# sp-uhh/buddy

Measured on AMD Instinct MI355X. Metric: diffusion steps/sec (4 s@16 kHz utterance, blind Euler-Heun DPS, order 1, 10 operator updates/step), higher is better.
Workload: dtype f32 (GEMM operands -- Winograd-domain and 1x1 / NIN -- as two-term f16 splits, 2^-22, fp32 accumulation)

## Files before the change

### buddy_amd/_lib.py

```python
from __future__ import annotations

import ctypes as C
import os

_HERE = os.path.dirname(os.path.abspath(__file__))
LIB_PATH = os.path.join(_HERE, "libbuddy_hip.so")


class BuddyHipError(RuntimeError):
    pass


_lib = None

_f32p = C.c_void_p
_SIGS = {
    "buddy_last_error": (C.c_char_p, []),
    "buddy_version": (C.c_int, []),
    "buddy_ncsnpp_param_count": (C.c_int, [C.c_int, C.POINTER(C.c_int), C.c_int, C.c_int, C.POINTER(C.c_longlong)]),
    "buddy_ncsnpp_create": (C.c_int, [_f32p, C.c_longlong, C.c_int, C.POINTER(C.c_int), C.c_int, C.c_int, C.c_int, C.c_int,
                                      C.POINTER(C.c_void_p)]),
    "buddy_ncsnpp_param_count_attn": (C.c_int, [C.c_int, C.POINTER(C.c_int), C.c_int, C.c_int, C.c_int, C.POINTER(C.c_longlong)]),
    "buddy_ncsnpp_create_attn": (C.c_int, [_f32p, C.c_longlong, C.c_int, C.POINTER(C.c_int), C.c_int, C.c_int, C.c_int, C.c_int, C.c_int,
                                           C.POINTER(C.c_void_p)]),
    "buddy_ncsnpp_destroy": (C.c_int, [C.c_void_p]),
    "buddy_ncsnpp_replica": (C.c_int, [C.c_void_p, C.POINTER(C.c_void_p)]),
    "buddy_ncsnpp_weight_bytes": (C.c_int, [C.c_void_p, C.POINTER(C.c_longlong), C.POINTER(C.c_longlong), C.POINTER(C.c_longlong),
                                            C.POINTER(C.c_int)]),
    "buddy_conv3_weight_prep": (C.c_int, [_f32p, C.c_int, C.c_int, C.c_int, C.c_int, _f32p, C.c_void_p]),
    "buddy_ncsnpp_reserve": (C.c_int, [C.c_void_p, C.c_int, C.c_int, C.c_int, C.POINTER(C.c_longlong)]),
    "buddy_ncsnpp_forward": (C.c_int, [C.c_void_p, _f32p, _f32p, _f32p, _f32p, _f32p, _f32p, C.c_int, C.c_int, C.c_int, C.c_void_p]),
    "buddy_ncsnpp_vjp": (C.c_int, [C.c_void_p, _f32p, _f32p, C.c_void_p]),
    "buddy_ncsnpp_vjp_params": (C.c_int, [C.c_void_p, _f32p, _f32p, _f32p, C.c_int, C.c_void_p]),
    "buddy_ncsnpp_update_params": (C.c_int, [C.c_void_p, _f32p, C.c_void_p]),
    "buddy_optim_sqnorm_chunk": (C.c_longlong, []),
    "buddy_optim_sqnorm": (C.c_int, [_f32p, C.c_longlong, C.c_void_p, C.c_void_p, C.c_void_p]),
    "buddy_optim_step": (C.c_int, [_f32p, _f32p, _f32p, _f32p, _f32p, C.c_longlong, C.c_void_p, C.c_double, C.c_double, C.c_double, C.c_double,
                                   C.c_double, C.c_double, C.c_double, C.POINTER(C.c_longlong), C.c_int, C.c_void_p]),
    "buddy_optim_ema": (C.c_int, [_f32p, _f32p, C.c_longlong, C.c_double, C.c_void_p]),
    "buddy_ncsnpp_tap": (C.c_int, [C.c_void_p, C.c_int, C.POINTER(C.c_void_p), C.POINTER(C.c_int * 4)]),
    "buddy_prof_enable": (C.c_int, [C.c_int]),
    "buddy_wpe": (C.c_int, [_f32p, _f32p, _f32p, C.c_int, C.c_int, C.c_int, C.c_int, C.c_int, C.c_void_p]),
    "buddy_wpe_workspace_bytes": (C.c_longlong, [C.c_int, C.c_int]),
    "buddy_wpe_dereverb": (C.c_int, [_f32p, _f32p, C.c_void_p, C.c_int, C.c_int, C.c_int, C.c_int, C.c_int, C.c_void_p]),
    "buddy_prof_collect_wino4": (C.c_int, [C.POINTER(C.c_double), C.POINTER(C.c_double), C.POINTER(C.c_double), C.POINTER(C.c_double), C.POINTER(C.c_double),
                                           C.POINTER(C.c_longlong)]),
    "buddy_prof_collect_hbm": (C.c_int, [C.POINTER(C.c_double), C.POINTER(C.c_double), C.POINTER(C.c_longlong)]),
    "buddy_prof_collect": (C.c_int, [C.POINTER(C.c_double), C.POINTER(C.c_double), C.POINTER(C.c_longlong), C.POINTER(C.c_double), C.POINTER(C.c_double)]),
    "buddy_copy_d2d": (C.c_int, [C.c_void_p, C.c_void_p, C.c_longlong, C.c_void_p]),
    "buddy_hbm_ubench": (C.c_int, [C.c_void_p, C.c_void_p, C.c_longlong, C.c_int, C.c_int, C.c_int, C.c_void_p]),
    "buddy_mfma_ubench": (C.c_int, [_f32p, _f32p, C.c_int, C.c_int, C.c_void_p, C.c_void_p]),
    "buddy_mfma_ubench_bf16": (C.c_int, [_f32p, _f32p, C.c_int, C.c_int, C.c_void_p, C.c_void_p]),
    "buddy_gemm": (C.c_int, [_f32p, C.c_int, C.c_int, _f32p, C.c_int, C.c_int, _f32p, C.c_int, C.c_int, C.c_int, C.c_int, C.c_float,
                             _f32p, C.c_int, C.c_int, C.c_longlong, C.c_longlong, C.c_longlong, C.c_void_p]),
    "buddy_gemm_winograd_domain": (C.c_int, [_f32p, _f32p, _f32p, C.c_int, C.c_int, C.c_int, C.c_int, C.c_void_p]),
    "buddy_wgemm_packed_bytes": (C.c_longlong, [C.c_int, C.c_int, C.c_int]),
    "buddy_wgemm_pack_weights": (C.c_int, [_f32p, C.c_void_p, C.c_int, C.c_int, C.c_int, C.c_void_p]),
    "buddy_gemm_winograd_domain_bf16x3": (C.c_int, [_f32p, C.c_void_p, _f32p, C.c_int, C.c_int, C.c_int, C.c_int, C.c_void_p]),
    "buddy_wgemm_f16x2_packed_bytes": (C.c_longlong, [C.c_int, C.c_int, C.c_int]),
    "buddy_wgemm_f16x2_pack_weights": (C.c_int, [_f32p, C.c_void_p, C.c_int, C.c_int, C.c_int, C.c_void_p]),
    "buddy_gemm_winograd_domain_f16x2": (C.c_int, [_f32p, C.c_void_p, _f32p, C.c_int, C.c_int, C.c_int, C.c_int, C.c_void_p, C.c_int, C.c_void_p]),
    "buddy_wgemm_f16_packed_bytes": (C.c_longlong, [C.c_int, C.c_int, C.c_int]),
    "buddy_wgemm_f16_pack_weights": (C.c_int, [_f32p, C.c_void_p, C.c_int, C.c_int, C.c_int, C.c_void_p]),
    "buddy_gemm_winograd_domain_f16": (C.c_int, [C.c_void_p, C.c_void_p, C.c_void_p, _f32p, C.c_int, C.c_int, C.c_int, C.c_int, C.c_void_p]),
    "buddy_conv3x3_winograd6_f16": (C.c_int, [_f32p, C.c_void_p, _f32p, _f32p, _f32p, C.c_int, C.c_int, C.c_int, C.c_int, C.c_int, C.c_void_p]),
    "buddy_abs_max_bits": (C.c_int, [_f32p, C.c_int, C.c_int, C.c_longlong, C.c_void_p, C.c_void_p]),
    "buddy_gemm_bf16x3": (C.c_int, [_f32p, C.c_int, _f32p, C.c_int, C.c_int, C.c_void_p, _f32p, C.c_int, C.c_longlong, C.c_int, C.c_int, _f32p, C.c_float,
                                    C.c_int, C.c_void_p]),
    "buddy_conv3x3": (C.c_int, [_f32p, _f32p, _f32p, _f32p, C.c_int, C.c_int, C.c_int, C.c_int, C.c_int, C.c_void_p]),
    "buddy_winograd_transform_weights": (C.c_int, [C.c_void_p, C.c_int, C.c_int, C.c_void_p]),
    "buddy_winograd4_transform_weights": (C.c_int, [C.c_void_p, C.c_int, C.c_int, C.c_void_p]),
    "buddy_conv3x3_winograd4": (C.c_int, [_f32p, _f32p, _f32p, _f32p, _f32p, C.c_int, C.c_int, C.c_int, C.c_int, C.c_int, C.c_void_p]),
    "buddy_winograd6_transform_weights": (C.c_int, [C.c_void_p, C.c_int, C.c_int, C.c_void_p]),
    "buddy_conv3x3_winograd6": (C.c_int, [_f32p, _f32p, _f32p, _f32p, _f32p, C.c_int, C.c_int, C.c_int, C.c_int, C.c_int, C.c_void_p]),
    "buddy_gn_conv3x3_winograd6": (C.c_int, [_f32p, _f32p, C.c_int, _f32p, _f32p, C.c_int, C.c_int, _f32p, _f32p, _f32p, _f32p, _f32p, C.c_void_p,
                                             C.c_void_p, C.c_int, C.c_int, C.c_int, C.c_int, C.c_int, C.c_void_p]),
    "buddy_gn_conv3x3_winograd6_f16": (C.c_int, [_f32p, _f32p, C.c_int, _f32p, _f32p, C.c_int, C.c_int, _f32p, _f32p, _f32p, _f32p, _f32p, C.c_void_p,
                                                 C.c_void_p, C.c_int, C.c_int, C.c_int, C.c_int, C.c_int, C.c_void_p]),
    "buddy_conv3x3_winograd6_gn_bwd_sums": (C.c_int, [_f32p, _f32p, _f32p, _f32p, _f32p, _f32p, C.c_int, _f32p, _f32p, _f32p, C.c_int, C.c_int,
                                                      C.c_void_p, C.c_void_p, C.c_int, C.c_int, C.c_int, C.c_int, C.c_int, C.c_void_p]),
    "buddy_gemm_bf16x3_gn_bwd": (C.c_int, [_f32p, C.c_int, C.c_void_p, _f32p, _f32p, C.c_int, _f32p, _f32p, _f32p, _f32p, C.c_int, C.c_int, C.c_float,
                                           _f32p, _f32p, C.c_int, C.c_int, C.c_void_p, _f32p, C.c_int, C.c_int, C.c_int, C.c_int, C.c_void_p]),
    "buddy_gemm_f16x2": (C.c_int, [_f32p, C.c_int, _f32p, C.c_int, C.c_int, C.c_void_p, _f32p, C.c_int, C.c_longlong, C.c_int, C.c_int, _f32p, C.c_float,
                                    C.c_int, C.c_void_p]),
    "buddy_gemm_f16x2_gn_bwd": (C.c_int, [_f32p, C.c_int, C.c_void_p, _f32p, _f32p, C.c_int, _f32p, _f32p, _f32p, _f32p, C.c_int, C.c_int, C.c_float,
                                           _f32p, _f32p, C.c_int, C.c_int, C.c_void_p, _f32p, C.c_int, C.c_int, C.c_int, C.c_int, C.c_void_p]),
    "buddy_gn_upconv3x3_winograd6": (C.c_int, [_f32p, _f32p, _f32p, C.c_int, C.c_int, _f32p, _f32p, _f32p, _f32p, _f32p, C.c_void_p, C.c_void_p,
                                               C.c_int, C.c_int, C.c_int, C.c_int, C.c_int, C.c_void_p]),
    "buddy_gn_upconv3x3_winograd6_f16": (C.c_int, [_f32p, _f32p, _f32p, C.c_int, C.c_int, _f32p, _f32p, _f32p, _f32p, _f32p, C.c_void_p, C.c_void_p,
                                                   C.c_int, C.c_int, C.c_int, C.c_int, C.c_int, C.c_void_p]),
    "buddy_gnbwd_upconv3x3_winograd6": (C.c_int, [_f32p, _f32p, _f32p, _f32p, _f32p, C.c_int, C.c_int, _f32p, _f32p, _f32p, C.c_void_p, _f32p,
                                                  C.c_int, C.c_int, C.c_int, C.c_int, C.c_int, C.c_void_p]),
    "buddy_gnbwd_upconv3x3_winograd6_f16": (C.c_int, [_f32p, _f32p, _f32p, _f32p, _f32p, C.c_int, C.c_int, _f32p, _f32p, _f32p, C.c_void_p, _f32p,
                                                      C.c_int, C.c_int, C.c_int, C.c_int, C.c_int, C.c_void_p]),
    "buddy_gnbwd_conv3x3_winograd6": (C.c_int, [_f32p, _f32p, _f32p, _f32p, _f32p, C.c_int, C.c_int, _f32p, _f32p, _f32p, C.c_void_p, _f32p,
                                                C.c_int, C.c_int, C.c_int, C.c_int, C.c_int, C.c_void_p]),
    "buddy_gnbwd_conv3x3_winograd6_f16": (C.c_int, [_f32p, _f32p, _f32p, _f32p, _f32p, C.c_int, C.c_int, _f32p, _f32p, _f32p, C.c_void_p, _f32p,
                                                    C.c_int, C.c_int, C.c_int, C.c_int, C.c_int, C.c_void_p]),
    "buddy_gn_conv3x3_winograd4": (C.c_int, [_f32p, _f32p, C.c_int, _f32p, _f32p, C.c_int, C.c_int, _f32p, _f32p, _f32p, _f32p, _f32p, C.c_void_p,
                                             C.c_void_p, C.c_int, C.c_int, C.c_int, C.c_int, C.c_int, C.c_void_p]),
    "buddy_conv3x3_winograd": (C.c_int, [_f32p, _f32p, _f32p, _f32p, C.c_int, C.c_int, C.c_int, C.c_int, C.c_int, C.c_void_p]),
    "buddy_groupnorm_act": (C.c_int, [_f32p, _f32p, _f32p, _f32p, _f32p, C.c_void_p, C.c_int, C.c_int, C.c_int, C.c_int, C.c_int,
                                      C.c_int, C.c_int, C.c_void_p]),
    "buddy_groupnorm_act_bwd": (C.c_int, [_f32p, _f32p, _f32p, _f32p, _f32p, _f32p, C.c_void_p, _f32p, C.c_int, C.c_int, C.c_int,
                                          C.c_int, C.c_int, C.c_int, C.c_int, C.c_void_p]),
    "buddy_fir_resample2": (C.c_int, [_f32p, _f32p, C.c_int, C.c_int, C.c_int, C.c_int, C.c_int, C.c_float, C.c_int, C.c_void_p]),
    "buddy_ncsnpp_set_fir": (C.c_int, [C.c_void_p, C.c_int]),
    "buddy_ncsnpp_set_gemm": (C.c_int, [C.c_void_p, C.c_int]),
    "buddy_ncsnpp_set_attention": (C.c_int, [C.c_void_p, C.c_int]),
    "buddy_options_check": (C.c_int, []),
    "buddy_option_validate": (C.c_int, [C.c_char_p, C.c_int]),
    "buddy_ncsnpp_set_option": (C.c_int, [C.c_void_p, C.c_char_p, C.c_int]),
    "buddy_ncsnpp_get_option": (C.c_int, [C.c_void_p, C.c_char_p, C.POINTER(C.c_int)]),
    "buddy_flash_attention_fwd": (C.c_int, [_f32p, _f32p, _f32p, _f32p, _f32p, C.c_int, C.c_int, C.c_int, C.c_float, C.c_int, C.c_void_p]),
    "buddy_flash_attention_bwd": (C.c_int, [_f32p, _f32p, _f32p, _f32p, _f32p, _f32p, _f32p, _f32p, _f32p, _f32p, C.c_int, C.c_int, C.c_int, C.c_float,
                                            C.c_int, C.c_void_p]),
    "buddy_flash_attention16_workspace": (C.c_longlong, [C.c_int, C.c_int, C.c_int]),
    "buddy_flash_attention16_fwd": (C.c_int, [_f32p, _f32p, _f32p, _f32p, _f32p, C.c_int, C.c_int, C.c_int, C.c_float, C.c_int, _f32p, C.c_void_p]),
    "buddy_flash_attention16_bwd": (C.c_int, [_f32p, _f32p, _f32p, _f32p, _f32p, _f32p, _f32p, _f32p, _f32p, _f32p, C.c_int, C.c_int, C.c_int, C.c_float,
                                              C.c_int, _f32p, C.c_void_p]),
    "buddy_flash_attention_splits": (C.c_int, [C.c_int, C.c_int]),
    "buddy_flash_attention_workspace": (C.c_longlong, [C.c_int, C.c_int, C.c_int, C.c_int]),
    "buddy_flash_attention_fwd_split": (C.c_int, [_f32p, _f32p, _f32p, _f32p, _f32p, C.c_int, C.c_int, C.c_int, C.c_float, C.c_int, _f32p, C.c_void_p]),
    "buddy_flash_attention_bwd_split": (C.c_int, [_f32p, _f32p, _f32p, _f32p, _f32p, _f32p, _f32p, _f32p, _f32p, _f32p, C.c_int, C.c_int, C.c_int, C.c_float,
                                                  C.c_int, _f32p, C.c_void_p]),
    "buddy_axpby_rows": (C.c_int, [_f32p, _f32p, _f32p, _f32p, _f32p, C.c_int, C.c_int, C.c_void_p]),
    "buddy_perturb": (C.c_int, [_f32p, _f32p, C.c_float, _f32p, C.c_longlong, C.c_void_p]),
    "buddy_dps_update": (C.c_int, [_f32p, _f32p, _f32p, _f32p, _f32p, _f32p, _f32p, C.c_float, C.c_float, C.c_float, C.c_float, _f32p, _f32p, _f32p,
                                   C.c_int, C.c_int, C.c_void_p]),
    "buddy_row_scale": (C.c_int, [_f32p, _f32p, C.c_int, C.c_int, C.c_int, C.c_float, C.c_float, C.c_void_p]),
    "buddy_fill_rows4": (C.c_int, [_f32p, C.c_int, C.c_float, C.c_float, C.c_float, C.c_float, C.c_void_p]),
    "buddy_row_moments": (C.c_int, [_f32p, C.c_void_p, C.c_int, C.c_int, C.c_void_p]),
    "buddy_blindop_create": (C.c_int, [C.c_int, C.c_int, C.c_int, C.c_int, C.c_int, C.POINTER(C.c_float), C.c_int, C.c_float, C.c_float, C.c_float,
                                       C.c_float, C.c_float, C.c_int, C.c_int, C.POINTER(C.c_void_p)]),
    "buddy_blindop_destroy": (C.c_int, [C.c_void_p]),
    "buddy_blindop_set_params": (C.c_int, [C.c_void_p, _f32p, _f32p, _f32p, C.c_int, C.c_void_p]),
    "buddy_blindop_get_params": (C.c_int, [C.c_void_p, _f32p, _f32p, _f32p, C.c_void_p]),
    "buddy_blindop_update_H": (C.c_int, [C.c_void_p, _f32p, C.c_void_p]),
    "buddy_blindop_get_H": (C.c_int, [C.c_void_p, _f32p, C.c_void_p]),
    "buddy_blindop_set_y": (C.c_int, [C.c_void_p, _f32p, C.c_void_p]),
    "buddy_blindop_degrade": (C.c_int, [C.c_void_p, _f32p, _f32p, C.c_void_p]),
    "buddy_blindop_time_rir": (C.c_int, [C.c_void_p, _f32p, C.c_void_p]),
    "buddy_blindop_design_filter": (C.c_int, [C.c_void_p, _f32p, C.c_void_p]),
    "buddy_blindop_apply_stft": (C.c_int, [C.c_void_p, _f32p, _f32p, C.c_void_p]),
    "buddy_blindop_degrade_vjp": (C.c_int, [C.c_void_p, _f32p, _f32p, _f32p, _f32p, C.c_void_p]),
    "buddy_blindop_time_rir_vjp": (C.c_int, [C.c_void_p, _f32p, _f32p, C.c_void_p]),
    "buddy_blindop_update_H_vjp": (C.c_int, [C.c_void_p, _f32p, _f32p, _f32p, _f32p, C.c_void_p]),
    "buddy_blindop_stft": (C.c_int, [C.c_void_p, _f32p, C.c_int, _f32p, C.c_void_p]),
    "buddy_blindop_stft_adjoint": (C.c_int, [C.c_void_p, _f32p, C.c_int, _f32p, C.c_void_p]),
    "buddy_blindop_stft_loss": (C.c_int, [C.c_void_p, _f32p, _f32p, C.c_int, C.c_float, _f32p, _f32p, _f32p, C.c_void_p]),
    "buddy_blindop_set_compression": (C.c_int, [C.c_void_p, C.c_float]),
    "buddy_blindop_set_loss_norm": (C.c_int, [C.c_void_p, C.c_int]),
    "buddy_blindop_set_loss": (C.c_int, [C.c_void_p, C.c_int, C.c_int, C.c_int, C.c_float]),
    "buddy_blindop_set_freq_weights": (C.c_int, [C.c_void_p, C.c_int, _f32p]),
    "buddy_blindop_lengths": (C.c_int, [C.c_void_p, C.POINTER(C.c_int), C.POINTER(C.c_int), C.POINTER(C.c_int), C.POINTER(C.c_int)]),
    "buddy_blindop_minphase": (C.c_int, [C.c_void_p, _f32p, _f32p, C.c_void_p]),
    "buddy_blindop_project": (C.c_int, [C.c_void_p, C.c_void_p]),
    "buddy_blindop_get_adam": (C.c_int, [C.c_void_p, _f32p, _f32p, _f32p, _f32p, _f32p, _f32p, C.POINTER(C.c_int), C.c_void_p]),
    "buddy_blindop_rec_loss_grad": (C.c_int, [C.c_void_p, _f32p, C.c_float, _f32p, _f32p, C.c_void_p]),
    "buddy_blindop_fir_loss_grad": (C.c_int, [C.c_void_p, _f32p, _f32p, C.c_longlong, C.c_int, C.c_float, _f32p, _f32p, C.c_void_p]),
    "buddy_blindop_param_grads": (C.c_int, [C.c_void_p, _f32p, _f32p, C.c_float, C.c_float, C.c_float, _f32p, _f32p, _f32p, _f32p, C.c_void_p]),
    "buddy_blindop_optimize": (C.c_int, [C.c_void_p, _f32p, _f32p, C.c_float, C.c_int, C.c_float, C.c_float, C.c_float, C.c_float, C.c_float,
                                         C.c_float, C.c_void_p]),
    "buddy_fir": (C.c_int, [_f32p, _f32p, C.c_longlong, _f32p, C.c_int, C.c_int, C.c_int, C.c_int, C.c_void_p]),
}
EXPORTED = sorted(_SIGS)


def load():
    global _lib
    if _lib is None:
        if not os.path.exists(LIB_PATH):
            raise BuddyHipError(f"{LIB_PATH} not found: build it with `python -c 'import __graft_entry__ as g; g.build()'` "
                                "(buddy_amd/csrc/build.sh); there is no CPU fallback")
        import torch
        lib = C.CDLL(LIB_PATH)
        for name, (res, args) in _SIGS.items():
            fn = getattr(lib, name)
            fn.restype, fn.argtypes = res, args
        _lib = lib
        rc = lib.buddy_options_check()
        if rc != 0:
            msg = lib.buddy_last_error().decode()
            _lib = None
            raise BuddyHipError(f"libbuddy_hip: {msg}")
    return _lib


# ... 25 lines not shown
```

### buddy_amd/csrc/capi.hip

```cpp
#include "../../include/buddy_hip.h"
#include "common.h"
#include "net.h"

#include <cstring>

using namespace buddy;

namespace buddy {
void launch_axpby_rows(const float* x, const float* y, const float* a, const float* c, float* out, int B, int L, hipStream_t st);
void launch_row_moments(const float* x, double* out, int B, int L, hipStream_t st);
void launch_perturb(const float* x, const float* eps, float scale, float* out, long long n, hipStream_t st);
void launch_dps_update(const float* x_hat, const float* x_den, const float* lh, const float* lh_scale_b, const float* den_scale_b, const float* base, const float* d_prev,
                       float t, float dt, float w_prev, float w_cur, float* out, float* d_out, float* x_den_out, int B, int L, hipStream_t st);
void launch_row_scale(const float* x, float* out, int B, int L, int mode, float p0, float p1, hipStream_t st);
void launch_fill_rows4(float* out, int B, float v0, float v1, float v2, float v3, hipStream_t st);
void launch_mfma_ubench(const float* seed, float* out, int blocks, int iters, unsigned long long* clk, hipStream_t st);
void launch_mfma_ubench_bf16(const float* seed, float* out, int blocks, int iters, unsigned long long* clk, hipStream_t st);
int launch_hbm_ubench(const void* src, void* dst, long long bytes, int mode, int nt, int blocks, hipStream_t st);
void launch_fir(const float* x, const float* h, long long h_stride, float* y, int B, int L, int M, int adjoint, hipStream_t st);
}

static int finish() {
  hipError_t e = hipGetLastError();
  if (e != hipSuccess) { set_error(std::string("kernel launch: ") + hipGetErrorString(e)); return BUDDY_ERR_HIP; }
// ... 412 lines not shown
  W4Gn gn;
  gn.x.p0 = x; gn.x.p1 = nullptr; gn.x.C0 = C; gn.x.ld0 = C; gn.x.ld1 = 0;
  gn.stats = stats; gn.gamma = gamma; gn.beta = beta; gn.G = G; gn.silu = silu; gn.da = da; gn.ldda = C; gn.red = red;
  launch_gn_bwd_sums(gn.x, stats, gamma, beta, da, B, up ? 2 * H : H, up ? 2 * W : W, C, G, 0, silu, stat_scratch, red, st);
  long long vf = 0, mf = 0; wino6_scratch(p, &vf, &mf, up);
  launch_wino6(p, U6, scratch, scratch + vf, st, &gn, nullptr, nullptr, U1, up, U1 ? 3 : 1);
  return finish();
}
int buddy_gnbwd_conv3x3_winograd6(const float* x, const float* gamma, const float* beta, const float* stats, const float* da, int G, int silu,
                                  const float* U6, float* y, float* scratch, double* stat_scratch, float* red, int B, int H, int W, int C, int Cout,
                                  void* stream) {
  return gnbwd_conv3x3_winograd6(0, x, gamma, beta, stats, da, G, silu, U6, nullptr, y, scratch, stat_scratch, red, B, H, W, C, Cout, stream);
}
int buddy_gnbwd_conv3x3_winograd6_f16(const float* x, const float* gamma, const float* beta, const float* stats, const float* da, int G, int silu,
                                      const void* U1, float* y, float* scratch, double* stat_scratch, float* red, int B, int H, int W, int C, int Cout,
                                      void* stream) {
  if (!U1) { set_error("null argument"); return BUDDY_ERR_ARG; }
  return gnbwd_conv3x3_winograd6(0, x, gamma, beta, stats, da, G, silu, nullptr, U1, y, scratch, stat_scratch, red, B, H, W, C, Cout, stream);
}

static int gn_upconv3x3_winograd6(const float* x, const float* gamma, const float* beta, int G, int silu, const float* U6up, const void* U1, const float* bias,
                                  float* y, float* scratch, float* stats, double* stat_scratch, double* csum, int B, int H, int W, int Cin, int Cout, void* stream) {
  if (!x || !gamma || !beta || !(U6up || U1) || !y || !scratch || !stats || !stat_scratch || G < 1 || Cin % 4 || (Cin / G) % 4 || Cin > 1024 || Cout % 4 ||
      (U1 && !wgemm_f16_supported(4 * Cout, Cin))) {
    set_error("bad arguments"); return BUDDY_ERR_ARG;
  }
  hipStream_t st = (hipStream_t)stream;
  IgemmParams p; std::memset(&p, 0, sizeof(p));
  p.ldA0 = Cin; p.Cin = Cin; p.H = H; p.W = W; p.M = B * H * W; p.N = Cout; p.C = y; p.ldC = Cout;
  p.bias_n = bias; p.alpha = 1.f; p.out_scale = 1.f; p.rows_per_batch = H * W;
  if (!wino6_supported(p)) { set_error("shape not supported by the F(6x6,3x3) path (H, W >= 6; Cin, Cout multiples of 4)"); return BUDDY_ERR_ARG; }
  const int sc = csum ? wino6_stat_chunks(p, 1) : 0;
  if (csum && (sc == 0 || (long long)sc * Cout > 256LL * 1024)) { set_error("shape not supported by the statistics epilogue"); return BUDDY_ERR_ARG; }
  W4Gn gn;
  gn.x.p0 = x; gn.x.p1 = nullptr; gn.x.C0 = Cin; gn.x.ld0 = Cin; gn.x.ld1 = 0;
  gn.stats = stats; gn.gamma = gamma; gn.beta = beta; gn.G = G; gn.silu = silu;
  launch_gn_stats(gn.x, B, H * W, Cin, G, 1e-6f, stat_scratch, stats, st);
  long long vf = 0, mf = 0; wino6_scratch(p, &vf, &mf, 1);
  launch_wino6(p, U6up, scratch, scratch + vf, st, &gn, csum ? stat_scratch : nullptr, nullptr, U1, 1, U1 ? 3 : 1);
  if (csum) launch_csum_collapse(stat_scratch, sc, B, Cout, csum, st);
  return finish();
}

int buddy_gn_upconv3x3_winograd6(const float* x, const float* gamma, const float* beta, int G, int silu, const float* U6up, const float* bias, float* y,
                                 float* scratch, float* stats, double* stat_scratch, double* csum, int B, int H, int W, int Cin, int Cout, void* stream) {
  return gn_upconv3x3_winograd6(x, gamma, beta, G, silu, U6up, nullptr, bias, y, scratch, stats, stat_scratch, csum, B, H, W, Cin, Cout, stream);
}
int buddy_gn_upconv3x3_winograd6_f16(const float* x, const float* gamma, const float* beta, int G, int silu, const void* U1up, const float* bias, float* y,
                                     float* scratch, float* stats, double* stat_scratch, double* csum, int B, int H, int W, int Cin, int Cout, void* stream) {
  if (!U1up) { set_error("null argument"); return BUDDY_ERR_ARG; }
  return gn_upconv3x3_winograd6(x, gamma, beta, G, silu, nullptr, U1up, bias, y, scratch, stats, stat_scratch, csum, B, H, W, Cin, Cout, stream);
}

int buddy_gnbwd_upconv3x3_winograd6(const float* h, const float* gamma, const float* beta, const float* stats, const float* da, int G, int silu,
                                    const float* U6upT, float* y, float* scratch, double* stat_scratch, float* red, int B, int H, int W, int C,
                                    int Cout, void* stream) {
  return gnbwd_conv3x3_winograd6(2, h, gamma, beta, stats, da, G, silu, U6upT, nullptr, y, scratch, stat_scratch, red, B, H, W, C, Cout, stream);
}
int buddy_gnbwd_upconv3x3_winograd6_f16(const float* h, const float* gamma, const float* beta, const float* stats, const float* da, int G, int silu,
                                        const void* U1upT, float* y, float* scratch, double* stat_scratch, float* red, int B, int H, int W, int C,
                                        int Cout, void* stream) {
  if (!U1upT) { set_error("null argument"); return BUDDY_ERR_ARG; }
  return gnbwd_conv3x3_winograd6(2, h, gamma, beta, stats, da, G, silu, nullptr, U1upT, y, scratch, stat_scratch, red, B, H, W, C, Cout, stream);
}

int buddy_groupnorm_act(const float* x, const float* gamma, const float* beta, float* y, float* stats, void* scratch, int B, int H, int W, int C,
                        int G, int mode, int silu, void* stream) {
  if (!x || !y || !stats || !scratch || C % 4 || (C / G) % 4 || C > 1024) { set_error("bad groupnorm arguments"); return BUDDY_ERR_ARG; }
  Src2 s; s.p0 = x; s.p1 = nullptr; s.C0 = C; s.ld0 = C; s.ld1 = 0;
  launch_gn_stats(s, B, H * W, C, G, 1e-6f, (double*)scratch, stats, (hipStream_t)stream);
  launch_gn_apply(s, stats, gamma, beta, B, H, W, C, G, mode, silu, y, nullptr, (hipStream_t)stream);
  return finish();
}

int buddy_groupnorm_act_bwd(const float* x, const float* gamma, const float* beta, const float* stats, const float* dy, float* dx, void* scratch,
                            float* red, int B, int H, int W, int C, int G, int mode, int silu, void* stream) {
  if (!x || !dy || !dx || !stats || !scratch || !red || C % 4 || (C / G) % 4 || C > 1024) { set_error("bad groupnorm arguments"); return BUDDY_ERR_ARG; }
  Src2 s; s.p0 = x; s.p1 = nullptr; s.C0 = C; s.ld0 = C; s.ld1 = 0;
  Dst2 d; d.p0 = dx; d.p1 = nullptr; d.C0 = C; d.ld0 = C; d.ld1 = 0; d.acc0 = 0; d.acc1 = 0;
  launch_gn_bwd(s, stats, gamma, beta, dy, B, H, W, C, G, mode, silu, nullptr, 0, 0.f, (double*)scratch, red, d, (hipStream_t)stream);
  return finish();
}

int buddy_options_check(void) { return options_check(); }
int buddy_option_validate(const char* key, int value) { Options o = default_options(); return option_set(o, key, value); }
int buddy_ncsnpp_set_option(void* h, const char* key, int value) { if (!h) { set_error("null handle"); return BUDDY_ERR_ARG; } return net_set_option((Net*)h, key, value); }
int buddy_ncsnpp_get_option(void* h, const char* key, int* value) { if (!h) { set_error("null handle"); return BUDDY_ERR_ARG; } return net_get_option((Net*)h, key, value); }
int buddy_ncsnpp_set_gemm(void* h, int mode) { if (!h) { set_error("null handle"); return BUDDY_ERR_ARG; } return net_set_gemm((Net*)h, mode); }
int buddy_ncsnpp_set_attention(void* h, int mode) { if (!h) { set_error("null handle"); return BUDDY_ERR_ARG; } return net_set_attention((Net*)h, mode); }
int buddy_ncsnpp_set_fir(void* h, int fir) { if (!h) { set_error("null handle"); return BUDDY_ERR_ARG; } return net_set_fir((Net*)h, fir); }
int buddy_fir_resample2(const float* x, float* y, int B, int H, int W, int C, int up, float scale, int accumulate, void* stream) {
  if (!x || !y || B < 1 || H < 1 || W < 1 || C < 1 || (!up && ((H | W) & 1))) { set_error("bad resample arguments"); return BUDDY_ERR_ARG; }
  if (up) launch_fir_up2(x, y, B, H, W, C, scale, accumulate, (hipStream_t)stream);
  else launch_fir_down2(x, y, B, H, W, C, scale, accumulate, (hipStream_t)stream);
  return finish();
}

int buddy_flash_attention_fwd(const float* q, const float* k, const float* v, float* O, float* lse, int B, int T, int C, float scale, int prec,
                              void* stream) {
  if (!q || !k || !v || !O || !lse || B < 1 || T < 1 || !flash_attn_supported(C) || prec != 0) {
    set_error("bad attention arguments (C in {32, 64, 128, 256}; prec 0 -- the 16-bit-operand kernels are buddy_flash_attention16_*)"); return BUDDY_ERR_ARG;
  }
  launch_flash_attn_fwd(q, k, v, O, lse, B, T, C, scale, nullptr, 1, (hipStream_t)stream);
  return finish();
}
long long buddy_flash_attention16_workspace(int B, int T, int C) { return (B < 1 || T < 1 || !flash_attn16_supported(C)) ? 0 : flash_attn16_ws_floats(B, T, C); }
int buddy_flash_attention16_fwd(const float* q, const float* k, const float* v, float* O, float* lse, int B, int T, int C, float scale, int prec, float* ws,
                                void* stream) {
  if (!q || !k || !v || !O || !lse || !ws || B < 1 || T < 1 || !flash_attn16_supported(C) || prec < 1 || prec > 2) {
    set_error("bad attention arguments (C in {64, 128, 256}; prec 1 = bf16, 2 = f16; ws = buddy_flash_attention16_workspace floats)"); return BUDDY_ERR_ARG;
  }
  launch_flash_attn16_fwd(q, k, v, O, lse, B, T, C, scale, prec, ws, (hipStream_t)stream);
  return finish();
}
int buddy_flash_attention16_bwd(const float* q, const float* k, const float* v, const float* O, const float* dO, const float* lse, float* delta, float* dq,
                                float* dk, float* dv, int B, int T, int C, float scale, int prec, float* ws, void* stream) {
  if (!q || !k || !v || !O || !dO || !lse || !delta || !dq || !dk || !dv || !ws || B < 1 || T < 1 || !flash_attn16_supported(C) || prec < 1 || prec > 2) {
    set_error("bad attention arguments (C in {64, 128, 256}; prec 1 = bf16, 2 = f16; ws = buddy_flash_attention16_workspace floats)"); return BUDDY_ERR_ARG;
  }
  launch_flash_attn16_bwd(q, k, v, O, dO, lse, delta, dq, dk, dv, B, T, C, scale, prec, ws, (hipStream_t)stream);
  return finish();
}
long long buddy_flash_attention_workspace(int B, int T, int C, int splits) {
  if (B < 1 || T < 1 || !flash_attn_supported(C)) return 0;
  return flash_attn_ws_floats(B, T, C, splits > 0 ? splits : flash_attn_splits(B, T));
}
int buddy_flash_attention_splits(int B, int T) { return (B < 1 || T < 1) ? 1 : flash_attn_splits(B, T); }
static bool split_args_ok(int T, int splits, const float* ws) {
  const int nb = (T + 31) / 32;
  if (splits < 1 || splits > nb || (splits > 1 && !ws)) return false;
  return splits == 1 || (long long)((nb + splits - 1) / splits) * (splits - 1) < nb;
}
int buddy_flash_attention_fwd_split(const float* q, const float* k, const float* v, float* O, float* lse, int B, int T, int C, float scale, int splits,
                                    float* ws, void* stream) {
  if (!q || !k || !v || !O || !lse || B < 1 || T < 1 || !flash_attn_supported(C) || !split_args_ok(T, splits, ws)) {
    set_error("bad split-attention arguments (C in {32, 64, 128, 256}; every split needs at least one 32-row block)"); return BUDDY_ERR_ARG;
  }
  launch_flash_attn_fwd(q, k, v, O, lse, B, T, C, scale, ws, splits, (hipStream_t)stream);
  return finish();
}
int buddy_flash_attention_bwd_split(const float* q, const float* k, const float* v, const float* O, const float* dO, const float* lse, float* delta,
                                    float* dq, float* dk, float* dv, int B, int T, int C, float scale, int splits, float* ws, void* stream) {
  if (!q || !k || !v || !O || !dO || !lse || !delta || !dq || !dk || !dv || B < 1 || T < 1 || !flash_attn_supported(C) || !split_args_ok(T, splits, ws)) {
    set_error("bad split-attention arguments (C in {32, 64, 128, 256}; every split needs at least one 32-row block)"); return BUDDY_ERR_ARG;
  }
  launch_flash_attn_bwd(q, k, v, O, dO, lse, delta, dq, dk, dv, B, T, C, scale, ws, splits, (hipStream_t)stream);
  return finish();
}
int buddy_flash_attention_bwd(const float* q, const float* k, const float* v, const float* O, const float* dO, const float* lse, float* delta, float* dq,
                              float* dk, float* dv, int B, int T, int C, float scale, int prec, void* stream) {
  if (prec != 0 || !q || !k || !v || !O || !dO || !lse || !delta || !dq || !dk || !dv || B < 1 || T < 1 || !flash_attn_supported(C)) {
    set_error("bad attention arguments (C in {32, 64, 128, 256}; prec 0 -- the 16-bit-operand kernels are buddy_flash_attention16_*)"); return BUDDY_ERR_ARG;
  }
  launch_flash_attn_bwd(q, k, v, O, dO, lse, delta, dq, dk, dv, B, T, C, scale, nullptr, 1, (hipStream_t)stream);
  return finish();
}

int buddy_axpby_rows(const float* x, const float* y, const float* a, const float* c, float* out, int B, int L, void* stream) {
  if (!x || !a || !out || (y && !c)) { set_error("null argument"); return BUDDY_ERR_ARG; }
  launch_axpby_rows(x, y, a, c, out, B, L, (hipStream_t)stream);
  return finish();
}

int buddy_perturb(const float* x, const float* eps, float scale, float* out, long long n, void* stream) {
  if (!x || !eps || !out) { set_error("null argument"); return BUDDY_ERR_ARG; }
  launch_perturb(x, eps, scale, out, n, (hipStream_t)stream);
// ... 124 lines not shown
```

### buddy_amd/csrc/common.h

```cpp
#pragma once
#include <hip/hip_runtime.h>
#include <cstdint>
#include <cstdio>

#define BUDDY_OK 0
#define BUDDY_ERR_HIP 1
#define BUDDY_ERR_ARG 2
#define BUDDY_ERR_STATE 3

namespace buddy {

struct Options {
  int conv;
  int gemm;
  int attn;
  int gn_fuse, upconv, c2_fuse;
  int attn_split, attn_nw;
  int wgemm_rt, gen_f16x2, gen_rows, gen_cp, gnb_nt;
  int c2out_tiled;
  int op_graph;
};
const Options& default_options();
int options_check();
const Options& cur_opt();
struct OptScope { const Options* prev; explicit OptScope(const Options* o); ~OptScope(); OptScope(const OptScope&) = delete; };
int option_set(Options& o, const char* key, int value);
int option_get(const Options& o, const char* key, int* value);
const char* prof_dump_path();

struct IgemmParams {
  const float* A0; const float* A1; int C0; int ldA0; int ldA1;
  int Cin;
  int H, W;
  int M, N;
  const float* Bt; int ldB;
  float* C; int ldC;
  long long sA, sB, sC;
  const float* bias_n; const float* bias_m; const float* bias_bn; int ld_bias_bn; int rows_per_batch;
  const float* res; int ldRes; int res_mode;
  float alpha, out_scale; int accumulate;
  int wide_epi;
  int tag;
};
void launch_igemm(const IgemmParams& p, int taps, bool transA, bool transB, int batch, hipStream_t st);
bool wgemm_supported(int Cout, int Cin);
size_t wgemm_packed_bytes(int P, int Cout, int Cin);
void wgemm_pack_weights(const float* U_dev, void* U3_dev, int P, int Cout, int Cin, hipStream_t st);
void launch_wgemm_bf16x3(const float* V, const void* U3, float* M, long long Mt, int Cout, int Cin, int P, hipStream_t st);
bool wgemm_f16x2_supported(int Cout, int Cin);
size_t wgemm_f16x2_packed_bytes(int P, int Cout, int Cin);
void wgemm_f16x2_pack_weights(const float* U_dev, void* U2_dev, int P, int Cout, int Cin, hipStream_t st);
constexpr int VMAX_SUB = 64, VMAX_STRIDE = 32;
void launch_abs_max_bits(const float* x, int groups, int segments, long long seg_len, unsigned* out, hipStream_t st);
void launch_wgemm_f16x2(const float* V, const void* U2, float* M, long long Mt, int Cout, int Cin, int P, const unsigned* vmax, int tiles_per_utt, hipStream_t st);
bool wgemm_f16_supported(int Cout, int Cin);
size_t wgemm_f16_packed_bytes(int P, int Cout, int Cin);
void wgemm_f16_pack_weights(const float* U_dev, void* U1_dev, int P, int Cout, int Cin, hipStream_t st);
void launch_wgemm_f16(const void* V16, const signed char* vexp, const void* U1, float* M, long long Mt, int Cout, int Cin, int P, hipStream_t st);
bool wgemm_general_supported(int N, int K, int C0, int ldA0, int ldA1, int ldC, const void* A0, const void* A1, const void* C, const void* bias);
void launch_wgemm_bf16x3_general(const float* A0, int ldA0, const float* A1, int ldA1, int C0, const void* W3, float* C, int ldC, long long M, int N, int K,
                                 const float* bias_n, float alpha, int accumulate, hipStream_t st);
bool wgemm_f16x2_general_supported(int N, int K, int C0, int ldA0, int ldA1, int ldC, const void* A0, const void* A1, const void* C, const void* bias);
void launch_wgemm_f16x2_general(const float* A0, int ldA0, const float* A1, int ldA1, int C0, const void* W2, float* C, int ldC, long long M, int N, int K,
                                const float* bias_n, float alpha, int accumulate, hipStream_t st);
bool wino_supported(const IgemmParams& p);
void launch_wino(const IgemmParams& p, const float* Uw, hipStream_t st);
void wino_transform_weights(const float* wt_host, int Cout, int Cin, float* U_host);
struct Src2 { const float* p0; const float* p1; int C0; int ld0; int ld1; };
struct Dst2 { float* p0; float* p1; int C0; int ld0; int ld1; int acc0; int acc1; };
bool wgemm_gnbwd_supported(int N, int K, int ldA, const Src2& x, const Dst2& d, const void* A, const void* da);
void launch_wgemm_bf16x3_gnbwd(const float* A, int ldA, const void* W3, long long M, int N, int K, float alpha, Src2 x, const float* da, const float* stats,
                               const float* red, const float* gamma, const float* beta, int G, int silu, int HW, Dst2 d, hipStream_t st);
void launch_wgemm_f16x2_gnbwd(const float* A, int ldA, const void* W2, long long M, int N, int K, float alpha, Src2 x, const float* da, const float* stats,
                              const float* red, const float* gamma, const float* beta, int G, int silu, int HW, Dst2 d, hipStream_t st);
struct W4Gn { Src2 x; const float* stats; const float* gamma; const float* beta; int G; int silu;
              const float* da = nullptr; int ldda = 0; const float* red = nullptr; };
bool wino4_supported(const IgemmParams& p);
void wino4_scratch(const IgemmParams& p, long long* v_floats, long long* m_floats);
int wino4_stat_chunks(const IgemmParams& p);
void launch_wino4(const IgemmParams& p, const float* U4, float* V, float* Mb, hipStream_t st, const W4Gn* gn = nullptr, double* stat = nullptr,
                  const void* U4x = nullptr);
void wino4_transform_weights(const float* wt_host, int Cout, int Cin, float* U4_host);
bool wino6_supported(const IgemmParams& p);
bool wino6_pays(const IgemmParams& p);
void wino6_scratch(const IgemmParams& p, long long* v_floats, long long* m_floats, int up = 0);
int wino6_stat_chunks(const IgemmParams& p, int up = 0);
double wino6_exec_ratio(const IgemmParams& p, int up = 0);
void launch_wino6(const IgemmParams& p, const float* U6, float* V, float* Mb, hipStream_t st, const W4Gn* gn = nullptr, double* stat = nullptr,
                  const W4Gn* bwd_gn = nullptr, const void* U6x = nullptr, int up = 0, int xform = 1, unsigned* vmax = nullptr);
void wino6_transform_weights(const float* wt_host, int Cout, int Cin, float* U6_host);
long long conv3_weight_floats(int O, int I, int kind);
int launch_conv3_weight_prep(const float* w_oihw, int O, int I, bool dgrad, int kind, float* out, hipStream_t st);
void igemm_prof_record(const IgemmParams& p, int taps, int batch, hipStream_t st, bool begin, double exec_ratio = 4.0 / 9.0);
void igemm_prof_enable(int level);
bool igemm_prof_enabled();
int igemm_prof_level();
void prof_w4_push(hipEvent_t e0, hipEvent_t e1, hipEvent_t e2, hipEvent_t e3, double gemm_flops, double bytes_in, double bytes_out, double bytes_gemm);
int prof_w4_collect(double ms[3], double* gemm_flops, double* bytes_in, double* bytes_out, double* bytes_gemm, long long* launches);
void prof_hbm_begin(double algorithmic_bytes, hipStream_t st);
void prof_hbm_end(hipStream_t st);
int prof_hbm_collect(double* ms, double* bytes, long long* launches);
int igemm_prof_collect(double ms[2], double flops[2], long long launches[2], double bytes[2], double exec_flops[2]);

void launch_conv_c2in(const float* x, const float* w , const float* bias, const float* add, int add_ld,
                      float* y, int ldY, int B, int H, int W, int Cout, int taps, int accumulate, hipStream_t st);
void launch_conv_c2out(const float* x, int ldX, const float* w , const float* bias, const float* up_add,
                       float* y, int B, int H, int W, int Cin, int taps, int accumulate, hipStream_t st);

int  gn_num_chunks(int HW);
void launch_gn_stats(Src2 x, int B, int HW, int C, int G, float eps, double* partial, float* stats , hipStream_t st);
void launch_chan_sums(const float* x, int B, int HW, int C, double* partial, double* csum, hipStream_t st);
void launch_csum_collapse(const double* partial, int chunks, int B, int C, double* csum, hipStream_t st);
void launch_gn_stats_partial(const double* partial, int chunks, int B, int HW, int C, int G, float eps, float* stats, hipStream_t st);
void launch_gn_stats_csum(const double* csum0, const double* csum1, int C0, int B, int HW, int C, int G, float eps, float* stats, hipStream_t st);
void launch_gn_apply(Src2 x, const float* stats, const float* gamma, const float* beta, int B, int H, int W, int C, int G,
                     int mode, int silu, float* out, float* pooled_raw, hipStream_t st);
void launch_gn_bwd_sums(Src2 x, const float* stats, const float* gamma, const float* beta, const float* da, int B, int H, int W, int C, int G,
                        int mode, int silu, double* partial, float* red , hipStream_t st, int ready_chunks = 0);
void launch_gn_bwd_apply(Src2 x, const float* stats, const float* gamma, const float* beta, const float* da, int B, int H, int W, int C, int G,
                         int mode, int silu, const float* extra, int extra_mode, float extra_scale, const float* red, Dst2 dx, hipStream_t st);
void launch_gn_bwd(Src2 x, const float* stats, const float* gamma, const float* beta, const float* da, int B, int H, int W, int C,
                   int G, int mode, int silu, const float* extra, int extra_mode, float extra_scale, double* partial,
                   float* red , Dst2 dx, hipStream_t st, int ready_chunks = 0);

void launch_wpe(const double* Y, double* X, double* inv_scratch, int rows, int T, int taps, int delay, int iters, hipStream_t st);
size_t wpe_workspace_bytes(int B, int L);
int wpe_frames(int L);
void launch_wpe_dereverb(const float* y, float* out, void* work, int B, int L, int taps, int delay, int iters, hipStream_t st);
void launch_axpy(float* dst, const float* src, float alpha, long long n, int accumulate, hipStream_t st);
void launch_fir_up2(const float* x, float* y, int B, int H, int W, int C, float scale, int accumulate, hipStream_t st);
void launch_fir_down2(const float* x, float* y, int B, int H, int W, int C, float scale, int accumulate, hipStream_t st);
void launch_pool2(const float* src, float* dst, int B, int H, int W, int C, float scale, int accumulate, hipStream_t st);
void launch_up2_acc(const float* src, float* dst, int B, int Hs, int Ws, int C, float scale, int accumulate, hipStream_t st);
bool flash_attn_supported(int C);
bool flash_attn16_supported(int C);
int flash_attn_splits(int B, int T);
long long flash_attn_ws_floats(int B, int T, int C, int splits);
void launch_flash_attn_fwd(const float* q, const float* k, const float* v, float* O, float* Lse, int B, int T, int C, float scale, float* ws, int splits,
                           hipStream_t st);
void launch_flash_attn_bwd(const float* q, const float* k, const float* v, const float* O, const float* dO, const float* Lse, float* D, float* dq,
                           float* dk, float* dv, int B, int T, int C, float scale, float* ws, int splits, hipStream_t st);
long long flash_attn16_ws_floats(int B, int T, int C);
void launch_flash_attn16_fwd(const float* q, const float* k, const float* v, float* O, float* Lse, int B, int T, int C, float scale, int prec, float* ws,
                             hipStream_t st);
void launch_flash_attn16_bwd(const float* q, const float* k, const float* v, const float* O, const float* dO, const float* Lse, float* D, float* dq,
                             float* dk, float* dv, int B, int T, int C, float scale, int prec, float* ws, hipStream_t st);
void launch_softmax_rows(float* S, int rows, int cols, hipStream_t st);
void launch_softmax_bwd_rows(const float* P, float* dP , int rows, int cols, hipStream_t st);
void launch_linear(const float* x, const float* W, const float* b, float* y, int B, int K, int N, int silu_in, hipStream_t st);
void launch_fourier(const float* cnoise, const float* Wf, float* out, int B, int nf, hipStream_t st);
void launch_mix2(const float* x, const float* w , const float* b, float* y, long long npix, int transpose, int accumulate, hipStream_t st);

void launch_reflect_pad(const float* x, float* xp, int B, int L, int pad, int Lp, float scale, const float* scale_b, hipStream_t st);
void launch_ola(const float* frames, int ldF, int Tp, int n_fft, int hop, const float* inv_env, float* y, int B, int L,
                int pad, const float* xin, const float* cskip_b, const float* cout_b, hipStream_t st);
void launch_ola_adj(const float* g, int B, int L, int pad, int Tp, int n_fft, int hop, const float* inv_env, const float* cout_b,
                    float* frames, int ldF, hipStream_t st);
void launch_unpad_adj(const float* dframes, int ldF, int T, int n_fft, int hop, int B, int L, int pad, float scale,
                      const float* scale_b, const float* g_out, const float* cskip_b, float* dx, hipStream_t st);

inline int cdiv(long long a, long long b) { return (int)((a + b - 1) / b); }

struct WgY { const float* p; long long T, sb, sm, sn; };
struct WgA { Src2 x; int H, W, Cin, taps, rs; const float* stats; const float* gamma; const float* beta; int G, silu; };
int wgrad_chunks(long long M, int N, int K);
long long wgrad_ws_floats(long long M, int N, int K);
void launch_wgrad(const WgY& y, const WgA& a, long long M, int N, int layout, float alpha, float* ws, float* out, hipStream_t st);
long long colsum_ws_floats(int B, long long T, int N);
void launch_colsum(const WgY& y, int B, int N, float alpha, float* ws, float* bc, int ld_bc, float* out, float* out2, hipStream_t st);
long long basis_bias_ws_floats(int B, long long T, int K);
void launch_basis_bias(const float* x, int K, int B, long long T, const double* bsum, float* ws, float* out, hipStream_t st);
long long gn_pgrad_ws_floats(int B, int H, int W, int C);
void launch_gn_pgrad(const Src2& x, const float* stats, const float* gamma, const float* beta, int G, int silu, const float* da, int da_mode, int B,
                     int H, int W, int C, float* ws, float* dgamma, float* dbeta, hipStream_t st);
void launch_linear_bwd_w(const float* dy, int ld_dy, const float* x, int silu_in, int B, int N, int K, float* gw, float* gb, float* gb2, hipStream_t st);
void launch_linear_bwd_x(const float* dy, const float* W, const float* x, int silu_in, int B, int N, int K, float* dx, hipStream_t st);

}
```

### buddy_amd/csrc/net.hip

```cpp
#include "common.h"
#include "net.h"

#include <algorithm>
#include <cmath>
#include <cstdlib>
#include <cstring>
#include <deque>
#include <functional>
#include <memory>
#include <mutex>
#include <string>
#include <vector>
#include <unordered_map>

namespace buddy {

#define HIPCHK(x) do { hipError_t e_ = (x); if (e_ != hipSuccess) { set_error(std::string(#x) + ": " + hipGetErrorString(e_)); return BUDDY_ERR_HIP; } } while (0)

static thread_local std::string g_err;
void set_error(const std::string& s) { g_err = s; }
const char* last_error() { return g_err.c_str(); }

static const float INV_SQRT2 = 0.70710678118654752440f;

// ... 62 lines not shown
  return v.back().off + v.back().numel;
}

struct Tens {
  float* p = nullptr; float* g = nullptr; int ginit = 0;
  int B = 0, H = 0, W = 0, C = 0;
  double* csum = nullptr; bool has_csum = false;
  long long numel() const { return (long long)B * H * W * C; }
};
struct View { Tens* a = nullptr; Tens* b = nullptr; int C() const { return a->C + (b ? b->C : 0); } };

struct Arena {
  char* base = nullptr; size_t cap = 0, off = 0, peak = 0; bool dry = false; bool overflow = false;
  void* alloc(size_t bytes) {
    off = (off + 255) & ~(size_t)255;
    void* r = dry ? (void*)(uintptr_t)(0x10000 + off) : (void*)(base + off);
    off += bytes;
    if (off > peak) peak = off;
    if (!dry && off > cap) overflow = true;
    return r;
  }
  float* f(long long n) { return (float*)alloc((size_t)n * 4); }
};

struct WVar { float* u = nullptr; void* x[4] = {nullptr, nullptr, nullptr, nullptr}; };
struct ConvW { int cin = 0, cout = 0, taps = 0; const float* raw = nullptr; float* wf = nullptr; float* wb = nullptr; float* bias = nullptr;
               mutable WVar var[2][5];
               long long go = -1; };
struct GNW { float* gamma = nullptr; float* beta = nullptr; int C = 0; long long go = -1; };
struct ResW { GNW gn0, gn1; ConvW c0, c1, c2; bool has_c2 = false; int cin = 0, cout = 0, dense_off = 0; long long dense_go = -1; };
struct AttnW { GNW gn; float* Wt[4]; float* Wn[4]; float* b[4]; int C = 0; int level = -1;
               long long go[4] = {-1, -1, -1, -1}; };

struct W3Img { const void* img; int N, K; const void* img2 = nullptr; };
struct Weights {
  NetCfg cfg;
  std::vector<PSpec> specs;
  float* dparams = nullptr;
  float* dpacked = nullptr;
  std::vector<long long> doff;
  std::vector<float> host_pack;
  std::vector<std::pair<long long, std::function<std::vector<float>(const float*)>>> repack;
  struct Img { const float* src; void* img; void* img2; int n, k; };
  std::vector<Img> imgs;
  int gen = 0;
  long long lin1_go = -1, lin2_go = -1, out_go = -1;
  float* Wf = nullptr; float* lin1_w = nullptr; float* lin1_b = nullptr; float* lin2_w = nullptr; float* lin2_b = nullptr;
  float* dense_w = nullptr; float* dense_b = nullptr; int dense_total = 0;
  ConvW conv_in;
  std::vector<ResW> res;
  std::vector<ConvW> combine;
  AttnW attn;
  std::vector<AttnW> sites;
  std::vector<GNW> pyr_gn; std::vector<ConvW> pyr_conv;
  float* out_w = nullptr; float* out_b = nullptr;
  float* basisF = nullptr; float* basisI = nullptr;
  double* basisI_sum = nullptr;
  unsigned char* dpacked3 = nullptr;
  std::unordered_map<const float*, W3Img> w3;
  std::mutex mu;
  std::vector<void*> lazy_allocs; size_t lazy_bytes = 0; int lazy_count = 0;
  float* prep_tmp = nullptr; size_t prep_cap = 0;
  ~Weights() {
    if (dparams) (void)hipFree(dparams);
    if (dpacked) (void)hipFree(dpacked);
    if (dpacked3) (void)hipFree(dpacked3);
    if (basisI_sum) (void)hipFree(basisI_sum);
    if (prep_tmp) (void)hipFree(prep_tmp);
    for (void* q : lazy_allocs) (void)hipFree(q);
  }
};

struct Net {
  NetCfg cfg;
  int Fb = 0, Kp = 0, pad = 0;
  std::shared_ptr<Weights> W;
  int B = 0, L = 0, T = 0, Tp = 0, Lp = 0;
  float* inv_env = nullptr; int env_len = 0; int env_Tp = -1;
  Arena arena;
  std::deque<Tens> pool;
  std::vector<std::function<void()>> tape;
  std::vector<std::pair<int, Tens*>> taps;
  double* partial = nullptr; float* red = nullptr;
  bool have_tape = false;
  hipStream_t st = nullptr;
  bool pgrad = false, pg_run = false; float* pg = nullptr; float* dtemb = nullptr; int tape_gen = 0;
  const float* k_four = nullptr; const float* k_t1 = nullptr; const float* k_temb = nullptr;
  Tens* spec = nullptr; Tens* pyr0 = nullptr;
  const float* k_cin = nullptr; const float* k_cskip = nullptr; const float* k_cout = nullptr;

  int rsv_B = 0, rsv_L = 0, rsv_vjp = -1;
  Options opt;
  bool prep_failed = false;
  bool fir = false;
  float* w4_scratch = nullptr; size_t w4_cap = 0, w4_need = 0;
  unsigned* vmax = nullptr; size_t vmax_cap = 0; int vslot = 0, vslots = 0, vdry = 0;
  int vslot_need[2] = {0, 0};
  bool dry() const { return arena.dry; }
  Tens* mk(int B_, int H, int W, int C, bool grad) {
    pool.emplace_back();
    Tens* t = &pool.back();
    t->B = B_; t->H = H; t->W = W; t->C = C;
    t->p = arena.f(t->numel());
    if (grad) t->g = arena.f(t->numel());
    t->csum = (double*)arena.alloc((size_t)B_ * C * 2 * sizeof(double));
    return t;
  }
  float* tmp(long long n) { return arena.f(n); }
};

namespace {
struct Packer {
  std::vector<float> buf;
  long long put(const std::vector<float>& v) {
    long long off = (long long)buf.size();
    buf.insert(buf.end(), v.begin(), v.end());
    while (buf.size() % 64) buf.push_back(0.f);
    return off;
  }
};

inline float w3(const float* w, int O, int I, int o, int i, int dy, int dx) { return w[(((long long)o * I + i) * 3 + dx) * 3 + dy]; }

std::vector<float> transpose2(const float* w, int R, int Cc) {
  std::vector<float> r((size_t)R * Cc);
  for (int i = 0; i < R; ++i) for (int j = 0; j < Cc; ++j) r[(size_t)j * R + i] = w[(size_t)i * Cc + j];
  return r;
}
}

static const PSpec* find_spec(const std::vector<PSpec>& v, const std::string& n) {
  for (auto& s : v) if (s.name == n) return &s;
  return nullptr;
}


static int weights_create(const float* hp, long long n, const NetCfg& cfg, std::shared_ptr<Weights>* out) {
  auto Wp = std::make_shared<Weights>();
  Weights* N = Wp.get();
  N->cfg = cfg;
  N->specs = build_specs(cfg);
  if (n != param_count(cfg)) { set_error("parameter blob size mismatch"); return BUDDY_ERR_ARG; }
  if (cfg.n_fft % 2) { set_error("n_fft must be even"); return BUDDY_ERR_ARG; }
  if (cfg.attn_mask < 0 || (cfg.attn_mask >> cfg.nlev) != 0) { set_error("attention mask selects a level the network does not have"); return BUDDY_ERR_ARG; }
  {
    int cmax = 0;
    for (int l = 0; l < cfg.nlev; ++l) cmax = std::max(cmax, cfg.nf * cfg.ch_mult[l]);
    if (2 * cmax > 1024) { set_error("nf * max(ch_mult) must be <= 512 (concatenated skip tensors of up to 1024 channels)"); return BUDDY_ERR_ARG; }
  }
  for (const PSpec& ps : N->specs) {
    if (ps.name.find("GroupNorm_") == std::string::npos) continue;
    const int C = ps.shape[0];
    if (C % 4 || (C > 128 && C % 128)) {
      set_error("unsupported width: a GroupNorm over " + std::to_string(C) + " channels (" + ps.name + ") has " + std::to_string(C / (C / 4 < 32 ? C / 4 : 32)) +
                " channels per group; the kernels need a multiple of 4 (C <= 128 or C % 128 == 0)");
      return BUDDY_ERR_ARG;
    }
  }
  const int Fb = cfg.n_fft / 2 + 1, Kp = (cfg.n_fft + 3) / 4 * 4;
  if (Fb % (1 << (cfg.nlev - 1))) { set_error("frequency bins not divisible by 2^(levels-1)"); return BUDDY_ERR_ARG; }
  std::vector<long long>& doff = N->doff;
  doff.resize(N->specs.size());
  {
    long long o = 0;
    for (size_t i = 0; i < N->specs.size(); ++i) { doff[i] = o; o += (N->specs[i].numel + 63) / 64 * 64; }
    HIPCHK(hipMalloc(&N->dparams, (size_t)o * 4));
// ... 321 lines not shown
  const int ki = kind == 0 ? 0 : kind == 2 ? 1 : kind == 4 ? 2 : kind == 6 ? 3 : 4;
  WVar& v = c.var[dgrad ? 1 : 0][ki];
  std::lock_guard<std::mutex> lk(Wt->mu);
  if (want_x ? v.x[want_x] != nullptr : v.u != nullptr) return &v;
  const int ph = kind == 61 ? 4 : 1;
  const int Co = dgrad ? c.cin : ph * c.cout, Ci = dgrad ? ph * c.cout : c.cin;
  const size_t nfl = (size_t)conv3_weight_floats(c.cout, c.cin, kind);
  hipStream_t st = N->st;
  float* u = v.u;
  if (u == nullptr) {
    if (want_x) {
      if (Wt->prep_cap < nfl) {
        if (Wt->prep_tmp) (void)hipFree(Wt->prep_tmp);
        Wt->prep_tmp = nullptr; Wt->prep_cap = 0;
        if (hipMalloc(&Wt->prep_tmp, nfl * 4) != hipSuccess) { N->prep_failed = true; set_error("out of memory preparing convolution weights"); return nullptr; }
        Wt->prep_cap = nfl;
      }
      u = Wt->prep_tmp;
    } else {
      if (hipMalloc(&u, nfl * 4) != hipSuccess) { N->prep_failed = true; set_error("out of memory preparing convolution weights"); return nullptr; }
      Wt->lazy_allocs.push_back(u); Wt->lazy_bytes += nfl * 4;
    }
    if (launch_conv3_weight_prep(c.raw, c.cout, c.cin, dgrad, kind, u, st) != BUDDY_OK) { N->prep_failed = true; set_error("bad weight form"); return nullptr; }
  }
  void* x = nullptr;
  if (want_x) {
    const int P = kind == 4 ? 36 : 64;
    const size_t bytes = kArith[want_x].packed_bytes(P, Co, Ci);
    if (hipMalloc(&x, bytes) != hipSuccess) { N->prep_failed = true; set_error("out of memory preparing convolution weights"); return nullptr; }
    Wt->lazy_allocs.push_back(x); Wt->lazy_bytes += bytes;
    kArith[want_x].pack_weights(u, x, P, Co, Ci, st);
  }
  (void)hipStreamSynchronize(st);
  if (want_x) v.x[want_x] = x; else v.u = u;
  ++Wt->lazy_count;
  return &v;
}

static Src2 src_of(const View& v) {
  Src2 s; s.p0 = v.a->p; s.p1 = v.b ? v.b->p : nullptr; s.C0 = v.a->C; s.ld0 = v.a->C; s.ld1 = v.b ? v.b->C : 0;
  return s;
}
static Dst2 gdst_of(const View& v) {
  Dst2 d; d.p0 = v.a->g; d.p1 = v.b ? v.b->g : nullptr; d.C0 = v.a->C; d.ld0 = v.a->C; d.ld1 = v.b ? v.b->C : 0;
  d.acc0 = v.a->ginit; d.acc1 = v.b ? v.b->ginit : 0;
  v.a->ginit = 1; if (v.b) v.b->ginit = 1;
  return d;
}
static IgemmParams ig_base() {
  IgemmParams p; std::memset(&p, 0, sizeof(p));
  p.alpha = 1.f; p.out_scale = 1.f; p.rows_per_batch = 1; p.H = 1; p.W = 1;
  return p;
}
static inline int gn_groups(int C) { int g = C / 4; return g < 32 ? g : 32; }

struct Conv3 {
  const float* a = nullptr;
  int B = 0, H = 0, W = 0, Cin = 0, Cout = 0;
  const ConvW* w = nullptr; bool dgrad = false;
  const float* bias = nullptr; const float* bias_bn = nullptr; int ld_bn = 0;
  const float* res = nullptr; int ldRes = 0; int res_mode = 0;
  float alpha = 1.f, out_scale = 1.f;
  float* out = nullptr;
  const W4Gn* gn = nullptr; float* gn_tmp = nullptr;
  Tens* stat_out = nullptr; bool direct = false;
  const W4Gn* bwd_gn = nullptr;
  int up = 0;
};
static unsigned* vmax_slot(Net* N, int B) {
  if (N->vmax == nullptr || N->vslot >= N->vslots || (size_t)(N->vslot + 1) * B * VMAX_SUB * VMAX_STRIDE > N->vmax_cap) { N->prep_failed = true; set_error("abs-max slots of the f16x2 GEMM exhausted"); return nullptr; }
  return N->vmax + (size_t)(N->vslot++) * B * VMAX_SUB * VMAX_STRIDE;
}
static bool conv3_up_ok(Net* N, int B, int H, int W, int Cin, int Cout) {
  if (H < 7 || W < 7) return false;
  const Options& o = N->opt;
  const bool on = o.conv == 0 && o.gn_fuse && o.upconv;
  if (!on || Cin % 8 || Cout % 8 || H < 6 || W < 6) return false;
  IgemmParams p = ig_base();
  p.ldA0 = Cin; p.Cin = Cin; p.H = H; p.W = W; p.M = B * H * W; p.N = Cout; p.ldC = Cout; p.ld_bias_bn = 4;
  if (!wino6_supported(p) || !wino6_pays(p)) return false;
  const int sc = wino6_stat_chunks(p, 1);
  return sc > 0 && (long long)sc * Cout <= 256LL * 1024 && (long long)wino6_stat_chunks(p, 0) * Cin <= 256LL * 1024;
}
static int conv3(Net* N, const Conv3& c) {
  const float* a = c.a; const int B = c.B, H = c.H, W = c.W, Cin = c.Cin, Cout = c.Cout;
  if (N->prep_failed) return -1;
  if (N->dry()) ++N->vdry;
  const bool wino_ok = c.w != nullptr && c.w->raw != nullptr && Cin % 8 == 0 && Cout % 8 == 0;
  const W4Gn* gn = c.gn; float* gn_tmp = c.gn_tmp; Tens* stat_out = c.stat_out; const W4Gn* bwd_gn = c.bwd_gn; const bool direct = c.direct;
  const int cmode = N->opt.conv;
  const bool use_wino = cmode != 1, use_wino4 = cmode != 1 && cmode != 2, use_wino6 = use_wino4 && cmode != 3;
  if (N->dry()) {
    if (use_wino4 && wino_ok && H % 4 == 0 && W % 4 == 0) {
      const size_t need = (size_t)36 * ((size_t)B * H * W / 16) * (size_t)(Cin + Cout);
      if (need > N->w4_need) N->w4_need = need;
    }
    if (use_wino6 && wino_ok && H >= 6 && W >= 6) {
      const size_t th = c.up == 1 ? H / 7 + 1 : c.up == 2 ? (H + 6) / 7 : (H + 5) / 6, tw = c.up == 1 ? W / 7 + 1 : c.up == 2 ? (W + 6) / 7 : (W + 5) / 6;
      const size_t need = (size_t)64 * ((size_t)B * th * tw) * (size_t)((c.up == 2 ? 4 : 1) * Cin + (c.up == 1 ? 4 : 1) * Cout);
      if (need > N->w4_need) N->w4_need = need;
    }
    return 0;
  }
  if (c.up) {
    IgemmParams p = ig_base();
    p.A0 = a; p.ldA0 = Cin; p.Cin = Cin; p.H = H; p.W = W; p.M = B * H * W; p.N = Cout; p.C = c.out; p.ldC = Cout;
    p.bias_n = c.bias; p.bias_bn = c.bias_bn; p.ld_bias_bn = c.ld_bn; p.rows_per_batch = H * W; p.alpha = c.alpha; p.out_scale = c.out_scale;
    const int x3 = gemm_arith(N, (c.up == 1 ? 4 : 1) * Cout, (c.up == 2 ? 4 : 1) * Cin);
    const WVar* wv = conv_weights(N, *c.w, c.dgrad, 61, x3);
    unsigned* vm = x3 == 2 ? vmax_slot(N, B) : nullptr;
    if (x3 == 2 && !vm) return -1;
    if (!wv || N->w4_scratch == nullptr) { if (wv) { N->prep_failed = true; set_error("convolution scratch buffer missing"); } return -1; }
    long long vf = 0, mf = 0; wino6_scratch(p, &vf, &mf, c.up);
    const bool want_bwd = c.up == 2 && bwd_gn != nullptr;
    const int sc = (c.up == 1 ? stat_out != nullptr : want_bwd) ? wino6_stat_chunks(p, c.up) : 0;
    const bool stat = sc > 0 && (long long)sc * Cout <= 256LL * 1024;
    IgemmParams pr = p; pr.M = 4 * p.M;
    const double xr = wino6_exec_ratio(p, c.up);
    igemm_prof_record(pr, 9, 1, N->st, true, xr);
    launch_wino6(p, wv->u, N->w4_scratch, N->w4_scratch + vf, N->st, gn, stat ? N->partial : nullptr, (stat && want_bwd) ? bwd_gn : nullptr,
                 wv->x[x3], c.up, x3, vm);
    igemm_prof_record(pr, 9, 1, N->st, false, xr);
    if (stat && (want_bwd || direct)) return sc;
    if (stat && stat_out) { launch_csum_collapse(N->partial, sc, B, Cout, stat_out->csum, N->st); stat_out->has_csum = true; }
    return 0;
  }
  IgemmParams p = ig_base();
  p.A0 = a; p.ldA0 = Cin; p.Cin = Cin; p.H = H; p.W = W; p.M = B * H * W; p.N = Cout;
  p.Bt = nullptr; p.ldB = 9 * Cin; p.C = c.out; p.ldC = Cout;
  p.bias_n = c.bias; p.bias_bn = c.bias_bn; p.ld_bias_bn = c.ld_bn; p.rows_per_batch = H * W;
  p.res = c.res; p.ldRes = c.ldRes; p.res_mode = c.res_mode; p.alpha = c.alpha; p.out_scale = c.out_scale;
  const bool fuse_gn = N->opt.gn_fuse != 0;
  const bool w6 = use_wino6 && wino_ok && N->w4_scratch != nullptr && wino6_supported(p) && wino6_pays(p);
  const bool w4 = !w6 && use_wino4 && wino_ok && N->w4_scratch != nullptr && wino4_supported(p);
  if (gn != nullptr && gn->da != nullptr && !(w6 && fuse_gn)) {
    Dst2 d; d.p0 = gn_tmp; d.p1 = nullptr; d.C0 = Cin; d.ld0 = Cin; d.ld1 = 0; d.acc0 = 0; d.acc1 = 0;
    launch_gn_bwd_apply(gn->x, gn->stats, gn->gamma, gn->beta, gn->da, B, H, W, Cin, gn->G, 0, gn->silu, nullptr, 0, 0.f, gn->red, d, N->st);
    p.A0 = gn_tmp; gn = nullptr;
  }
  if (gn != nullptr && gn->da == nullptr && !((w4 || w6) && fuse_gn)) {
    launch_gn_apply(gn->x, gn->stats, gn->gamma, gn->beta, B, H, W, Cin, gn->G, 0, gn->silu, gn_tmp, nullptr, N->st);
    p.A0 = gn_tmp; gn = nullptr;
  }
  const int xf = gemm_arith(N, Cout, Cin);
  if (w6) {
    const WVar* wv = conv_weights(N, *c.w, c.dgrad, 6, xf);
    if (!wv) return -1;
    unsigned* vm = xf == 2 ? vmax_slot(N, B) : nullptr;
    if (xf == 2 && !vm) return -1;
    const float* U6 = wv->u; const void* U6x = wv->x[xf];
    long long vf = 0, mf = 0; wino6_scratch(p, &vf, &mf);
    const bool want_bwd = bwd_gn != nullptr && fuse_gn;
    const int sc = ((stat_out != nullptr && fuse_gn) || want_bwd) ? wino6_stat_chunks(p) : 0;
    const bool stat = sc > 0 && (long long)sc * Cout <= 256LL * 1024;
    const double xr = wino6_exec_ratio(p);
    igemm_prof_record(p, 9, 1, N->st, true, xr);
    launch_wino6(p, U6, N->w4_scratch, N->w4_scratch + vf, N->st, gn, stat ? N->partial : nullptr, (stat && want_bwd) ? bwd_gn : nullptr, U6x, 0, xf, vm);
    igemm_prof_record(p, 9, 1, N->st, false, xr);
    if (stat && (want_bwd || direct)) return sc;
    if (stat && stat_out) { launch_csum_collapse(N->partial, sc, B, Cout, stat_out->csum, N->st); stat_out->has_csum = true; }
  } else if (w4) {
    const int x4 = xf ? 1 : 0;
    const WVar* wv = conv_weights(N, *c.w, c.dgrad, 4, x4);
    if (!wv) return -1;
    const float* U4 = wv->u; const void* U4x = wv->x[x4];
    long long vf = 0, mf = 0; wino4_scratch(p, &vf, &mf);
    const int sc = (stat_out != nullptr && fuse_gn) ? wino4_stat_chunks(p) : 0;
    const bool stat = sc > 0 && (long long)sc * Cout <= 256LL * 1024;
    igemm_prof_record(p, 9, 1, N->st, true, 0.25);
    launch_wino4(p, U4, N->w4_scratch, N->w4_scratch + vf, N->st, gn, stat ? N->partial : nullptr, U4x);
    igemm_prof_record(p, 9, 1, N->st, false, 0.25);
    if (stat) { launch_csum_collapse(N->partial, sc, B, Cout, stat_out->csum, N->st); stat_out->has_csum = true; }
  } else if (use_wino && wino_ok && wino_supported(p)) {
    const WVar* wv = conv_weights(N, *c.w, c.dgrad, 2, 0);
    if (!wv) return -1;
    igemm_prof_record(p, 9, 1, N->st, true);
    launch_wino(p, wv->u, N->st);
    igemm_prof_record(p, 9, 1, N->st, false);
  } else {
    const WVar* wv = conv_weights(N, *c.w, c.dgrad, 0, 0);
    if (!wv) return -1;
    p.Bt = wv->u;
    launch_igemm(p, 9, false, false, 1, N->st);
  }
  return 0;
}
static bool gen_f16x2_on(const Net* N, long long M) {
  if ((N->opt.gemm != 2 && N->opt.gemm != 3) || N->opt.gen_f16x2 == 0) return false;
  return N->opt.gen_f16x2 == 1 || M <= 600000;
}
static bool try_wgemm(Net* N, const IgemmParams& p) {
  if (N->opt.gemm < 1 || p.bias_m || p.bias_bn || p.res_mode || p.out_scale != 1.f || p.sA || p.sC) return false;
  const auto it = N->W->w3.find(p.Bt);
  if (it == N->W->w3.end() || p.ldB != p.Cin || it->second.N != p.N || it->second.K != p.Cin) return false;
  if (!wgemm_general_supported(p.N, p.Cin, p.A1 ? p.C0 : 0, p.ldA0, p.A1 ? p.ldA1 : 0, p.ldC, p.A0, p.A1, p.C, p.bias_n)) return false;
  igemm_prof_record(p, 1, 1, N->st, true, 1.0);
  if (gen_f16x2_on(N, p.M) && it->second.img2 && wgemm_f16x2_supported(p.N, p.Cin))
    launch_wgemm_f16x2_general(p.A0, p.ldA0, p.A1, p.ldA1, p.C0, it->second.img2, p.C, p.ldC, p.M, p.N, p.Cin, p.bias_n, p.alpha, p.accumulate, N->st);
  else
    launch_wgemm_bf16x3_general(p.A0, p.ldA0, p.A1, p.ldA1, p.C0, it->second.img, p.C, p.ldC, p.M, p.N, p.Cin, p.bias_n, p.alpha, p.accumulate, N->st);
  igemm_prof_record(p, 1, 1, N->st, false, 1.0);
  return true;
}
static void conv1(Net* N, Src2 a, long long M, int Cin, const float* wt, int Cout, const float* bias, float alpha, float* out, int accumulate) {
  if (N->dry()) return;
  IgemmParams p = ig_base();
  p.A0 = a.p0; p.A1 = a.p1; p.C0 = a.C0; p.ldA0 = a.ld0; p.ldA1 = a.ld1; p.Cin = Cin; p.M = (int)M; p.N = Cout;
  p.Bt = wt; p.ldB = Cin; p.C = out; p.ldC = Cout; p.bias_n = bias; p.alpha = alpha; p.accumulate = accumulate;
  if (try_wgemm(N, p)) return;
  launch_igemm(p, 1, false, false, 1, N->st);
}
static Src2 single(const float* p, int C) { Src2 s; s.p0 = p; s.p1 = nullptr; s.C0 = C; s.ld0 = C; s.ld1 = 0; return s; }

static void view_stats(Net* N, const View& x, int HW, int G, float* stats) {
  hipStream_t st = N->st;
  const int B = x.a->B;
  for (Tens* t : {x.a, x.b})
    if (t != nullptr && !t->has_csum) { launch_chan_sums(t->p, B, HW, t->C, N->partial, t->csum, st); t->has_csum = true; }
  launch_gn_stats_csum(x.a->csum, x.b ? x.b->csum : nullptr, x.a->C, B, HW, x.C(), G, 1e-6f, stats, st);
}

static WgY wy(const float* p, long long T, int ld) { WgY y; y.p = p; y.T = T; y.sb = T * ld; y.sm = ld; y.sn = 1; return y; }
static WgA wa(Src2 x, int H, int W, int Cin, int taps, int rs) {
  WgA a; a.x = x; a.H = H; a.W = W; a.Cin = Cin; a.taps = taps; a.rs = rs; a.stats = nullptr; a.gamma = nullptr; a.beta = nullptr; a.G = 1; a.silu = 0;
  return a;
}
static WgA wa_gn(Src2 x, int H, int W, int Cin, int taps, int rs, const float* stats, const GNW& g, int G, int silu) {
  WgA a = wa(x, H, W, Cin, taps, rs); a.stats = stats; a.gamma = g.gamma; a.beta = g.beta; a.G = G; a.silu = silu;
  return a;
}
static void pg_weight(Net* n, const WgY& y, const WgA& a, long long M, int Nn, int layout, float alpha, long long go) {
  float* ws = n->tmp(wgrad_ws_floats(M, Nn, a.taps * a.Cin));
  if (!n->dry()) launch_wgrad(y, a, M, Nn, layout, alpha, ws, n->pg + go, n->st);
}
static void pg_colsum(Net* n, const WgY& y, int B, int Nn, float alpha, float* bc, int ld_bc, long long go1, long long go2) {
  float* ws = n->tmp(colsum_ws_floats(B, y.T, Nn));
  if (!n->dry()) launch_colsum(y, B, Nn, alpha, ws, bc, ld_bc, go1 >= 0 ? n->pg + go1 : nullptr, go2 >= 0 ? n->pg + go2 : nullptr, n->st);
}
static void pg_gn(Net* n, Src2 x, const float* stats, const GNW& g, int G, int silu, const float* da, int da_mode, int B, int H, int W, int C) {
  float* ws = n->tmp(gn_pgrad_ws_floats(B, H, W, C));
  if (!n->dry()) launch_gn_pgrad(x, stats, g.gamma, g.beta, G, silu, da, da_mode, B, H, W, C, ws, n->pg + g.go, n->pg + g.go + C, n->st);
}

static Tens* resblock(Net* N, const ResW& R, View x, int mode, const float* temb_all, bool rec) {
  const int B = x.a->B, H = x.a->H, W = x.a->W, Cin = R.cin, Cout = R.cout;
  const int Ho = mode == 1 ? H / 2 : (mode == 2 ? H * 2 : H), Wo = mode == 1 ? W / 2 : (mode == 2 ? W * 2 : W);
  const int G0 = gn_groups(Cin), G1 = gn_groups(Cout);
  hipStream_t st = N->st;
  Tens* out = N->mk(B, Ho, Wo, Cout, rec);
  Tens* h1 = N->mk(B, Ho, Wo, Cout, false);
  float* stats0 = N->tmp((long long)B * G0 * 2);
  float* stats1 = N->tmp((long long)B * G1 * 2);
  const size_t mark = N->arena.off;
  const bool firm = N->fir && mode != 0;
  float* a0 = N->tmp((long long)B * Ho * Wo * Cin);
  float* xr = (mode == 1 || firm) ? N->tmp((long long)B * Ho * Wo * Cin) : nullptr;
  float* xs = R.has_c2 ? N->tmp((long long)B * ((mode == 2 && !firm) ? H * W : Ho * Wo) * Cout) : nullptr;
  float* a1 = N->tmp((long long)B * Ho * Wo * Cout);
  float* a0f = firm ? N->tmp((long long)B * H * W * Cin) : nullptr;
  const bool up6 = mode == 2 && !firm && conv3_up_ok(N, B, H, W, Cin, Cout);
  if (N->dry()) {
    Conv3 c; c.B = B; c.H = Ho; c.W = Wo; c.Cin = Cin; c.Cout = Cout; c.w = &R.c0;
    if (up6) { c.H = H; c.W = W; c.up = 1; }
    conv3(N, c);
    c.H = Ho; c.W = Wo; c.up = 0; c.Cin = Cout; c.w = &R.c1; conv3(N, c);
  }
  if (!N->dry()) {
    view_stats(N, x, H * W, G0, stats0);
    W4Gn g0{src_of(x), stats0, R.gn0.gamma, R.gn0.beta, G0, 1}, g1{single(h1->p, Cout), stats1, R.gn1.gamma, R.gn1.beta, G1, 1};
    if (firm) {
      launch_gn_apply(src_of(x), stats0, R.gn0.gamma, R.gn0.beta, B, H, W, Cin, G0, 0, 1, a0f, nullptr, st);
      if (mode == 2) { launch_fir_up2(a0f, a0, B, H, W, Cin, 1.f, 0, st); launch_fir_up2(x.a->p, xr, B, H, W, Cin, 1.f, 0, st); }
      else { launch_fir_down2(a0f, a0, B, H, W, Cin, 1.f, 0, st); launch_fir_down2(x.a->p, xr, B, H, W, Cin, 1.f, 0, st); }
    } else if (mode != 0 && !up6)
    launch_gn_apply(src_of(x), stats0, R.gn0.gamma, R.gn0.beta, B, H, W, Cin, G0, mode, 1, a0, xr, st);
    Conv3 c0; c0.a = a0; c0.B = B; c0.H = Ho; c0.W = Wo; c0.Cin = Cin; c0.Cout = Cout; c0.w = &R.c0; c0.bias = R.c0.bias;
    c0.bias_bn = temb_all + R.dense_off; c0.ld_bn = N->W->dense_total; c0.out = h1->p;
    c0.gn = (mode == 0 || up6) ? &g0 : nullptr; c0.gn_tmp = a0; c0.stat_out = h1; c0.direct = true;
    if (up6) { c0.H = H; c0.W = W; c0.up = 1; }
    const int ch1 = conv3(N, c0);
    if (ch1 > 0) launch_gn_stats_partial(N->partial, ch1, B, Ho * Wo, Cout, G1, 1e-6f, stats1, st);
    else { View vh1; vh1.a = h1; view_stats(N, vh1, Ho * Wo, G1, stats1); }
    const float* res; int res_mode = 1;
    if (R.has_c2) {
      if (mode == 1 || firm) conv1(N, single(xr, Cin), (long long)B * Ho * Wo, Cin, R.c2.wf, Cout, R.c2.bias, 1.f, xs, 0);
      else conv1(N, src_of(x), (long long)B * H * W, Cin, R.c2.wf, Cout, R.c2.bias, 1.f, xs, 0);
      res = xs; if (mode == 2 && !firm) res_mode = 2;
    } else {
      res = x.a->p;
    }
    Conv3 c1; c1.a = a1; c1.B = B; c1.H = Ho; c1.W = Wo; c1.Cin = Cout; c1.Cout = Cout; c1.w = &R.c1; c1.bias = R.c1.bias;
    c1.res = res; c1.ldRes = Cout; c1.res_mode = res_mode; c1.out_scale = INV_SQRT2; c1.out = out->p;
    c1.gn = &g1; c1.gn_tmp = a1; c1.stat_out = out;
    conv3(N, c1);
  }
  N->arena.off = mark;
  if (rec) {
    const ResW* Rp = &R;
    N->tape.push_back([=]() {
// ... 240 lines not shown
    gemm_b(N, hn, C, 0, false, A.Wt[1], C, 0, false, k, C, 0, B * T, C, C, A.b[1], nullptr, 1.f, 0, 1);
    gemm_b(N, A.Wt[2], C, 0, false, hn, C, (long long)T * C, false, vT, T, (long long)C * T, C, T, C, nullptr, A.b[2], 1.f, 0, B);
    gemm_b(N, q, C, (long long)T * C, false, k, C, (long long)T * C, false, P, T, (long long)T * T, T, T, C, nullptr, nullptr, scale, 0, B);
    launch_softmax_rows(P, B * T, T, st);
    gemm_b(N, P, T, (long long)T * T, false, vT, T, (long long)C * T, false, O, C, (long long)T * C, T, C, T, nullptr, nullptr, 1.f, 0, B);
    IgemmParams p = ig_base();
    p.A0 = O; p.ldA0 = C; p.Cin = C; p.M = B * T; p.N = C; p.Bt = A.Wt[3]; p.ldB = C; p.C = out->p; p.ldC = C; p.bias_n = A.b[3];
    p.res = x->p; p.ldRes = C; p.res_mode = 1; p.out_scale = INV_SQRT2;
    launch_igemm(p, 1, false, false, 1, st);
  }
  N->arena.off = mark;
  if (rec) {
    const AttnW* Ap = &A;
    N->tape.push_back([=]() {
      Net* n = N; hipStream_t s = n->st;
      const size_t mk = n->arena.off;
      const float* dout = out->g;
      const long long TC = (long long)T * C, TT = (long long)T * T;
      float* dO = n->tmp(B * TC); float* dP = n->tmp(B * TT); float* dvT = n->tmp(B * TC);
      float* dq = n->tmp(B * TC); float* dk = n->tmp(B * TC); float* dhn = n->tmp(B * TC);
      const bool tr = T % 32 == 0;
      float* Tr = tr ? n->tmp(B * TT) : nullptr;
      gemm_b(n, dout, C, 0, false, Ap->Wn[3], C, 0, false, dO, C, 0, B * T, C, C, nullptr, nullptr, INV_SQRT2, 0, 1);
      gemm_b(n, dO, C, TC, false, vT, T, TC, true, dP, T, TT, T, T, C, nullptr, nullptr, 1.f, 0, B);
      if (tr) {
        if (!n->dry()) launch_transpose_sq(P, Tr, B, T, s);
        gemm_b(n, Tr, T, TT, false, dO, C, TC, true, dvT, C, TC, T, C, T, nullptr, nullptr, 1.f, 0, B);
      } else
      gemm_b(n, dO, C, TC, true, P, T, TT, true, dvT, T, TC, C, T, T, nullptr, nullptr, 1.f, 0, B);
      if (!n->dry()) launch_softmax_bwd_rows(P, dP, B * T, T, s);
      gemm_b(n, dP, T, TT, false, k, C, TC, true, dq, C, TC, T, C, T, nullptr, nullptr, scale, 0, B);
      if (tr) {
        if (!n->dry()) launch_transpose_sq(dP, Tr, B, T, s);
        gemm_b(n, Tr, T, TT, false, q, C, TC, true, dk, C, TC, T, C, T, nullptr, nullptr, scale, 0, B);
      } else
      gemm_b(n, dP, T, TT, true, q, C, TC, true, dk, C, TC, T, C, T, nullptr, nullptr, scale, 0, B);
      gemm_b(n, dq, C, 0, false, Ap->Wn[0], C, 0, false, dhn, C, 0, B * T, C, C, nullptr, nullptr, 1.f, 0, 1);
      gemm_b(n, dk, C, 0, false, Ap->Wn[1], C, 0, false, dhn, C, 0, B * T, C, C, nullptr, nullptr, 1.f, 1, 1);
      if (tr) gemm_b(n, dvT, C, 0, false, Ap->Wn[2], C, 0, false, dhn, C, 0, B * T, C, C, nullptr, nullptr, 1.f, 1, 1);
      else
      gemm_b(n, dvT, T, TC, true, Ap->Wn[2], C, 0, false, dhn, C, TC, T, C, C, nullptr, nullptr, 1.f, 1, B);
      View xv; xv.a = x;
      Dst2 d = gdst_of(xv);
      if (!n->dry())
        launch_gn_bwd(single(x->p, C), stats, Ap->gn.gamma, Ap->gn.beta, dhn, B, H, W, C, G, 0, 0, dout, 1, INV_SQRT2, n->partial, n->red, d, s);
      if (n->pg_run) {
        float* O2 = n->tmp(B * TC);
        gemm_b(n, P, T, TT, false, vT, T, (long long)C * T, false, O2, C, TC, T, C, T, nullptr, nullptr, 1.f, 0, B);
        WgY ydv = wy(dvT, T, C);
        if (!tr) { ydv.sb = TC; ydv.sm = 1; ydv.sn = T; }
        attn_pgrad(n, *Ap, x, stats, dq, dk, ydv, O2, dout, dhn);
      }
      n->arena.off = mk;
    });
  }
  return out;
}

static int ensure_env(Net* N, int Tp) {
  if (N->env_Tp == Tp) return BUDDY_OK;
  const int nfft = N->cfg.n_fft, hop = N->cfg.hop;
  const int len = nfft + hop * (Tp - 1);
  std::vector<double> env(len, 0.0);
  const double PI = 3.14159265358979323846;
  for (int t = 0; t < Tp; ++t)
    for (int k = 0; k < nfft; ++k) { const double w = 0.5 - 0.5 * std::cos(2.0 * PI * k / nfft); env[t * hop + k] += w * w; }
  std::vector<float> inv(len);
  for (int i = 0; i < len; ++i) inv[i] = env[i] > 1e-11 ? (float)(1.0 / (double)(float)env[i]) : 0.f;
  if (N->inv_env) (void)hipFree(N->inv_env);
  HIPCHK(hipMalloc(&N->inv_env, (size_t)len * 4));
  HIPCHK(hipMemcpy(N->inv_env, inv.data(), (size_t)len * 4, hipMemcpyHostToDevice));
  N->env_len = len; N->env_Tp = Tp;
  return BUDDY_OK;
}

static void run_forward(Net* N, const float* x, const float* cnoise, const float* cin_b, const float* cskip_b, const float* cout_b, float* y,
                        int B, int L, bool rec) {
  const NetCfg& c = N->cfg;
  hipStream_t st = N->st;
  const int nf = c.nf, Fb = N->Fb, Kp = N->Kp, hop = c.hop, nfft = c.n_fft;
  const int T = 1 + L / hop, Tp = (T + 15) / 16 * 16;
  const int Lp = (L + nfft + 8 + 3) / 4 * 4;
  N->B = B; N->L = L; N->T = T; N->Tp = Tp; N->Lp = Lp;
  N->pool.clear(); N->tape.clear(); N->taps.clear();
  N->arena.off = 0;
  N->k_cin = N->k_cskip = N->k_cout = nullptr;
  if (cin_b) {
    float* sc = N->tmp(3 * (long long)B);
    if (!N->dry()) {
      (void)hipMemcpyAsync(sc, cin_b, (size_t)B * 4, hipMemcpyDeviceToDevice, st);
      (void)hipMemcpyAsync(sc + B, cskip_b, (size_t)B * 4, hipMemcpyDeviceToDevice, st);
      (void)hipMemcpyAsync(sc + 2 * B, cout_b, (size_t)B * 4, hipMemcpyDeviceToDevice, st);
    }
    N->k_cin = sc; N->k_cskip = sc + B; N->k_cout = sc + 2 * B;
    cin_b = N->k_cin; cskip_b = N->k_cskip; cout_b = N->k_cout;
  }
  N->partial = (double*)N->arena.alloc((size_t)B * 256 * 1024 * 2 * sizeof(double));
  N->red = N->tmp((long long)B * 32 * 2);

  float* xp = N->tmp((long long)B * Lp);
  Tens* spec = N->mk(B, Tp, Fb, 2, rec);
  N->spec = spec;
  if (!N->dry()) {
    launch_reflect_pad(x, xp, B, L, N->pad, Lp, 1.f, cin_b, st);
    (void)hipMemsetAsync(spec->p, 0, (size_t)spec->numel() * 4, st);
    gemm_b(N, xp, hop, Lp, false, N->W->basisF, Kp, 0, false, spec->p, 2 * Fb, (long long)Tp * 2 * Fb, T, 2 * Fb, Kp, nullptr, nullptr, 1.f, 0, B);
  }
  float* four = N->tmp((long long)B * 2 * nf);
  float* t1 = N->tmp((long long)B * 4 * nf);
  float* temb = N->tmp((long long)B * 4 * nf);
  float* temb_all = N->tmp((long long)B * N->W->dense_total);
  if (!N->dry()) {
    launch_fourier(cnoise, N->W->Wf, four, B, nf, st);
    launch_linear(four, N->W->lin1_w, N->W->lin1_b, t1, B, 2 * nf, 4 * nf, 0, st);
    launch_linear(t1, N->W->lin2_w, N->W->lin2_b, temb, B, 4 * nf, 4 * nf, 1, st);
    launch_linear(temb, N->W->dense_w, N->W->dense_b, temb_all, B, 4 * nf, N->W->dense_total, 1, st);
  }
  N->k_four = four; N->k_t1 = t1; N->k_temb = temb;

  int mi = 3, ri = 0, ci = 0, si = 0;
  auto tap = [&](int idx, Tens* t) { N->taps.push_back({idx, t}); };
  Tens* h0 = N->mk(B, Tp, Fb, nf, rec);
  if (!N->dry()) launch_conv_c2in(spec->p, N->W->conv_in.wf, N->W->conv_in.bias, nullptr, 0, h0->p, nf, B, Tp, Fb, nf, 9, 0, st);
  if (rec) N->tape.push_back([=]() {
    if (N->pg_run) {
      const WgY y0 = wy(h0->g, (long long)Tp * Fb, nf);
      pg_weight(N, y0, wa(single(spec->p, 2), Tp, Fb, 2, 9, 0), (long long)B * Tp * Fb, nf, 1, 1.f, N->W->conv_in.go);
      pg_colsum(N, y0, B, nf, 1.f, nullptr, 0, N->W->conv_in.go + 18LL * nf, -1);
    }
    if (N->dry()) { spec->ginit = 1; return; }
    launch_conv_c2out(h0->g, nf, N->W->conv_in.wb, nullptr, nullptr, spec->g, B, Tp, Fb, nf, 9, spec->ginit, N->st);
    spec->ginit = 1;
  });
  tap(mi, h0); ++mi;
  std::vector<Tens*> hs{h0};
  Tens* pyr_in = spec;
  for (int l = 0; l < c.nlev; ++l) {
    for (int b = 0; b < c.nrb; ++b) {
      View v; v.a = hs.back();
      Tens* h = resblock(N, N->W->res[ri++], v, 0, temb_all, rec); tap(mi, h); ++mi;
      if (c.attn_mask >> l & 1) { h = attnblock(N, N->W->sites[si++], h, rec); tap(mi, h); ++mi; }
      hs.push_back(h);
    }
    if (l != c.nlev - 1) {
      View v; v.a = hs.back();
      Tens* h = resblock(N, N->W->res[ri++], v, 1, temb_all, rec); tap(mi, h); ++mi;
      Tens* pin = N->mk(B, pyr_in->H / 2, pyr_in->W / 2, 2, rec);
      Tens* prev = pyr_in;
      if (!N->dry()) {
        if (N->fir) launch_fir_down2(prev->p, pin->p, B, prev->H, prev->W, 2, 1.f, 0, st);
        else launch_pool2(prev->p, pin->p, B, prev->H, prev->W, 2, 0.25f, 0, st);
      }
      if (rec) N->tape.push_back([=]() {
        if (!N->dry()) {
          if (N->fir) launch_fir_up2(pin->g, prev->g, B, pin->H, pin->W, 2, 0.25f, prev->ginit, N->st);
          else launch_up2_acc(pin->g, prev->g, B, pin->H, pin->W, 2, 0.25f, prev->ginit, N->st);
        }
        prev->ginit = 1;
      });
      pyr_in = pin;
      const ConvW& cw = N->W->combine[ci++];
      Tens* hc = N->mk(B, h->H, h->W, h->C, rec);
      if (!N->dry()) launch_conv_c2in(pin->p, cw.wf, cw.bias, h->p, h->C, hc->p, h->C, B, h->H, h->W, h->C, 1, 0, st);
      if (rec) { const ConvW* cwp = &cw; N->tape.push_back([=]() {
        if (!N->dry()) {
          launch_axpy(h->g, hc->g, 1.f, h->numel(), h->ginit, N->st);
          launch_conv_c2out(hc->g, h->C, cwp->wb, nullptr, nullptr, pin->g, B, h->H, h->W, h->C, 1, pin->ginit, N->st);
        }
        h->ginit = 1; pin->ginit = 1;
        if (N->pg_run) {
          const WgY yc = wy(hc->g, (long long)h->H * h->W, h->C);
          pg_weight(N, yc, wa(single(pin->p, 2), h->H, h->W, 2, 1, 0), (long long)B * h->H * h->W, h->C, 0, 1.f, cwp->go);
          pg_colsum(N, yc, B, h->C, 1.f, nullptr, 0, cwp->go + 2LL * h->C, -1);
        }
      }); }
      tap(mi, hc); ++mi;
      hs.push_back(hc);
    }
  }
  Tens* h = hs.back();
  { View v; v.a = h; h = resblock(N, N->W->res[ri++], v, 0, temb_all, rec); tap(mi, h); ++mi; }
  h = attnblock(N, N->W->attn, h, rec); tap(mi, h); ++mi;
  { View v; v.a = h; h = resblock(N, N->W->res[ri++], v, 0, temb_all, rec); tap(mi, h); ++mi; }
  Tens* pyr = nullptr;
  for (int l = c.nlev - 1, j = 0; l >= 0; --l, ++j) {
    for (int b = 0; b < c.nrb + 1; ++b) {
      View v; v.a = h; v.b = hs.back(); hs.pop_back();
      h = resblock(N, N->W->res[ri++], v, 0, temb_all, rec); tap(mi, h); ++mi;
    }
    if (c.attn_mask >> l & 1) { h = attnblock(N, N->W->sites[si++], h, rec); tap(mi, h); ++mi; }
    {
      const GNW& gw = N->W->pyr_gn[j]; const ConvW& cw = N->W->pyr_conv[j];
      const int C = h->C, G = gn_groups(C), Hh = h->H, Ww = h->W;
      Tens* np = N->mk(B, Hh, Ww, 2, rec);
      float* stats = N->tmp((long long)B * G * 2);
      const size_t mark = N->arena.off;
      float* a = N->tmp(h->numel());
      Tens* prevp = pyr; Tens* hh = h;
      if (!N->dry()) {
        { View vx; vx.a = h; view_stats(N, vx, Hh * Ww, G, stats); }
        launch_gn_apply(single(h->p, C), stats, gw.gamma, gw.beta, B, Hh, Ww, C, G, 0, 1, a, nullptr, st);
        if (N->fir) {
          launch_conv_c2out(a, C, cw.wf, cw.bias, nullptr, np->p, B, Hh, Ww, C, 9, 0, st);
          if (prevp) launch_fir_up2(prevp->p, np->p, B, Hh / 2, Ww / 2, 2, 1.f, 1, st);
        } else
        launch_conv_c2out(a, C, cw.wf, cw.bias, prevp ? prevp->p : nullptr, np->p, B, Hh, Ww, C, 9, 0, st);
      }
      N->arena.off = mark;
      if (rec) { const GNW* gp = &gw; const ConvW* cp = &cw; N->tape.push_back([=]() {
        const size_t mk = N->arena.off;
        float* da = N->tmp(hh->numel());
        if (!N->dry()) {
          if (prevp && N->fir) launch_fir_down2(np->g, prevp->g, B, Hh, Ww, 2, 4.f, prevp->ginit, N->st);
          else if (prevp) launch_pool2(np->g, prevp->g, B, Hh, Ww, 2, 1.f, prevp->ginit, N->st);
          launch_conv_c2in(np->g, cp->wb, nullptr, nullptr, 0, da, C, B, Hh, Ww, C, 9, 0, N->st);
        }
        if (prevp) prevp->ginit = 1;
        View hv; hv.a = hh;
        Dst2 d = gdst_of(hv);
        if (!N->dry()) launch_gn_bwd(single(hh->p, C), stats, gp->gamma, gp->beta, da, B, Hh, Ww, C, G, 0, 1, nullptr, 0, 0.f, N->partial, N->red, d, N->st);
        if (N->pg_run) {
          const WgY yp = wy(np->g, (long long)Hh * Ww, 2);
          pg_weight(N, yp, wa_gn(single(hh->p, C), Hh, Ww, C, 9, 0, stats, *gp, G, 1), (long long)B * Hh * Ww, 2, 1, 1.f, cp->go);
          pg_colsum(N, yp, B, 2, 1.f, nullptr, 0, cp->go + 18LL * C, -1);
          pg_gn(N, single(hh->p, C), stats, *gp, G, 1, da, 0, B, Hh, Ww, C);
        }
        N->arena.off = mk;
      }); }
      pyr = np; mi += 2; tap(mi - 1, pyr);
    }
    if (l != 0) { View v; v.a = h; h = resblock(N, N->W->res[ri++], v, 2, temb_all, rec); tap(mi, h); ++mi; }
  }
  N->pyr0 = pyr;
  float* o2 = N->tmp((long long)B * Tp * Fb * 2);
  float* frames = N->tmp((long long)B * Tp * Kp);
  if (!N->dry()) {
    launch_mix2(pyr->p, N->W->out_w, N->W->out_b, o2, (long long)B * Tp * Fb, 0, 0, st);
    gemm_b(N, o2, 2 * Fb, 0, false, N->W->basisI, 2 * Fb, 0, false, frames, Kp, 0, B * Tp, Kp, 2 * Fb, nullptr, nullptr, 1.f, 0, 1);
    launch_ola(frames, Kp, Tp, nfft, hop, N->inv_env, y, B, L, N->pad, cskip_b ? x : nullptr, cskip_b, cout_b, st);
  }
  N->have_tape = rec;
}

static void run_vjp(Net* N, const float* cot, float* gx) {
  const NetCfg& c = N->cfg;
  const int B = N->B, L = N->L, T = N->T, Tp = N->Tp, Fb = N->Fb, Kp = N->Kp, hop = c.hop, nfft = c.n_fft;
  hipStream_t st = N->st;
  for (auto& t : N->pool) t.ginit = 0;
  const size_t mark = N->arena.off;
  float* dframes = N->tmp((long long)B * Tp * Kp);
  float* do2 = N->tmp((long long)B * Tp * Fb * 2);
  if (!N->dry()) {
    launch_ola_adj(cot, B, L, N->pad, Tp, nfft, hop, N->inv_env, N->k_cout, dframes, Kp, st);
    gemm_b(N, dframes, Kp, 0, false, N->W->basisI, 2 * Fb, 0, true, do2, 2 * Fb, 0, B * Tp, 2 * Fb, Kp, nullptr, nullptr, 1.f, 0, 1);
    launch_mix2(do2, N->W->out_w, nullptr, N->pyr0->g, (long long)B * Tp * Fb, 1, 0, st);
  }
  N->pyr0->ginit = 1;
  const int nf = c.nf, DT = N->W->dense_total;
  N->dtemb = N->pg_run ? N->tmp((long long)B * DT) : nullptr;
  if (N->pg_run) {
    const WgY y2 = wy(do2, (long long)Tp * Fb, 2);
    pg_weight(N, y2, wa(single(N->pyr0->p, 2), Tp, Fb, 2, 1, 0), (long long)B * Tp * Fb, 2, 0, 1.f, N->W->out_go);
    float* wsb = N->tmp(basis_bias_ws_floats(B, Tp, Kp));
    if (!N->dry()) launch_basis_bias(dframes, Kp, B, Tp, N->W->basisI_sum, wsb, N->pg + N->W->out_go + 4, st);
  }
  for (int i = (int)N->tape.size() - 1; i >= 0; --i) N->tape[i]();
  if (N->pg_run) {
    float* dte = N->tmp((long long)B * 4 * nf);
    float* dt1 = N->tmp((long long)B * 4 * nf);
    if (!N->dry()) {
      const Weights* Wt = N->W.get();
      for (const ResW& R : Wt->res)
        launch_linear_bwd_w(N->dtemb + R.dense_off, DT, N->k_temb, 1, B, R.cout, 4 * nf, N->pg + R.dense_go, N->pg + R.dense_go + (long long)R.cout * 4 * nf,
                            nullptr, st);
      launch_linear_bwd_x(N->dtemb, Wt->dense_w, N->k_temb, 1, B, DT, 4 * nf, dte, st);
      launch_linear_bwd_w(dte, 4 * nf, N->k_t1, 1, B, 4 * nf, 4 * nf, N->pg + Wt->lin2_go, N->pg + Wt->lin2_go + 16LL * nf * nf, nullptr, st);
      launch_linear_bwd_x(dte, Wt->lin2_w, N->k_t1, 1, B, 4 * nf, 4 * nf, dt1, st);
      launch_linear_bwd_w(dt1, 4 * nf, N->k_four, 0, B, 4 * nf, 2 * nf, N->pg + Wt->lin1_go, N->pg + Wt->lin1_go + 8LL * nf * nf, nullptr, st);
    }
  }
  float* dfx = N->tmp((long long)B * T * Kp);
  if (!N->dry() && gx) {
    gemm_b(N, N->spec->g, 2 * Fb, (long long)Tp * 2 * Fb, false, N->W->basisF, Kp, 0, true, dfx, Kp, (long long)T * Kp, T, Kp, 2 * Fb, nullptr, nullptr,
           1.f, 0, B);
    launch_unpad_adj(dfx, Kp, T, nfft, hop, B, L, N->pad, 1.f, N->k_cin, N->k_cskip ? cot : nullptr, N->k_cskip, gx, st);
  }
  N->arena.off = mark;
}

static int check_sites(const Net* N, int L) {
  const int Tp = (1 + L / N->cfg.hop + 15) / 16 * 16;
  for (const AttnW& a : N->W->sites) {
    const long long T = (long long)(Tp >> a.level) * (N->Fb >> a.level);
    if (!flash_attn_supported(a.C) && T > ATTN_MATRIX_MAX_T) {
      set_error("attention at level " + std::to_string(a.level) + ": C = " + std::to_string(a.C) + " has no flash kernel (C in {32, 64, 128, 256}) and T = " +
                std::to_string(T) + " tokens exceeds the materialised form's limit of " + std::to_string(ATTN_MATRIX_MAX_T));
      return BUDDY_ERR_ARG;
    }
  }
  return BUDDY_OK;
}

int net_reserve(Net* N, int B, int L, int with_vjp, long long* bytes) {
  if (int rc = check_sites(N, L)) return rc;
  OptScope scope(&N->opt);
  Arena saved = N->arena;
  N->w4_need = 0;
  N->arena = Arena(); N->arena.dry = true;
  static const float dry_scalars[1] = {0.f};
  N->vdry = 0;
  run_forward(N, nullptr, nullptr, dry_scalars, dry_scalars, dry_scalars, nullptr, B, L, with_vjp != 0);
  const int conv_fwd = N->vdry;
  N->pg_run = with_vjp >= 2;
  if (with_vjp) run_vjp(N, nullptr, nullptr);
  N->pg_run = false;
  const int conv_slots = std::max(conv_fwd, N->vdry - conv_fwd) + 1;
  const size_t need = N->arena.peak + (1 << 20);
  N->arena = saved;
  N->pool.clear(); N->tape.clear(); N->taps.clear(); N->have_tape = false;
  if (bytes) *bytes = (long long)need + (long long)N->w4_need * 4;
  if (N->w4_cap < N->w4_need) {
    if (N->w4_scratch) (void)hipFree(N->w4_scratch);
    N->w4_scratch = nullptr; N->w4_cap = 0;
// ... 74 lines not shown
```

### buddy_amd/csrc/ops.hip

```cpp
#include "common.h"
#include <cstdlib>

namespace buddy {
namespace {

__device__ __forceinline__ float silu_f(float z) { return z / (1.f + expf(-z)); }
__device__ __forceinline__ float dsilu_f(float z) {
  const float s = 1.f / (1.f + expf(-z));
  return s * (1.f + z * (1.f - s));
}
__device__ __forceinline__ const float* src_ptr(const Src2& x, long long pix, int c) {
  return (x.p1 != nullptr && c >= x.C0) ? x.p1 + pix * x.ld1 + (c - x.C0) : x.p0 + pix * x.ld0 + c;
}
__device__ __forceinline__ float4 ld4(const float* p) { return *reinterpret_cast<const float4*>(p); }
typedef float f32x4s __attribute__((ext_vector_type(4)));
__device__ __forceinline__ float4 ld4s(const float* p) { const f32x4s v = __builtin_nontemporal_load(reinterpret_cast<const f32x4s*>(p)); return make_float4(v.x, v.y, v.z, v.w); }
__device__ __forceinline__ void st4(float* p, float4 v) { *reinterpret_cast<float4*>(p) = v; }
__device__ __forceinline__ float4 add4(float4 a, float4 b) { return make_float4(a.x + b.x, a.y + b.y, a.z + b.z, a.w + b.w); }
__device__ __forceinline__ float4 mul4(float4 a, float s) { return make_float4(a.x * s, a.y * s, a.z * s, a.w * s); }

__device__ __forceinline__ float4 da_eff(const float* da, int mode, int b, int h, int w, int H, int W, int C, int c) {
  if (mode == 0) return ld4(da + (((long long)b * H + h) * W + w) * C + c);
  if (mode == 1) {
    const int H2 = H >> 1, W2 = W >> 1;
    return mul4(ld4(da + (((long long)b * H2 + (h >> 1)) * W2 + (w >> 1)) * C + c), 0.25f);
  }
  const int H2 = H << 1, W2 = W << 1;
  const float* q = da + (((long long)b * H2 + 2 * h) * W2 + 2 * w) * C + c;
  return add4(add4(ld4(q), ld4(q + C)), add4(ld4(q + (long long)W2 * C), ld4(q + (long long)W2 * C + C)));
}

struct RedArgs {
  Src2 x; int B, H, W, C, G; int chunks, ppc;
  const float* stats; const float* gamma; const float* beta; const float* da; int mode; int silu;
  double* partial;
};

template <int KIND>
__global__ __launch_bounds__(256) void chan_reduce_kernel(const RedArgs a) {
  __shared__ double red[256 * 8];
  const int q = a.C >> 2, pl = 256 / q;
  const int tid = threadIdx.x, quad = tid % q, lp = tid / q;
  const int b = blockIdx.y, chunk = blockIdx.x;
  const int HW = a.H * a.W;
  const int p0 = chunk * a.ppc, p1 = min(HW, p0 + a.ppc);
  double s[4] = {0, 0, 0, 0}, t[4] = {0, 0, 0, 0};
  if (lp < pl) {
    const int c = quad * 4;
    float mean = 0.f, rstd = 0.f; float4 gm = make_float4(0, 0, 0, 0), bt = gm;
    if (KIND == 1) {
      const int g = c / (a.C / a.G);
      mean = a.stats[((long long)b * a.G + g) * 2]; rstd = a.stats[((long long)b * a.G + g) * 2 + 1];
      gm = ld4(a.gamma + c); bt = ld4(a.beta + c);
    }
    if (KIND == 1 && a.mode == 0) {
      const float gv[4] = {gm.x, gm.y, gm.z, gm.w}, bv[4] = {bt.x, bt.y, bt.z, bt.w};
      const bool second = a.x.p1 != nullptr && c >= a.x.C0;
      const float* xs = (second ? a.x.p1 + (c - a.x.C0) : a.x.p0 + c) + (long long)b * HW * (second ? a.x.ld1 : a.x.ld0);
      const long long ldx = second ? a.x.ld1 : a.x.ld0;
      const float* ds = a.da + (long long)b * HW * a.C + c;
      int p = p0 + lp;
      while (p < p1) {
        float fs[4] = {0.f, 0.f, 0.f, 0.f}, ft[4] = {0.f, 0.f, 0.f, 0.f};
        auto one = [&](float4 v, float4 d) {
          const float xv[4] = {v.x, v.y, v.z, v.w}, dv[4] = {d.x, d.y, d.z, d.w};
#pragma unroll
          for (int j = 0; j < 4; ++j) {
            const float xh = (xv[j] - mean) * rstd;
            const float z = xh * gv[j] + bv[j];
            const float dxh = dv[j] * (a.silu ? dsilu_f(z) : 1.f) * gv[j];
            fs[j] += dxh; ft[j] += dxh * xh;
          }
        };
        int n = 0;
        for (; n < 8 && p + pl < p1; n += 2, p += 2 * pl) {
          const float4 v0 = ld4s(xs + (long long)p * ldx), v1 = ld4s(xs + (long long)(p + pl) * ldx);
          const float4 d0 = ld4s(ds + (long long)p * a.C), d1 = ld4s(ds + (long long)(p + pl) * a.C);
          one(v0, d0); one(v1, d1);
        }
        if (n < 8 && p < p1) { one(ld4s(xs + (long long)p * ldx), ld4s(ds + (long long)p * a.C)); p += pl; }
#pragma unroll
        for (int j = 0; j < 4; ++j) { s[j] += (double)fs[j]; t[j] += (double)ft[j]; }
      }
    } else
    for (int p = p0 + lp; p < p1; p += pl) {
      const float4 v = ld4s(src_ptr(a.x, (long long)b * HW + p, c));
      const float xv[4] = {v.x, v.y, v.z, v.w};
      if (KIND == 0) {
#pragma unroll
        for (int j = 0; j < 4; ++j) { s[j] += (double)xv[j]; t[j] += (double)xv[j] * (double)xv[j]; }
      } else {
        const int h = p / a.W, w = p - h * a.W;
        const float4 d = da_eff(a.da, a.mode, b, h, w, a.H, a.W, a.C, c);
        const float dv[4] = {d.x, d.y, d.z, d.w};
        const float gv[4] = {gm.x, gm.y, gm.z, gm.w}, bv[4] = {bt.x, bt.y, bt.z, bt.w};
#pragma unroll
        for (int j = 0; j < 4; ++j) {
          const float xh = (xv[j] - mean) * rstd;
          const float z = xh * gv[j] + bv[j];
          const float dxh = dv[j] * (a.silu ? dsilu_f(z) : 1.f) * gv[j];
          s[j] += (double)dxh; t[j] += (double)dxh * (double)xh;
        }
// ... 4 lines not shown
  for (int j = 0; j < 4; ++j) { red[tid * 8 + j] = s[j]; red[tid * 8 + 4 + j] = t[j]; }
  __syncthreads();
  if (tid < q) {
    double r[8] = {0, 0, 0, 0, 0, 0, 0, 0};
    for (int l = 0; l < pl; ++l)
#pragma unroll
      for (int j = 0; j < 8; ++j) r[j] += red[(l * q + tid) * 8 + j];
    double* o = a.partial + (((long long)b * a.chunks + chunk) * a.C + tid * 4) * 2;
#pragma unroll
    for (int j = 0; j < 4; ++j) { o[j * 2] = r[j]; o[j * 2 + 1] = r[4 + j]; }
  }
}

template <int KIND>
__global__ __launch_bounds__(256) void group_finalize_kernel(const double* partial, float* out, int C, int G, int chunks, int HW, float eps) {
  __shared__ double red[8];
  const int g = blockIdx.x, b = blockIdx.y, tid = threadIdx.x, lane = tid & 63, w = tid >> 6;
  const int cpg = C / G;
  double s = 0, t = 0;
  for (int i = tid; i < chunks * cpg; i += 256) {
    const int ch = i / cpg, c = g * cpg + (i - ch * cpg);
    const double2 v = *reinterpret_cast<const double2*>(partial + (((long long)b * chunks + ch) * C + c) * 2);
    s += v.x; t += v.y;
  }
#pragma unroll
  for (int off = 32; off > 0; off >>= 1) { s += __shfl_down(s, off, 64); t += __shfl_down(t, off, 64); }
  if (lane == 0) { red[2 * w] = s; red[2 * w + 1] = t; }
  __syncthreads();
  if (tid == 0) {
    s = ((red[0] + red[2]) + red[4]) + red[6]; t = ((red[1] + red[3]) + red[5]) + red[7];
    const double n = (double)cpg * (double)HW;
    float* o = out + ((long long)b * G + g) * 2;
    if (KIND == 0) {
      const double mean = s / n;
      double var = t / n - mean * mean;
      if (var < 0) var = 0;
      o[0] = (float)mean; o[1] = (float)(1.0 / sqrt(var + (double)eps));
    } else {
      o[0] = (float)(s / n); o[1] = (float)(t / n);
    }
  }
}

__global__ __launch_bounds__(256) void csum_collapse_kernel(const double* __restrict__ partial, int chunks, int C, double* __restrict__ csum) {
  __shared__ double red[256 * 2];
  const int tid = threadIdx.x, cl = tid & 15, sl = tid >> 4, b = blockIdx.y;
  const int c = blockIdx.x * 16 + cl;
  double s = 0, t = 0;
  if (c < C)
    for (int ch = sl; ch < chunks; ch += 16) {
      const double2 v = *reinterpret_cast<const double2*>(partial + (((long long)b * chunks + ch) * C + c) * 2);
      s += v.x; t += v.y;
    }
  red[tid * 2] = s; red[tid * 2 + 1] = t;
  __syncthreads();
  if (sl == 0 && c < C) {
    for (int l = 1; l < 16; ++l) { s += red[(l * 16 + cl) * 2]; t += red[(l * 16 + cl) * 2 + 1]; }
    csum[((long long)b * C + c) * 2] = s; csum[((long long)b * C + c) * 2 + 1] = t;
  }
}

__global__ __launch_bounds__(64) void group_finalize_csum_kernel(const double* __restrict__ c0, const double* __restrict__ c1, int C0, int C, int G,
                                                                 int HW, float eps, float* __restrict__ out) {
  const int g = blockIdx.x, b = blockIdx.y, lane = threadIdx.x;
  const int cpg = C / G;
  double s = 0, t = 0;
  for (int i = lane; i < cpg; i += 64) {
    const int c = g * cpg + i;
    const double* p = (c1 != nullptr && c >= C0) ? c1 + ((long long)b * (C - C0) + (c - C0)) * 2 : c0 + ((long long)b * C0 + c) * 2;
    s += p[0]; t += p[1];
  }
#pragma unroll
  for (int off = 32; off > 0; off >>= 1) { s += __shfl_down(s, off, 64); t += __shfl_down(t, off, 64); }
  if (lane == 0) {
    const double n = (double)cpg * (double)HW;
    float* o = out + ((long long)b * G + g) * 2;
    const double mean = s / n;
    double var = t / n - mean * mean;
    if (var < 0) var = 0;
    o[0] = (float)mean; o[1] = (float)(1.0 / sqrt(var + (double)eps));
  }
}

__global__ __launch_bounds__(256) void gn_apply_kernel(Src2 x, const float* stats, const float* gamma, const float* beta, int B, int H,
                                                       int W, int C, int G, int mode, int silu, float* out, float* pooled_raw) {
  const int q = C >> 2, cpg = C / G;
  const int Ho = (mode == 1) ? H >> 1 : H, Wo = (mode == 1) ? W >> 1 : W;
  const long long total = (long long)B * Ho * Wo * q;
  for (long long idx = (long long)blockIdx.x * 256 + threadIdx.x; idx < total; idx += (long long)gridDim.x * 256) {
    const int quad = (int)(idx % q); long long pix = idx / q;
    const int w = (int)(pix % Wo); pix /= Wo; const int h = (int)(pix % Ho); const int b = (int)(pix / Ho);
    const int c = quad * 4, g = c / cpg;
    const float mean = stats[((long long)b * G + g) * 2], rstd = stats[((long long)b * G + g) * 2 + 1];
    const float4 gm = ld4(gamma + c), bt = ld4(beta + c);
    auto act = [&](float4 v) {
      float4 z = make_float4((v.x - mean) * rstd * gm.x + bt.x, (v.y - mean) * rstd * gm.y + bt.y,
                             (v.z - mean) * rstd * gm.z + bt.z, (v.w - mean) * rstd * gm.w + bt.w);
      if (silu) z = make_float4(silu_f(z.x), silu_f(z.y), silu_f(z.z), silu_f(z.w));
      return z;
    };
    if (mode == 0) {
      const long long p = ((long long)b * H + h) * W + w;
      st4(out + p * C + c, act(ld4(src_ptr(x, p, c))));
    } else if (mode == 1) {
      const long long p = ((long long)b * H + 2 * h) * W + 2 * w;
      const float4 v0 = ld4(src_ptr(x, p, c)), v1 = ld4(src_ptr(x, p + 1, c)), v2 = ld4(src_ptr(x, p + W, c)), v3 = ld4(src_ptr(x, p + W + 1, c));
      const long long po = ((long long)b * Ho + h) * Wo + w;
      st4(out + po * C + c, mul4(add4(add4(act(v0), act(v1)), add4(act(v2), act(v3))), 0.25f));
      if (pooled_raw) st4(pooled_raw + po * C + c, mul4(add4(add4(v0, v1), add4(v2, v3)), 0.25f));
    } else {
      const long long p = ((long long)b * H + h) * W + w;
      const float4 a = act(ld4(src_ptr(x, p, c)));
      const int W2 = W << 1;
      float* o = out + ((((long long)b * (H << 1)) + 2 * h) * W2 + 2 * w) * C + c;
      st4(o, a); st4(o + C, a); st4(o + (long long)W2 * C, a); st4(o + (long long)W2 * C + C, a);
    }
  }
}

__global__ __launch_bounds__(256) void gn_bwd_apply_kernel(Src2 x, const float* stats, const float* gamma, const float* beta, const float* da,
                                                           int B, int H, int W, int C, int G, int mode, int silu, const float* extra,
                                                           int extra_mode, float extra_scale, const float* red, Dst2 dx) {
  const int q = C >> 2, cpg = C / G;
  const long long total = (long long)B * H * W * q;
  for (long long idx = (long long)blockIdx.x * 256 + threadIdx.x; idx < total; idx += (long long)gridDim.x * 256) {
    const int quad = (int)(idx % q); long long pix = idx / q;
    const long long p = pix;
    const int w = (int)(pix % W); pix /= W; const int h = (int)(pix % H); const int b = (int)(pix / H);
    const int c = quad * 4, g = c / cpg;
    const float mean = stats[((long long)b * G + g) * 2], rstd = stats[((long long)b * G + g) * 2 + 1];
    const float m1 = red[((long long)b * G + g) * 2], m2 = red[((long long)b * G + g) * 2 + 1];
    const float4 gm = ld4(gamma + c), bt = ld4(beta + c);
    const float4 v = ld4s(src_ptr(x, p, c));
    const float4 d = da_eff(da, mode, b, h, w, H, W, C, c);
    const float xv[4] = {v.x, v.y, v.z, v.w}, dv[4] = {d.x, d.y, d.z, d.w};
    const float gv[4] = {gm.x, gm.y, gm.z, gm.w}, bv[4] = {bt.x, bt.y, bt.z, bt.w};
    float r[4];
#pragma unroll
    for (int j = 0; j < 4; ++j) {
      const float xh = (xv[j] - mean) * rstd;
      const float z = xh * gv[j] + bv[j];
      const float dxh = dv[j] * (silu ? dsilu_f(z) : 1.f) * gv[j];
      r[j] = rstd * (dxh - m1 - xh * m2);
    }
    if (extra_mode == 1) {
      const float4 e = ld4(extra + p * C + c);
      r[0] += extra_scale * e.x; r[1] += extra_scale * e.y; r[2] += extra_scale * e.z; r[3] += extra_scale * e.w;
    } else if (extra_mode == 2) {
      const float4 e = ld4(extra + ((((long long)b * (H >> 1)) + (h >> 1)) * (W >> 1) + (w >> 1)) * C + c);
      const float s = 0.25f * extra_scale;
      r[0] += s * e.x; r[1] += s * e.y; r[2] += s * e.z; r[3] += s * e.w;
    }
    float* o; int acc;
    if (dx.p1 != nullptr && c >= dx.C0) { o = dx.p1 + p * dx.ld1 + (c - dx.C0); acc = dx.acc1; }
    else { o = dx.p0 + p * dx.ld0 + c; acc = dx.acc0; }
    float4 res = make_float4(r[0], r[1], r[2], r[3]);
    if (acc) res = add4(res, ld4(o));
    st4(o, res);
  }
}

struct GnFast { int HW, C, G, q, pl, ppc; };
__global__ __launch_bounds__(256) void gn_apply_m0_kernel(Src2 x, const float* stats, const float* gamma, const float* beta, GnFast a, int silu, float* out) {
  const int tid = threadIdx.x, quad = tid % a.q, lp = tid / a.q, b = blockIdx.y;
  const int c = quad * 4, g = c / (a.C / a.G);
  const float mean = stats[((long long)b * a.G + g) * 2], rstd = stats[((long long)b * a.G + g) * 2 + 1];
  const float4 gm = ld4(gamma + c), bt = ld4(beta + c);
  const bool second = x.p1 != nullptr && c >= x.C0;
  const float* src = second ? x.p1 + (c - x.C0) : x.p0 + c;
  const long long ld = second ? x.ld1 : x.ld0;
  src += (long long)b * a.HW * ld;
  float* dst = out + (long long)b * a.HW * a.C + c;
  const int p0 = blockIdx.x * a.ppc, p1 = min(a.HW, p0 + a.ppc);
  auto act = [&](float4 v) {
    float4 z = make_float4((v.x - mean) * rstd * gm.x + bt.x, (v.y - mean) * rstd * gm.y + bt.y,
                           (v.z - mean) * rstd * gm.z + bt.z, (v.w - mean) * rstd * gm.w + bt.w);
    if (silu) z = make_float4(silu_f(z.x), silu_f(z.y), silu_f(z.z), silu_f(z.w));
    return z;
  };
  int p = p0 + lp;
  for (; p + 3 * a.pl < p1; p += 4 * a.pl) {
    float4 v[4];
#pragma unroll
    for (int j = 0; j < 4; ++j) v[j] = ld4s(src + (long long)(p + j * a.pl) * ld);
#pragma unroll
    for (int j = 0; j < 4; ++j) st4(dst + (long long)(p + j * a.pl) * a.C, act(v[j]));
  }
  for (; p < p1; p += a.pl) st4(dst + (long long)p * a.C, act(ld4s(src + (long long)p * ld)));
}

template <bool EX, bool ACC>
__global__ __launch_bounds__(256) void gn_bwd_apply_m0_kernel(Src2 x, const float* stats, const float* gamma, const float* beta, const float* da,
                                                              GnFast a, int silu, const float* extra, float extra_scale, const float* red, Dst2 dx) {
  const int tid = threadIdx.x, quad = tid % a.q, lp = tid / a.q, b = blockIdx.y;
  const int c = quad * 4, g = c / (a.C / a.G);
  const float mean = stats[((long long)b * a.G + g) * 2], rstd = stats[((long long)b * a.G + g) * 2 + 1];
  const float m1 = red[((long long)b * a.G + g) * 2], m2 = red[((long long)b * a.G + g) * 2 + 1];
  const float4 gm = ld4(gamma + c), bt = ld4(beta + c);
  const float gv[4] = {gm.x, gm.y, gm.z, gm.w}, bv[4] = {bt.x, bt.y, bt.z, bt.w};
  const bool second = x.p1 != nullptr && c >= x.C0;
  const float* src = second ? x.p1 + (c - x.C0) : x.p0 + c;
  const long long ld = second ? x.ld1 : x.ld0;
  src += (long long)b * a.HW * ld;
  const float* dap = da + (long long)b * a.HW * a.C + c;
  const float* ex = EX ? extra + (long long)b * a.HW * a.C + c : nullptr;
  const bool dsecond = dx.p1 != nullptr && c >= dx.C0;
  float* o = dsecond ? dx.p1 + (c - dx.C0) : dx.p0 + c;
  const long long ldo = dsecond ? dx.ld1 : dx.ld0;
  const bool acc = ACC && (dsecond ? dx.acc1 : dx.acc0) != 0;
  o += (long long)b * a.HW * ldo;
  const int p0 = blockIdx.x * a.ppc, p1 = min(a.HW, p0 + a.ppc);
  auto one = [&](float4 v, float4 d, float4 e, float4 prev) {
    const float xv[4] = {v.x, v.y, v.z, v.w}, dv[4] = {d.x, d.y, d.z, d.w}, ev[4] = {e.x, e.y, e.z, e.w}, pv[4] = {prev.x, prev.y, prev.z, prev.w};
    float r[4];
#pragma unroll
    for (int j = 0; j < 4; ++j) {
      const float xh = (xv[j] - mean) * rstd;
      const float z = xh * gv[j] + bv[j];
      const float dxh = dv[j] * (silu ? dsilu_f(z) : 1.f) * gv[j];
      r[j] = rstd * (dxh - m1 - xh * m2);
      if (EX) r[j] += extra_scale * ev[j];
      if (ACC) r[j] = acc ? r[j] + pv[j] : r[j];
    }
    return make_float4(r[0], r[1], r[2], r[3]);
  };
  const float4 z4 = make_float4(0.f, 0.f, 0.f, 0.f);
  int p = p0 + lp;
  __builtin_amdgcn_s_waitcnt(0x0F70);
  for (; p + a.pl < p1; p += 2 * a.pl) {
    float4 v[2], d[2], e[2], pr[2];
#pragma unroll
    for (int j = 0; j < 2; ++j) {
      const long long pp = p + j * a.pl;
      v[j] = ld4s(src + pp * ld); d[j] = ld4s(dap + pp * a.C); e[j] = EX ? ld4s(ex + pp * a.C) : z4; pr[j] = ACC ? ld4(o + pp * ldo) : z4;
    }
#pragma unroll
    for (int j = 0; j < 2; ++j) st4(o + (long long)(p + j * a.pl) * ldo, one(v[j], d[j], e[j], pr[j]));
  }
  for (; p < p1; p += a.pl)
    st4(o + (long long)p * ldo, one(ld4s(src + (long long)p * ld), ld4s(dap + (long long)p * a.C), EX ? ld4s(ex + (long long)p * a.C) : z4, ACC ? ld4(o + (long long)p * ldo) : z4));
}

__global__ __launch_bounds__(256) void axpy_kernel(float* dst, const float* src, float alpha, long long n4, int accumulate) {
  for (long long i = (long long)blockIdx.x * 256 + threadIdx.x; i < n4; i += (long long)gridDim.x * 256) {
    float4 v = mul4(ld4(src + i * 4), alpha);
    if (accumulate) v = add4(v, ld4(dst + i * 4));
    st4(dst + i * 4, v);
  }
}

__global__ __launch_bounds__(256) void pool2_kernel(const float* src, float* dst, int B, int H, int W, int C, float scale, int accumulate) {
  const int q = C >> 2, Ho = H >> 1, Wo = W >> 1;
  const long long total = (long long)B * Ho * Wo * q;
  for (long long idx = (long long)blockIdx.x * 256 + threadIdx.x; idx < total; idx += (long long)gridDim.x * 256) {
    const int quad = (int)(idx % q); long long pix = idx / q;
    const int w = (int)(pix % Wo); pix /= Wo; const int h = (int)(pix % Ho); const int b = (int)(pix / Ho);
    const float* s = src + ((((long long)b * H) + 2 * h) * W + 2 * w) * C + quad * 4;
    float4 v = mul4(add4(add4(ld4(s), ld4(s + C)), add4(ld4(s + (long long)W * C), ld4(s + (long long)W * C + C))), scale);
    float* o = dst + idx * 4;
    if (accumulate) v = add4(v, ld4(o));
    st4(o, v);
  }
// ... 145 lines not shown
                                                            float* y, int ldY, int B, int H, int W, int Cout, int accumulate) {
  const int q = Cout >> 2;
  const int quad = threadIdx.x % q, c = quad * 4;
  float2 wr[TAPS][4];
#pragma unroll
  for (int t = 0; t < TAPS; ++t)
#pragma unroll
    for (int j = 0; j < 4; ++j) wr[t][j] = *reinterpret_cast<const float2*>(w + ((long long)(c + j) * TAPS + t) * 2);
  float b4[4];
#pragma unroll
  for (int j = 0; j < 4; ++j) b4[j] = bias ? bias[c + j] : 0.f;
  const int ppb = 256 / q;
  const long long npix = (long long)B * H * W;
  for (long long p = (long long)blockIdx.x * ppb + threadIdx.x / q; p < npix; p += (long long)gridDim.x * ppb) {
    const int wq = (int)(p % W); const int h = (int)((p / W) % H);
    float acc[4] = {b4[0], b4[1], b4[2], b4[3]};
#pragma unroll
    for (int t = 0; t < TAPS; ++t) {
      const int dy = (TAPS == 9) ? t / 3 - 1 : 0, dx = (TAPS == 9) ? t % 3 - 1 : 0;
      if ((unsigned)(h + dy) >= (unsigned)H || (unsigned)(wq + dx) >= (unsigned)W) continue;
      const float2 v = reinterpret_cast<const float2*>(x)[p + dy * W + dx];
#pragma unroll
      for (int j = 0; j < 4; ++j) acc[j] += wr[t][j].x * v.x + wr[t][j].y * v.y;
    }
    float4 r = make_float4(acc[0], acc[1], acc[2], acc[3]);
    if (add) r = add4(r, ld4(add + p * add_ld + c));
    float* o = y + p * ldY + c;
    if (accumulate) r = add4(r, ld4(o));
    st4(o, r);
  }
}

__global__ __launch_bounds__(256) void conv_c2in_reg4_kernel(const float* x, const float* w, const float* bias, const float* add, int add_ld,
                                                             float* y, int ldY, int B, int H, int W, int Cout, int accumulate) {
  const int q = Cout >> 2;
  const int quad = threadIdx.x % q, c = quad * 4;
  float2 wr[9][4];
#pragma unroll
  for (int t = 0; t < 9; ++t)
#pragma unroll
    for (int j = 0; j < 4; ++j) wr[t][j] = *reinterpret_cast<const float2*>(w + ((long long)(c + j) * 9 + t) * 2);
  float b4[4];
#pragma unroll
  for (int j = 0; j < 4; ++j) b4[j] = bias ? bias[c + j] : 0.f;
  const int ppb = 256 / q;
  const int W4 = W >> 2;
  const long long ngrp = (long long)B * H * W4;
  for (long long gi = (long long)blockIdx.x * ppb + threadIdx.x / q; gi < ngrp; gi += (long long)gridDim.x * ppb) {
    const int wg = (int)(gi % W4) * 4; const int h = (int)((gi / W4) % H);
    const long long p0 = (gi / W4) * W + wg;
    float2 in[3][6];
#pragma unroll
    for (int r = 0; r < 3; ++r) {
      const bool rok = (unsigned)(h + r - 1) < (unsigned)H;
#pragma unroll
      for (int cc = 0; cc < 6; ++cc) {
        const int wx = wg + cc - 1;
        in[r][cc] = (rok && (unsigned)wx < (unsigned)W) ? reinterpret_cast<const float2*>(x)[p0 + (long long)(r - 1) * W + cc - 1] : make_float2(0.f, 0.f);
      }
    }
    float4 ad[4], pr[4];
#pragma unroll
    for (int u = 0; u < 4; ++u) {
      ad[u] = add ? ld4(add + (p0 + u) * add_ld + c) : make_float4(0.f, 0.f, 0.f, 0.f);
      pr[u] = accumulate ? ld4(y + (p0 + u) * ldY + c) : make_float4(0.f, 0.f, 0.f, 0.f);
    }
#pragma unroll
    for (int u = 0; u < 4; ++u) {
      float acc[4] = {b4[0], b4[1], b4[2], b4[3]};
#pragma unroll
      for (int t = 0; t < 9; ++t) {
        const float2 v = in[t / 3][u + t % 3];
#pragma unroll
        for (int j = 0; j < 4; ++j) acc[j] += wr[t][j].x * v.x + wr[t][j].y * v.y;
      }
      float4 r = make_float4(acc[0], acc[1], acc[2], acc[3]);
      if (add) r = add4(r, ad[u]);
      if (accumulate) r = add4(r, pr[u]);
      st4(y + (p0 + u) * ldY + c, r);
    }
  }
}

template <int TAPS>
__global__ __launch_bounds__(256) void conv_c2out_kernel(const float* x, int ldX, const float* w, const float* bias, const float* up_add,
                                                         float* y, int B, int H, int W, int Cin, int accumulate) {
  const int lpp = Cin >> 2, ppb = 256 / lpp;
  const int tid = threadIdx.x, sub = tid % lpp, slot = tid / lpp;
  const int c = sub * 4;
  float wr[TAPS][8];
#pragma unroll
  for (int t = 0; t < TAPS; ++t)
#pragma unroll
    for (int j = 0; j < 8; ++j) wr[t][j] = w[((long long)t * Cin + c) * 2 + j];
  const long long npix = (long long)B * H * W;
  const long long ngroups = (npix + ppb - 1) / ppb;
  for (long long gidx = blockIdx.x; gidx < ngroups; gidx += gridDim.x) {
    const long long p = gidx * ppb + slot;
    float s0 = 0.f, s1 = 0.f;
    int b = 0, h = 0, wq = 0;
    if (p < npix) {
      long long pix = p;
      wq = (int)(pix % W); pix /= W; h = (int)(pix % H); b = (int)(pix / H);
#pragma unroll
      for (int t = 0; t < TAPS; ++t) {
        const int dy = (TAPS == 9) ? t / 3 - 1 : 0, dx = (TAPS == 9) ? t % 3 - 1 : 0;
        if ((unsigned)(h + dy) >= (unsigned)H || (unsigned)(wq + dx) >= (unsigned)W) continue;
        const float4 v = ld4(x + (p + dy * W + dx) * ldX + c);
        s0 += v.x * wr[t][0] + v.y * wr[t][2] + v.z * wr[t][4] + v.w * wr[t][6];
        s1 += v.x * wr[t][1] + v.y * wr[t][3] + v.z * wr[t][5] + v.w * wr[t][7];
      }
    }
    for (int off = lpp >> 1; off > 0; off >>= 1) { s0 += __shfl_xor(s0, off, 64); s1 += __shfl_xor(s1, off, 64); }
    if (sub == 0 && p < npix) {
      if (bias) { s0 += bias[0]; s1 += bias[1]; }
      if (up_add) {
        const float2 u = reinterpret_cast<const float2*>(up_add)[(((long long)b * (H >> 1)) + (h >> 1)) * (W >> 1) + (wq >> 1)];
        s0 += u.x; s1 += u.y;
      }
      float2* o = reinterpret_cast<float2*>(y) + p;
      if (accumulate) { s0 += o->x; s1 += o->y; }
      *o = make_float2(s0, s1);
    }
  }
}

constexpr int C2O_TH = 8, C2O_TW = 32, C2O_CK = 32, C2O_PITCH = C2O_CK + 4;
__global__ __launch_bounds__(256) void conv_c2out_tiled_kernel(const float* __restrict__ x, int ldX, const float* __restrict__ w, const float* bias,
                                                               const float* up_add, float* y, int B, int H, int W, int Cin, int accumulate) {
  __shared__ __attribute__((aligned(16))) float tile[(C2O_TH + 2) * (C2O_TW + 2) * C2O_PITCH];
  __shared__ __attribute__((aligned(16))) float wsh[9 * C2O_CK * 2];
  const int tid = threadIdx.x;
  const int tx = tid & (C2O_TW - 1), ty = tid / C2O_TW;
  const int nbx = (W + C2O_TW - 1) / C2O_TW, nby = (H + C2O_TH - 1) / C2O_TH;
  int blk = blockIdx.x;
  const int bxi = blk % nbx; blk /= nbx;
  const int byi = blk % nby; const int b = blk / nby;
  const int h0 = byi * C2O_TH, w0 = bxi * C2O_TW;
  const int h = h0 + ty, wq = w0 + tx;
  float s0 = 0.f, s1 = 0.f;
  constexpr int NPX = (C2O_TH + 2) * (C2O_TW + 2);
  constexpr int NLD = (NPX * (C2O_CK / 4) + 255) / 256;
  for (int c0 = 0; c0 < Cin; c0 += C2O_CK) {
    float4 v[NLD];
#pragma unroll
    for (int i = 0; i < NLD; ++i) {
      const int e = tid + 256 * i;
      const int px = e >> 3, c4 = (e & 7) * 4;
      const int hr = px / (C2O_TW + 2), wc = px - hr * (C2O_TW + 2);
      const int gh = h0 - 1 + hr, gw = w0 - 1 + wc;
      v[i] = make_float4(0.f, 0.f, 0.f, 0.f);
      if (e < NPX * (C2O_CK / 4) && (unsigned)gh < (unsigned)H && (unsigned)gw < (unsigned)W) v[i] = ld4(x + (((long long)b * H + gh) * W + gw) * ldX + c0 + c4);
    }
    float wv[3];
#pragma unroll
    for (int i = 0; i < 3; ++i) { const int e = tid + 256 * i; wv[i] = e < 9 * C2O_CK * 2 ? w[((long long)(e / (C2O_CK * 2)) * Cin + c0) * 2 + e % (C2O_CK * 2)] : 0.f; }
#pragma unroll
    for (int i = 0; i < NLD; ++i) {
      const int e = tid + 256 * i;
      if (e < NPX * (C2O_CK / 4)) *reinterpret_cast<float4*>(tile + (e >> 3) * C2O_PITCH + (e & 7) * 4) = v[i];
    }
#pragma unroll
    for (int i = 0; i < 3; ++i) { const int e = tid + 256 * i; if (e < 9 * C2O_CK * 2) wsh[e] = wv[i]; }
    __syncthreads();
#pragma unroll
    for (int t = 0; t < 9; ++t) {
      const float* src = tile + ((ty + t / 3) * (C2O_TW + 2) + tx + t % 3) * C2O_PITCH;
      const float* wt = wsh + t * C2O_CK * 2;
#pragma unroll
      for (int c4 = 0; c4 < C2O_CK; c4 += 4) {
        const float4 vv = *reinterpret_cast<const float4*>(src + c4);
        const float4 wa = *reinterpret_cast<const float4*>(wt + c4 * 2), wb = *reinterpret_cast<const float4*>(wt + c4 * 2 + 4);
        s0 += vv.x * wa.x + vv.y * wa.z + vv.z * wb.x + vv.w * wb.z;
        s1 += vv.x * wa.y + vv.y * wa.w + vv.z * wb.y + vv.w * wb.w;
      }
    }
    __syncthreads();
  }
  if (h < H && wq < W) {
    const long long p = ((long long)b * H + h) * W + wq;
    if (bias) { s0 += bias[0]; s1 += bias[1]; }
    if (up_add) {
      const float2 u = reinterpret_cast<const float2*>(up_add)[(((long long)b * (H >> 1)) + (h >> 1)) * (W >> 1) + (wq >> 1)];
      s0 += u.x; s1 += u.y;
    }
    float2* o = reinterpret_cast<float2*>(y) + p;
    if (accumulate) { s0 += o->x; s1 += o->y; }
    *o = make_float2(s0, s1);
  }
}

__global__ __launch_bounds__(256, 3) void conv_c2out_strip_kernel(const float* __restrict__ x, int ldX, const float* __restrict__ w, const float* bias,
                                                               const float* up_add, float* y, int B, int H, int W, int Cin, int accumulate) {
  __shared__ __attribute__((aligned(16))) float tile[(C2O_TH + 2) * (C2O_TW + 2) * C2O_PITCH];
  __shared__ __attribute__((aligned(16))) float wsh[9 * C2O_CK * 2];
  const int tid = threadIdx.x;
  const int q = tid & 7, strip = tid >> 3, ry = strip >> 2, sx = (strip & 3) * 8;
  const int nbx = (W + C2O_TW - 1) / C2O_TW, nby = (H + C2O_TH - 1) / C2O_TH;
  int blk = blockIdx.x;
  const int bxi = blk % nbx; blk /= nbx;
  const int byi = blk % nby; const int b = blk / nby;
  const int h0 = byi * C2O_TH, w0 = bxi * C2O_TW;
  float s[8][2];
#pragma unroll
  for (int i = 0; i < 8; ++i) { s[i][0] = 0.f; s[i][1] = 0.f; }
  constexpr int NPX = (C2O_TH + 2) * (C2O_TW + 2);
  constexpr int NLD = (NPX * (C2O_CK / 4) + 255) / 256;
  for (int c0 = 0; c0 < Cin; c0 += C2O_CK) {
    float4 v[NLD];
#pragma unroll
    for (int i = 0; i < NLD; ++i) {
      const int e = tid + 256 * i;
      const int px = e >> 3, c4 = (e & 7) * 4;
      const int hr = px / (C2O_TW + 2), wc = px - hr * (C2O_TW + 2);
      const int gh = h0 - 1 + hr, gw = w0 - 1 + wc;
      v[i] = make_float4(0.f, 0.f, 0.f, 0.f);
      if (e < NPX * (C2O_CK / 4) && (unsigned)gh < (unsigned)H && (unsigned)gw < (unsigned)W) v[i] = ld4(x + (((long long)b * H + gh) * W + gw) * ldX + c0 + c4);
    }
    float wv[3];
#pragma unroll
    for (int i = 0; i < 3; ++i) { const int e = tid + 256 * i; wv[i] = e < 9 * C2O_CK * 2 ? w[((long long)(e / (C2O_CK * 2)) * Cin + c0) * 2 + e % (C2O_CK * 2)] : 0.f; }
#pragma unroll
    for (int i = 0; i < NLD; ++i) {
      const int e = tid + 256 * i;
      if (e < NPX * (C2O_CK / 4)) *reinterpret_cast<float4*>(tile + (e >> 3) * C2O_PITCH + (e & 7) * 4) = v[i];
    }
#pragma unroll
    for (int i = 0; i < 3; ++i) { const int e = tid + 256 * i; if (e < 9 * C2O_CK * 2) wsh[e] = wv[i]; }
    __syncthreads();
#pragma unroll 1
    for (int r = 0; r < 3; ++r) {
      float4 wa[3], wb[3];
#pragma unroll
      for (int dx = 0; dx < 3; ++dx) {
        wa[dx] = *reinterpret_cast<const float4*>(wsh + (r * 3 + dx) * C2O_CK * 2 + q * 8);
        wb[dx] = *reinterpret_cast<const float4*>(wsh + (r * 3 + dx) * C2O_CK * 2 + q * 8 + 4);
      }
      const float* row = tile + ((ry + r) * (C2O_TW + 2) + sx) * C2O_PITCH + q * 4;
#pragma unroll
      for (int j = 0; j < 10; ++j) {
        const float4 vv = *reinterpret_cast<const float4*>(row + j * C2O_PITCH);
#pragma unroll
        for (int dx = 0; dx < 3; ++dx) {
          const int px = j - dx;
          if (px >= 0 && px < 8) {
            s[px][0] += vv.x * wa[dx].x + vv.y * wa[dx].z + vv.z * wb[dx].x + vv.w * wb[dx].z;
            s[px][1] += vv.x * wa[dx].y + vv.y * wa[dx].w + vv.z * wb[dx].y + vv.w * wb[dx].w;
          }
        }
      }
      __builtin_amdgcn_sched_barrier(0);
    }
    __syncthreads();
  }
#pragma unroll
  for (int o = 1; o < 8; o <<= 1)
#pragma unroll
    for (int i = 0; i < 8; ++i) { s[i][0] += __shfl_xor(s[i][0], o); s[i][1] += __shfl_xor(s[i][1], o); }
  float s0 = s[0][0], s1 = s[0][1];
#pragma unroll
  for (int i = 1; i < 8; ++i) if (q == i) { s0 = s[i][0]; s1 = s[i][1]; }
  const int h = h0 + ry, wq = w0 + sx + q;
  if (h < H && wq < W) {
    const long long p = ((long long)b * H + h) * W + wq;
    if (bias) { s0 += bias[0]; s1 += bias[1]; }
    if (up_add) {
      const float2 u = reinterpret_cast<const float2*>(up_add)[(((long long)b * (H >> 1)) + (h >> 1)) * (W >> 1) + (wq >> 1)];
      s0 += u.x; s1 += u.y;
    }
    float2* o = reinterpret_cast<float2*>(y) + p;
    if (accumulate) { s0 += o->x; s1 += o->y; }
    *o = make_float2(s0, s1);
  }
}

__global__ __launch_bounds__(256) void reflect_pad_kernel(const float* x, float* xp, int B, int L, int pad, int Lp, float scale, const float* scale_b) {
  const long long total = (long long)B * Lp;
  for (long long idx = (long long)blockIdx.x * 256 + threadIdx.x; idx < total; idx += (long long)gridDim.x * 256) {
    const int b = (int)(idx / Lp), j = (int)(idx % Lp);
    float v = 0.f;
    if (j < L + 2 * pad) {
      int i = j - pad;
      if (i < 0) i = -i;
      if (i >= L) i = 2 * (L - 1) - i;
      v = x[(long long)b * L + i] * scale * (scale_b ? scale_b[b] : 1.f);
    }
    xp[idx] = v;
  }
}

__global__ __launch_bounds__(256) void ola_kernel(const float* frames, int ldF, int Tp, int n_fft, int hop, const float* inv_env, float* y, int B,
                                                  int L, int pad, const float* xin, const float* cskip_b, const float* cout_b) {
  const long long total = (long long)B * L;
  for (long long idx = (long long)blockIdx.x * 256 + threadIdx.x; idx < total; idx += (long long)gridDim.x * 256) {
    const int b = (int)(idx / L), s = (int)(idx % L);
    const int j = s + pad;
    int t0 = (j - n_fft + hop) / hop; if (t0 < 0) t0 = 0;
    int t1 = j / hop; if (t1 > Tp - 1) t1 = Tp - 1;
    float acc = 0.f;
    for (int t = t0; t <= t1; ++t) {
// ... 66 lines not shown
    float acc = 0.f;
#pragma unroll
    for (int dy = 0; dy < 2; ++dy) {
      const int yy = y0 + dy;
      if ((unsigned)yy >= (unsigned)H) continue;
      const float wy = dy ? 1.f - wy0 : wy0;
      float row = 0.f;
#pragma unroll
      for (int dx = 0; dx < 2; ++dx) {
        const int xx = x0 + dx;
        if ((unsigned)xx >= (unsigned)W) continue;
        row += (dx ? 1.f - wx0 : wx0) * x[(((long long)b * H + yy) * W + xx) * C + c];
      }
      acc += wy * row;
    }
    acc *= scale;
    y[idx] = accumulate ? y[idx] + acc : acc;
  }
}
__global__ __launch_bounds__(256) void fir_down2_kernel(const float* __restrict__ x, float* __restrict__ y, int B, int H, int W, int C, float scale, int accumulate) {
  const int Ho = H >> 1, Wo = W >> 1;
  const long long total = (long long)B * Ho * Wo * C;
  for (long long idx = (long long)blockIdx.x * 256 + threadIdx.x; idx < total; idx += (long long)gridDim.x * 256) {
    const int c = (int)(idx % C); long long r = idx / C;
    const int ox = (int)(r % Wo); r /= Wo;
    const int oy = (int)(r % Ho); const int b = (int)(r / Ho);
    const float wt[4] = {0.125f, 0.375f, 0.375f, 0.125f};
    float acc = 0.f;
#pragma unroll
    for (int dy = 0; dy < 4; ++dy) {
      const int yy = 2 * oy - 1 + dy;
      if ((unsigned)yy >= (unsigned)H) continue;
      float row = 0.f;
#pragma unroll
      for (int dx = 0; dx < 4; ++dx) {
        const int xx = 2 * ox - 1 + dx;
        if ((unsigned)xx >= (unsigned)W) continue;
        row += wt[dx] * x[(((long long)b * H + yy) * W + xx) * C + c];
      }
      acc += wt[dy] * row;
    }
    acc *= scale;
    y[idx] = accumulate ? y[idx] + acc : acc;
  }
}
}

int gn_num_chunks(int HW) {
  int c = HW / 64;
  if (c < 1) c = 1;
  if (c > 256) c = 256;
  return c;
}

static GnFast gn_m0_geo(int HW, int C, int G) {
  GnFast a; a.HW = HW; a.C = C; a.G = G; a.q = C / 4; a.pl = 256 / a.q; if (a.pl < 1) a.pl = 1;
  constexpr int trips = 4;
  int chunks = HW / (a.pl * trips); if (chunks < 1) chunks = 1; if (chunks > 32768) chunks = 32768;
  a.ppc = (HW + chunks - 1) / chunks;
  a.ppc = (a.ppc + a.pl - 1) / a.pl * a.pl;
  return a;
}

static RedArgs make_red(Src2 x, int B, int H, int W, int C, int G, double* partial) {
  RedArgs a{};
  a.x = x; a.B = B; a.H = H; a.W = W; a.C = C; a.G = G;
  a.chunks = gn_num_chunks(H * W);
  a.ppc = (H * W + a.chunks - 1) / a.chunks;
  a.partial = partial;
  return a;
}

void launch_gn_stats(Src2 x, int B, int HW, int C, int G, float eps, double* partial, float* stats, hipStream_t st) {
  RedArgs a = make_red(x, B, 1, HW, C, G, partial);
  prof_hbm_begin(4.0 * B * HW * C, st);
  hipLaunchKernelGGL(chan_reduce_kernel<0>, dim3(a.chunks, B), dim3(256), 0, st, a);
  hipLaunchKernelGGL(group_finalize_kernel<0>, dim3(G, B), dim3(256), 0, st, (const double*)partial, stats, C, G, a.chunks, HW, eps);
  prof_hbm_end(st);
}

void launch_csum_collapse(const double* partial, int chunks, int B, int C, double* csum, hipStream_t st) {
  hipLaunchKernelGGL(csum_collapse_kernel, dim3((C + 15) / 16, B), dim3(256), 0, st, partial, chunks, C, csum);
}
void launch_chan_sums(const float* x, int B, int HW, int C, double* partial, double* csum, hipStream_t st) {
  Src2 s; s.p0 = x; s.p1 = nullptr; s.C0 = C; s.ld0 = C; s.ld1 = 0;
  RedArgs a = make_red(s, B, 1, HW, C, 1, partial);
  prof_hbm_begin(4.0 * B * HW * C, st);
  hipLaunchKernelGGL(chan_reduce_kernel<0>, dim3(a.chunks, B), dim3(256), 0, st, a);
  launch_csum_collapse(partial, a.chunks, B, C, csum, st);
  prof_hbm_end(st);
}
void launch_gn_stats_partial(const double* partial, int chunks, int B, int HW, int C, int G, float eps, float* stats, hipStream_t st) {
  hipLaunchKernelGGL(group_finalize_kernel<0>, dim3(G, B), dim3(256), 0, st, partial, stats, C, G, chunks, HW, eps);
}
void launch_gn_stats_csum(const double* csum0, const double* csum1, int C0, int B, int HW, int C, int G, float eps, float* stats, hipStream_t st) {
  hipLaunchKernelGGL(group_finalize_csum_kernel, dim3(G, B), dim3(64), 0, st, csum0, csum1, csum1 ? C0 : C, C, G, HW, eps, stats);
}

void launch_gn_apply(Src2 x, const float* stats, const float* gamma, const float* beta, int B, int H, int W, int C, int G, int mode, int silu,
                     float* out, float* pooled_raw, hipStream_t st) {
  const long long total = (long long)B * (mode == 1 ? (H / 2) * (W / 2) : H * W) * (C / 4);
  const double n_in = (double)B * H * W * C, n_out = mode == 1 ? n_in / 4 : (mode == 2 ? n_in * 4 : n_in);
  prof_hbm_begin(4.0 * (n_in + n_out + (pooled_raw ? n_out : 0.0)), st);
  if (mode == 0 && C % 4 == 0 && C / 4 <= 256) {
    GnFast a = gn_m0_geo(H * W, C, G);
    hipLaunchKernelGGL(gn_apply_m0_kernel, dim3((H * W + a.ppc - 1) / a.ppc, B), dim3(a.q * a.pl), 0, st, x, stats, gamma, beta, a, silu, out);
  } else {
    hipLaunchKernelGGL(gn_apply_kernel, dim3(grid_for(total)), dim3(256), 0, st, x, stats, gamma, beta, B, H, W, C, G, mode, silu, out, pooled_raw);
  }
  prof_hbm_end(st);
}

void launch_gn_bwd_sums(Src2 x, const float* stats, const float* gamma, const float* beta, const float* da, int B, int H, int W, int C, int G, int mode,
                        int silu, double* partial, float* red, hipStream_t st, int ready_chunks) {
  if (ready_chunks > 0) {
    hipLaunchKernelGGL(group_finalize_kernel<1>, dim3(G, B), dim3(256), 0, st, (const double*)partial, red, C, G, ready_chunks, H * W, 0.f);
    return;
  }
  RedArgs a = make_red(x, B, H, W, C, G, partial);
  a.stats = stats; a.gamma = gamma; a.beta = beta; a.da = da; a.mode = mode; a.silu = silu;
  const double n_in = (double)B * H * W * C, n_da = mode == 1 ? n_in / 4 : (mode == 2 ? n_in * 4 : n_in);
  prof_hbm_begin(4.0 * (n_in + n_da), st);
  hipLaunchKernelGGL(chan_reduce_kernel<1>, dim3(a.chunks, B), dim3(256), 0, st, a);
  hipLaunchKernelGGL(group_finalize_kernel<1>, dim3(G, B), dim3(256), 0, st, (const double*)partial, red, C, G, a.chunks, H * W, 0.f);
  prof_hbm_end(st);
}
void launch_gn_bwd_apply(Src2 x, const float* stats, const float* gamma, const float* beta, const float* da, int B, int H, int W, int C, int G, int mode,
                         int silu, const float* extra, int extra_mode, float extra_scale, const float* red, Dst2 dx, hipStream_t st) {
  const double n_in = (double)B * H * W * C, n_da = mode == 1 ? n_in / 4 : (mode == 2 ? n_in * 4 : n_in);
  prof_hbm_begin(4.0 * (n_in + n_da + n_in + (extra_mode ? (extra_mode == 2 ? n_in / 4 : n_in) : 0.0)), st);
  const long long total = (long long)B * H * W * (C / 4);
  if (mode == 0 && extra_mode != 2 && C % 4 == 0 && C / 4 <= 256) {
    GnFast g = gn_m0_geo(H * W, C, G);
    const bool ex = extra_mode == 1 && extra != nullptr, acc = dx.acc0 != 0 || (dx.p1 != nullptr && dx.acc1 != 0);
    const dim3 grid((H * W + g.ppc - 1) / g.ppc, B), block(g.q * g.pl);
#define GN_M0(E, A) hipLaunchKernelGGL((gn_bwd_apply_m0_kernel<E, A>), grid, block, 0, st, x, stats, gamma, beta, da, g, silu, ex ? extra : nullptr, extra_scale, red, dx)
    if (ex && acc) GN_M0(true, true); else if (ex) GN_M0(true, false); else if (acc) GN_M0(false, true); else GN_M0(false, false);
#undef GN_M0
  } else
  hipLaunchKernelGGL(gn_bwd_apply_kernel, dim3(grid_for(total)), dim3(256), 0, st, x, stats, gamma, beta, da, B, H, W, C, G, mode, silu, extra,
                     extra_mode, extra_scale, red, dx);
  prof_hbm_end(st);
}
void launch_gn_bwd(Src2 x, const float* stats, const float* gamma, const float* beta, const float* da, int B, int H, int W, int C, int G, int mode,
                   int silu, const float* extra, int extra_mode, float extra_scale, double* partial, float* red, Dst2 dx, hipStream_t st,
                   int ready_chunks) {
  launch_gn_bwd_sums(x, stats, gamma, beta, da, B, H, W, C, G, mode, silu, partial, red, st, ready_chunks);
  launch_gn_bwd_apply(x, stats, gamma, beta, da, B, H, W, C, G, mode, silu, extra, extra_mode, extra_scale, red, dx, st);
}

void launch_axpy(float* dst, const float* src, float alpha, long long n, int accumulate, hipStream_t st) {
  hipLaunchKernelGGL(axpy_kernel, dim3(grid_for(n / 4)), dim3(256), 0, st, dst, src, alpha, n / 4, accumulate);
}

void launch_fir_up2(const float* x, float* y, int B, int H, int W, int C, float scale, int accumulate, hipStream_t st) {
  hipLaunchKernelGGL(fir_up2_kernel, dim3(grid_for((long long)B * 4 * H * W * C)), dim3(256), 0, st, x, y, B, H, W, C, scale, accumulate);
}
void launch_fir_down2(const float* x, float* y, int B, int H, int W, int C, float scale, int accumulate, hipStream_t st) {
  hipLaunchKernelGGL(fir_down2_kernel, dim3(grid_for((long long)B * (H / 2) * (W / 2) * C)), dim3(256), 0, st, x, y, B, H, W, C, scale, accumulate);
}

void launch_pool2(const float* src, float* dst, int B, int H, int W, int C, float scale, int accumulate, hipStream_t st) {
  if (C == 2) {
    hipLaunchKernelGGL(pool2_c2_kernel, dim3(grid_for((long long)B * (H / 2) * (W / 2))), dim3(256), 0, st, src, dst, B, H, W, scale, accumulate);
  } else {
    hipLaunchKernelGGL(pool2_kernel, dim3(grid_for((long long)B * (H / 2) * (W / 2) * (C / 4))), dim3(256), 0, st, src, dst, B, H, W, C, scale, accumulate);
  }
}

void launch_up2_acc(const float* src, float* dst, int B, int Hs, int Ws, int C, float scale, int accumulate, hipStream_t st) {
  hipLaunchKernelGGL(up2_acc_kernel, dim3(grid_for((long long)B * Hs * Ws * 4 * (C / 2))), dim3(256), 0, st, src, dst, B, Hs, Ws, C, scale, accumulate);
}

void launch_transpose_sq(const float* src, float* dst, int batch, int n, hipStream_t st) {
  hipLaunchKernelGGL(transpose_sq_kernel, dim3(n / 32, n / 32, batch), dim3(256), 0, st, src, dst, n);
}
void launch_softmax_rows(float* S, int rows, int cols, hipStream_t st) {
  hipLaunchKernelGGL(softmax_rows_kernel, dim3(cdiv(rows, 4)), dim3(256), 0, st, S, rows, cols);
}

void launch_softmax_bwd_rows(const float* P, float* dP, int rows, int cols, hipStream_t st) {
  hipLaunchKernelGGL(softmax_bwd_rows_kernel, dim3(cdiv(rows, 4)), dim3(256), 0, st, P, dP, rows, cols);
}

void launch_linear(const float* x, const float* W, const float* b, float* y, int B, int K, int N, int silu_in, hipStream_t st) {
  hipLaunchKernelGGL(linear_kernel, dim3(cdiv((long long)B * N, 4)), dim3(256), 0, st, x, W, b, y, B, K, N, silu_in);
}

void launch_fourier(const float* cnoise, const float* Wf, float* out, int B, int nf, hipStream_t st) {
  hipLaunchKernelGGL(fourier_kernel, dim3(cdiv(B * nf, 256)), dim3(256), 0, st, cnoise, Wf, out, B, nf);
}

void launch_mix2(const float* x, const float* w, const float* b, float* y, long long npix, int transpose, int accumulate, hipStream_t st) {
  hipLaunchKernelGGL(mix2_kernel, dim3(grid_for(npix)), dim3(256), 0, st, x, w, b, y, npix, transpose, accumulate);
}

void launch_conv_c2in(const float* x, const float* w, const float* bias, const float* add, int add_ld, float* y, int ldY, int B, int H, int W,
                      int Cout, int taps, int accumulate, hipStream_t st) {
  const long long total = (long long)B * H * W * (Cout / 4);
  if (Cout % 4 == 0 && 256 % (Cout / 4) == 0) {
    const int ppb = 256 / (Cout / 4);
    long long g = ((long long)B * H * W + ppb - 1) / ppb;
    if (g > 256 * 8) g = 256 * 8;
    if (taps == 9 && W % 4 == 0) {
      long long g4 = ((long long)B * H * (W / 4) + ppb - 1) / ppb;
      if (g4 > 256 * 16) g4 = 256 * 16;
      hipLaunchKernelGGL(conv_c2in_reg4_kernel, dim3((int)g4), dim3(256), 0, st, x, w, bias, add, add_ld, y, ldY, B, H, W, Cout, accumulate);
    } else if (taps == 9)
      hipLaunchKernelGGL(conv_c2in_reg_kernel<9>, dim3((int)g), dim3(256), 0, st, x, w, bias, add, add_ld, y, ldY, B, H, W, Cout, accumulate);
    else
      hipLaunchKernelGGL(conv_c2in_reg_kernel<1>, dim3((int)g), dim3(256), 0, st, x, w, bias, add, add_ld, y, ldY, B, H, W, Cout, accumulate);
    return;
  }
  if (taps == 9)
    hipLaunchKernelGGL(conv_c2in_kernel<9>, dim3(grid_for(total)), dim3(256), 0, st, x, w, bias, add, add_ld, y, ldY, B, H, W, Cout, accumulate);
  else
    hipLaunchKernelGGL(conv_c2in_kernel<1>, dim3(grid_for(total)), dim3(256), 0, st, x, w, bias, add, add_ld, y, ldY, B, H, W, Cout, accumulate);
}

void launch_conv_c2out(const float* x, int ldX, const float* w, const float* bias, const float* up_add, float* y, int B, int H, int W, int Cin,
                       int taps, int accumulate, hipStream_t st) {
  const int ppb = 256 / (Cin / 4);
  long long groups = ((long long)B * H * W + ppb - 1) / ppb;
  int grid = (int)(groups < 256 * 8 ? groups : 256 * 8);
  const bool tiled = cur_opt().c2out_tiled != 0;
  if (taps == 9 && cur_opt().c2out_tiled == 2 && Cin % C2O_CK == 0 && ldX % 4 == 0) {
    const int blocks = B * ((H + C2O_TH - 1) / C2O_TH) * ((W + C2O_TW - 1) / C2O_TW);
    hipLaunchKernelGGL(conv_c2out_strip_kernel, dim3(blocks), dim3(256), 0, st, x, ldX, w, bias, up_add, y, B, H, W, Cin, accumulate);
  } else if (taps == 9 && tiled && Cin % C2O_CK == 0 && ldX % 4 == 0) {
    const int blocks = B * ((H + C2O_TH - 1) / C2O_TH) * ((W + C2O_TW - 1) / C2O_TW);
    hipLaunchKernelGGL(conv_c2out_tiled_kernel, dim3(blocks), dim3(256), 0, st, x, ldX, w, bias, up_add, y, B, H, W, Cin, accumulate);
  } else if (taps == 9)
    hipLaunchKernelGGL(conv_c2out_kernel<9>, dim3(grid), dim3(256), 0, st, x, ldX, w, bias, up_add, y, B, H, W, Cin, accumulate);
  else
    hipLaunchKernelGGL(conv_c2out_kernel<1>, dim3(grid), dim3(256), 0, st, x, ldX, w, bias, up_add, y, B, H, W, Cin, accumulate);
}

void launch_reflect_pad(const float* x, float* xp, int B, int L, int pad, int Lp, float scale, const float* scale_b, hipStream_t st) {
  hipLaunchKernelGGL(reflect_pad_kernel, dim3(grid_for((long long)B * Lp)), dim3(256), 0, st, x, xp, B, L, pad, Lp, scale, scale_b);
}

void launch_ola(const float* frames, int ldF, int Tp, int n_fft, int hop, const float* inv_env, float* y, int B, int L, int pad, const float* xin,
                const float* cskip_b, const float* cout_b, hipStream_t st) {
  hipLaunchKernelGGL(ola_kernel, dim3(grid_for((long long)B * L)), dim3(256), 0, st, frames, ldF, Tp, n_fft, hop, inv_env, y, B, L, pad, xin, cskip_b, cout_b);
}

void launch_ola_adj(const float* g, int B, int L, int pad, int Tp, int n_fft, int hop, const float* inv_env, const float* cout_b, float* frames,
                    int ldF, hipStream_t st) {
  hipLaunchKernelGGL(ola_adj_kernel, dim3(grid_for((long long)B * Tp * ldF)), dim3(256), 0, st, g, B, L, pad, Tp, n_fft, hop, inv_env, cout_b, frames, ldF);
}

void launch_unpad_adj(const float* dframes, int ldF, int T, int n_fft, int hop, int B, int L, int pad, float scale, const float* scale_b,
                      const float* g_out, const float* cskip_b, float* dx, hipStream_t st) {
  hipLaunchKernelGGL(unpad_adj_kernel, dim3(grid_for((long long)B * L)), dim3(256), 0, st, dframes, ldF, T, n_fft, hop, B, L, pad, scale, scale_b, g_out, cskip_b, dx);
}

}
```

### include/buddy_hip.h

```cpp
#ifndef BUDDY_HIP_H
#define BUDDY_HIP_H
#ifdef __cplusplus
extern "C" {
#endif

const char* buddy_last_error(void);
int buddy_version(void);


int buddy_ncsnpp_param_count(int nf, const int* ch_mult, int n_levels, int num_res_blocks, long long* count);

int buddy_ncsnpp_create(const float* host_params, long long n_params, int nf, const int* ch_mult, int n_levels,
                        int num_res_blocks, int n_fft, int hop, void** handle);
int buddy_ncsnpp_param_count_attn(int nf, const int* ch_mult, int n_levels, int num_res_blocks, int attn_mask, long long* count);
int buddy_ncsnpp_create_attn(const float* host_params, long long n_params, int nf, const int* ch_mult, int n_levels,
                             int num_res_blocks, int n_fft, int hop, int attn_mask, void** handle);
int buddy_ncsnpp_destroy(void* handle);
int buddy_ncsnpp_replica(void* handle, void** replica);
int buddy_ncsnpp_weight_bytes(void* handle, long long* params, long long* packed, long long* lazy, int* lazy_forms);
int buddy_conv3_weight_prep(const float* w_oihw, int O, int I, int dgrad, int kind, float* out, void* stream);

int buddy_ncsnpp_reserve(void* handle, int B, int L, int with_vjp, long long* bytes);

int buddy_ncsnpp_forward(void* handle, const float* x, const float* cnoise, const float* cin, const float* cskip,
// ... 18 lines not shown

int buddy_prof_enable(int level);
int buddy_prof_collect(double* ms , double* flops , long long* launches , double* bytes ,
                       double* executed_flops );
int buddy_prof_collect_hbm(double* ms, double* bytes, long long* launches);
int buddy_prof_collect_wino4(double* ms , double* gemm_flops, double* bytes_in, double* bytes_out, double* bytes_gemm, long long* launches);

int buddy_mfma_ubench(const float* seed, float* out, int blocks, int iters, unsigned long long* clk, void* stream);
int buddy_mfma_ubench_bf16(const float* seed, float* out, int blocks, int iters, unsigned long long* clk, void* stream);

int buddy_hbm_ubench(const void* src, void* dst, long long bytes, int mode, int nt, int blocks, void* stream);

int buddy_gemm(const float* A, int ldA, int transA, const float* Bt, int ldB, int transB, float* C, int ldC, int M, int N,
               int K, float alpha, const float* bias_n, int accumulate, int batch, long long strideA, long long strideB,
               long long strideC, void* stream);
int buddy_gemm_winograd_domain(const float* V, const float* U, float* M, int tiles, int Cout, int Cin, int positions, void* stream);
long long buddy_wgemm_packed_bytes(int positions, int Cout, int Cin);
int buddy_wgemm_pack_weights(const float* U, void* U3, int positions, int Cout, int Cin, void* stream);
int buddy_gemm_winograd_domain_bf16x3(const float* V, const void* U3, float* M, int tiles, int Cout, int Cin, int positions, void* stream);
long long buddy_wgemm_f16x2_packed_bytes(int positions, int Cout, int Cin);
int buddy_wgemm_f16x2_pack_weights(const float* U, void* U2, int positions, int Cout, int Cin, void* stream);
int buddy_gemm_winograd_domain_f16x2(const float* V, const void* U2, float* M, int tiles, int Cout, int Cin, int positions, const unsigned* vmax,
                                     int tiles_per_utt, void* stream);
long long buddy_wgemm_f16_packed_bytes(int positions, int Cout, int Cin);
int buddy_wgemm_f16_pack_weights(const float* U, void* U1, int positions, int Cout, int Cin, void* stream);
int buddy_gemm_winograd_domain_f16(const void* V16, const signed char* vexp, const void* U1, float* M, int tiles, int Cout, int Cin, int positions, void* stream);
int buddy_abs_max_bits(const float* x, int groups, int segments, long long seg_len, unsigned* out, void* stream);
int buddy_gemm_bf16x3(const float* A0, int ldA0, const float* A1, int ldA1, int C0, const void* W3, float* C, int ldC, long long M, int N, int K,
                      const float* bias_n, float alpha, int accumulate, void* stream);
int buddy_gemm_bf16x3_gn_bwd(const float* A, int ldA, const void* W3, const float* x0, const float* x1, int C0, const float* da, const float* stats,
                             const float* gamma, const float* beta, int G, int silu, float alpha, float* dx0, float* dx1, int acc0, int acc1,
                             double* stat_scratch, float* red, int B, int HW, int N, int K, void* stream);
int buddy_gemm_f16x2(const float* A0, int ldA0, const float* A1, int ldA1, int C0, const void* W2, float* C, int ldC, long long M, int N, int K,
                     const float* bias_n, float alpha, int accumulate, void* stream);
int buddy_gemm_f16x2_gn_bwd(const float* A, int ldA, const void* W2, const float* x0, const float* x1, int C0, const float* da, const float* stats,
                            const float* gamma, const float* beta, int G, int silu, float alpha, float* dx0, float* dx1, int acc0, int acc1,
                            double* stat_scratch, float* red, int B, int HW, int N, int K, void* stream);
int buddy_conv3x3(const float* x, const float* wt, const float* bias, float* y, int B, int H, int W, int Cin, int Cout,
                  void* stream);
int buddy_winograd_transform_weights(const float* wt_host, int Cout, int Cin, float* U_host);
int buddy_conv3x3_winograd(const float* x, const float* U, const float* bias, float* y, int B, int H, int W, int Cin, int Cout,
                           void* stream);
int buddy_winograd4_transform_weights(const float* wt_host, int Cout, int Cin, float* U4_host);
int buddy_conv3x3_winograd4(const float* x, const float* U4, const float* bias, float* y, float* scratch, int B, int H, int W, int Cin, int Cout,
                            void* stream);
int buddy_winograd6_transform_weights(const float* wt_host, int Cout, int Cin, float* U6_host);
int buddy_conv3x3_winograd6(const float* x, const float* U6, const float* bias, float* y, float* scratch, int B, int H, int W, int Cin, int Cout,
                            void* stream);
int buddy_conv3x3_winograd6_f16(const float* x, const void* U1, const float* bias, float* y, float* scratch, int B, int H, int W, int Cin, int Cout,
                                void* stream);
int buddy_gn_conv3x3_winograd6_f16(const float* x0, const float* x1, int C0, const float* gamma, const float* beta, int G, int silu, const void* U1,
                                   const float* bias, float* y, float* scratch, float* stats, double* stat_scratch, double* csum, int B, int H, int W,
                                   int Cin, int Cout, void* stream);
int buddy_gnbwd_conv3x3_winograd6_f16(const float* x, const float* gamma, const float* beta, const float* stats, const float* da, int G, int silu,
                                      const void* U1, float* y, float* scratch, double* stat_scratch, float* red, int B, int H, int W, int C, int Cout,
                                      void* stream);
int buddy_gn_upconv3x3_winograd6_f16(const float* x, const float* gamma, const float* beta, int G, int silu, const void* U1up, const float* bias, float* y,
                                     float* scratch, float* stats, double* stat_scratch, double* csum, int B, int H, int W, int Cin, int Cout, void* stream);
int buddy_gnbwd_upconv3x3_winograd6_f16(const float* h, const float* gamma, const float* beta, const float* stats, const float* da, int G, int silu,
                                        const void* U1upT, float* y, float* scratch, double* stat_scratch, float* red, int B, int H, int W, int C,
                                        int Cout, void* stream);
int buddy_gn_conv3x3_winograd4(const float* x0, const float* x1, int C0, const float* gamma, const float* beta, int G, int silu, const float* U4,
                               const float* bias, float* y, float* scratch, float* stats, double* stat_scratch, double* csum, int B, int H, int W,
                               int Cin, int Cout, void* stream);
int buddy_gn_conv3x3_winograd6(const float* x0, const float* x1, int C0, const float* gamma, const float* beta, int G, int silu, const float* U6,
                               const float* bias, float* y, float* scratch, float* stats, double* stat_scratch, double* csum, int B, int H, int W,
                               int Cin, int Cout, void* stream);
int buddy_conv3x3_winograd6_gn_bwd_sums(const float* g, const float* U6, float* da, float* scratch, const float* x0, const float* x1, int C0,
                                        const float* stats, const float* gamma, const float* beta, int G, int silu, double* stat_scratch,
                                        double* chsum, int B, int H, int W, int Cin, int Cout, void* stream);
int buddy_gnbwd_conv3x3_winograd6(const float* x, const float* gamma, const float* beta, const float* stats, const float* da, int G, int silu,
                                  const float* U6, float* y, float* scratch, double* stat_scratch, float* red, int B, int H, int W, int C, int Cout,
                                  void* stream);
int buddy_gn_upconv3x3_winograd6(const float* x, const float* gamma, const float* beta, int G, int silu, const float* U6up, const float* bias, float* y,
                                 float* scratch, float* stats, double* stat_scratch, double* csum, int B, int H, int W, int Cin, int Cout, void* stream);
int buddy_gnbwd_upconv3x3_winograd6(const float* h, const float* gamma, const float* beta, const float* stats, const float* da, int G, int silu,
                                    const float* U6upT, float* y, float* scratch, double* stat_scratch, float* red, int B, int H, int W, int C,
                                    int Cout, void* stream);
int buddy_groupnorm_act(const float* x, const float* gamma, const float* beta, float* y, float* stats, void* scratch, int B,
                        int H, int W, int C, int G, int mode, int silu, void* stream);
int buddy_groupnorm_act_bwd(const float* x, const float* gamma, const float* beta, const float* stats, const float* dy, float* dx,
                            void* scratch, float* red, int B, int H, int W, int C, int G, int mode, int silu, void* stream);

int buddy_fir_resample2(const float* x, float* y, int B, int H, int W, int C, int up, float scale, int accumulate, void* stream);
int buddy_ncsnpp_set_fir(void* handle, int fir);
int buddy_options_check(void);
int buddy_option_validate(const char* key, int value);
int buddy_ncsnpp_set_option(void* handle, const char* key, int value);
int buddy_ncsnpp_get_option(void* handle, const char* key, int* value);
int buddy_ncsnpp_set_attention(void* handle, int mode);
int buddy_ncsnpp_set_gemm(void* handle, int mode);

int buddy_flash_attention_fwd(const float* q, const float* k, const float* v, float* O, float* lse, int B, int T, int C, float scale, int prec, void* stream);
int buddy_flash_attention_bwd(const float* q, const float* k, const float* v, const float* O, const float* dO, const float* lse, float* delta,
                              float* dq, float* dk, float* dv, int B, int T, int C, float scale, int prec, void* stream);
long long buddy_flash_attention16_workspace(int B, int T, int C);
int buddy_flash_attention16_fwd(const float* q, const float* k, const float* v, float* O, float* lse, int B, int T, int C, float scale, int prec,
                                float* ws, void* stream);
int buddy_flash_attention16_bwd(const float* q, const float* k, const float* v, const float* O, const float* dO, const float* lse, float* delta,
                                float* dq, float* dk, float* dv, int B, int T, int C, float scale, int prec, float* ws, void* stream);
int buddy_flash_attention_splits(int B, int T);
long long buddy_flash_attention_workspace(int B, int T, int C, int splits);
int buddy_flash_attention_fwd_split(const float* q, const float* k, const float* v, float* O, float* lse, int B, int T, int C, float scale, int splits,
                                    float* ws, void* stream);
int buddy_flash_attention_bwd_split(const float* q, const float* k, const float* v, const float* O, const float* dO, const float* lse, float* delta,
                                    float* dq, float* dk, float* dv, int B, int T, int C, float scale, int splits, float* ws, void* stream);

int buddy_axpby_rows(const float* x, const float* y, const float* a, const float* c, float* out, int B, int L, void* stream);
int buddy_perturb(const float* x, const float* eps, float scale, float* out, long long n, void* stream);
int buddy_dps_update(const float* x_hat, const float* x_den, const float* lh, const float* lh_scale, const float* den_scale, const float* base,
                     const float* d_prev, float t, float dt, float w_prev, float w_cur, float* out, float* d_out, float* x_den_out, int B, int L, void* stream);
int buddy_row_scale(const float* x, float* out, int B, int L, int mode, float p0, float p1, void* stream);
int buddy_fill_rows4(float* out, int B, float v0, float v1, float v2, float v3, void* stream);
int buddy_row_moments(const float* x, double* out, int B, int L, void* stream);
int buddy_fir(const float* x, const float* h, long long h_stride, float* y, int B, int L, int M, int adjoint, void* stream);

int buddy_wpe(const double* Y, double* X, double* scratch, int rows, int T, int taps, int delay, int iterations, void* stream);
long long buddy_wpe_workspace_bytes(int B, int L);
int buddy_wpe_dereverb(const float* y, float* out, void* workspace, int B, int L, int taps, int delay, int iterations, void* stream);

int buddy_blindop_create(int U, int L, int Nf, int E, int num_knots, const float* knots_hz , int sample_rate, float compression,
                         float min_decay, float max_decay, float w_lo, float w_hi, int clamp_decay, int long_second, void** handle);
int buddy_blindop_destroy(void* handle);
int buddy_blindop_set_params(void* handle, const float* decay, const float* weights, const float* phases, int reset_adam, void* stream);
int buddy_blindop_get_params(void* handle, float* decay, float* weights, float* phases, void* stream);
int buddy_blindop_update_H(void* handle, const float* noise, void* stream);
int buddy_blindop_get_H(void* handle, float* H_out, void* stream);
int buddy_blindop_set_y(void* handle, const float* y , void* stream);
int buddy_blindop_degrade(void* handle, const float* x, float* y, void* stream);
int buddy_blindop_time_rir(void* handle, float* rir , void* stream);
int buddy_blindop_design_filter(void* handle, float* A, void* stream);
int buddy_blindop_apply_stft(void* handle, const float* x, float* X, void* stream);
int buddy_blindop_minphase(void* handle, const float* h, float* out, void* stream);
int buddy_blindop_degrade_vjp(void* handle, const float* x, const float* g_y, float* g_x, float* g_H, void* stream);
int buddy_blindop_time_rir_vjp(void* handle, const float* g_rir , float* g_H, void* stream);
int buddy_blindop_update_H_vjp(void* handle, const float* g_H, float* g_decay, float* g_weights, float* g_phases, void* stream);
int buddy_blindop_stft(void* handle, const float* x, int len, float* X, void* stream);
int buddy_blindop_stft_adjoint(void* handle, const float* G, int len, float* g_x, void* stream);
int buddy_blindop_stft_loss(void* handle, const float* a, const float* b, int len, float weight, float* loss, float* g_a, float* g_b, void* stream);
int buddy_blindop_set_compression(void* handle, float compression_factor);
int buddy_blindop_set_loss_norm(void* handle, int mode);
int buddy_blindop_set_loss(void* handle, int slot, int kind, int freq_weighting, float compression);
int buddy_blindop_set_freq_weights(void* handle, int freq_weighting, const float* w);
int buddy_blindop_lengths(void* handle, int* L, int* L_rir, int* frames, int* frames_rir);
int buddy_blindop_project(void* handle, void* stream);
int buddy_blindop_get_adam(void* handle, float* m_decay, float* v_decay, float* m_weights, float* v_weights, float* m_phases, float* v_phases,
                           int* step , void* stream);
int buddy_blindop_rec_loss_grad(void* handle, const float* x_den, float weight, float* loss, float* g_x, void* stream);
int buddy_blindop_fir_loss_grad(void* handle, const float* x_den, const float* rir, long long rir_stride, int M, float weight, float* loss,
                                float* g_x, void* stream);
int buddy_blindop_param_grads(void* handle, const float* x_den, const float* noise, float t_op, float w_rec, float w_reg, float* g_decay,
                              float* g_weights, float* g_phases, float* losses, void* stream);
int buddy_blindop_optimize(void* handle, const float* x_den, const float* noise, float t_op, int n_iters, float w_rec, float w_reg, float lr,
                           float beta1, float beta2, float weight_decay, void* stream);

#ifdef __cplusplus
}
#endif
#endif
```

Baseline: 143.7.

## Fuse GroupNorm into c2out conv and defer channel-sum collapse into stats finalize

Fuses the GroupNorm+SiLU apply into the output-projection conv's input load, so the normalized activation temporary is no longer written and read back. Defers the per-channel partial-sum collapse after conv epilogues and merges it with the group-stats finalize into one kernel, dropping a launch per GroupNorm. Also replaces three small device memcpys with one gather kernel. Adds pending-state bookkeeping in the net and extra template variants, at the cost of more complexity and the risk of ordering bugs if the pending sum is not settled in time.

```diff
diff --git a/buddy_amd/_lib.py b/buddy_amd/_lib.py
--- a/buddy_amd/_lib.py
+++ b/buddy_amd/_lib.py
@@ -104,6 +104,10 @@
                                       C.c_int, C.c_int, C.c_void_p]),
     "buddy_groupnorm_act_bwd": (C.c_int, [_f32p, _f32p, _f32p, _f32p, _f32p, _f32p, C.c_void_p, _f32p, C.c_int, C.c_int, C.c_int,
                                           C.c_int, C.c_int, C.c_int, C.c_int, C.c_void_p]),
+    "buddy_gn_conv_c2out": (C.c_int, [_f32p, _f32p, _f32p, _f32p, C.c_int, C.c_int, _f32p, _f32p, _f32p, _f32p, _f32p, C.c_int, C.c_int, C.c_int,
+                                      C.c_int, C.c_void_p]),
+    "buddy_gn_stats_from_partials": (C.c_int, [C.c_void_p, C.c_int, C.c_void_p, C.c_void_p, C.c_int, C.c_int, C.c_int, C.c_int, C.c_int, C.c_int,
+                                               _f32p, C.c_void_p]),
     "buddy_fir_resample2": (C.c_int, [_f32p, _f32p, C.c_int, C.c_int, C.c_int, C.c_int, C.c_int, C.c_float, C.c_int, C.c_void_p]),
     "buddy_ncsnpp_set_fir": (C.c_int, [C.c_void_p, C.c_int]),
     "buddy_ncsnpp_set_gemm": (C.c_int, [C.c_void_p, C.c_int]),
diff --git a/buddy_amd/csrc/capi.hip b/buddy_amd/csrc/capi.hip
--- a/buddy_amd/csrc/capi.hip
+++ b/buddy_amd/csrc/capi.hip
@@ -518,6 +518,37 @@
   return finish();
 }
 
+int buddy_gn_conv_c2out(const float* x, const float* gamma, const float* beta, const float* stats, int G, int silu, const float* w, const float* bias,
+                        const float* up_add, float* y, float* act_tmp, int B, int H, int W, int C, void* stream) {
+  if (!x || !gamma || !beta || !stats || !w || !y || B < 1 || H < 1 || W < 1 || G < 1 || C % 4 || C % G || (C / G) % 4 || 256 % (C / 4)) {
+    set_error("bad gn_conv_c2out arguments"); return BUDDY_ERR_ARG;
+  }
+  hipStream_t st = (hipStream_t)stream;
+  if (act_tmp) {
+    Src2 s; s.p0 = x; s.p1 = nullptr; s.C0 = C; s.ld0 = C; s.ld1 = 0;
+    launch_gn_apply(s, stats, gamma, beta, B, H, W, C, G, 0, silu, act_tmp, nullptr, st);
+    launch_conv_c2out(act_tmp, C, w, bias, up_add, y, B, H, W, C, 9, 0, st);
+  } else {
+    const C2oGn gn{stats, gamma, beta, G, silu};
+    launch_conv_c2out(x, C, w, bias, up_add, y, B, H, W, C, 9, 0, st, &gn);
+  }
+  return finish();
+}
+
+int buddy_gn_stats_from_partials(const double* partial, int chunks, double* csum0, const double* csum1, int C0, int B, int HW, int C, int G, int merged,
+                                 float* stats, void* stream) {
+  if (!partial || !csum0 || !stats || chunks < 1 || B < 1 || HW < 1 || G < 1 || C % G || C0 < 1 || C0 > C || (csum1 == nullptr) != (C0 == C)) {
+    set_error("bad gn_stats_from_partials arguments"); return BUDDY_ERR_ARG;
+  }
+  hipStream_t st = (hipStream_t)stream;
+  if (merged) launch_csum_collapse_stats(partial, chunks, csum0, csum1, C0, B, HW, C, G, 1e-6f, stats, st);
+  else {
+    launch_csum_collapse(partial, chunks, B, C0, csum0, st);
+    launch_gn_stats_csum(csum0, csum1, C0, B, HW, C, G, 1e-6f, stats, st);
+  }
+  return finish();
+}
+
 int buddy_options_check(void) { return options_check(); }
 int buddy_option_validate(const char* key, int value) { Options o = default_options(); return option_set(o, key, value); }
 int buddy_ncsnpp_set_option(void* h, const char* key, int value) { if (!h) { set_error("null handle"); return BUDDY_ERR_ARG; } return net_set_option((Net*)h, key, value); }
diff --git a/buddy_amd/csrc/common.h b/buddy_amd/csrc/common.h
--- a/buddy_amd/csrc/common.h
+++ b/buddy_amd/csrc/common.h
@@ -104,15 +104,19 @@
 
 void launch_conv_c2in(const float* x, const float* w , const float* bias, const float* add, int add_ld,
                       float* y, int ldY, int B, int H, int W, int Cout, int taps, int accumulate, hipStream_t st);
+struct C2oGn { const float* stats; const float* gamma; const float* beta; int G; int silu; };
 void launch_conv_c2out(const float* x, int ldX, const float* w , const float* bias, const float* up_add,
-                       float* y, int B, int H, int W, int Cin, int taps, int accumulate, hipStream_t st);
+                       float* y, int B, int H, int W, int Cin, int taps, int accumulate, hipStream_t st, const C2oGn* gn = nullptr);
 
 int  gn_num_chunks(int HW);
 void launch_gn_stats(Src2 x, int B, int HW, int C, int G, float eps, double* partial, float* stats , hipStream_t st);
-void launch_chan_sums(const float* x, int B, int HW, int C, double* partial, double* csum, hipStream_t st);
+int launch_chan_sums(const float* x, int B, int HW, int C, double* partial, double* csum, hipStream_t st);
 void launch_csum_collapse(const double* partial, int chunks, int B, int C, double* csum, hipStream_t st);
 void launch_gn_stats_partial(const double* partial, int chunks, int B, int HW, int C, int G, float eps, float* stats, hipStream_t st);
 void launch_gn_stats_csum(const double* csum0, const double* csum1, int C0, int B, int HW, int C, int G, float eps, float* stats, hipStream_t st);
+void launch_csum_collapse_stats(const double* partial, int chunks, double* csum0, const double* csum1, int C0, int B, int HW, int C, int G, float eps,
+                                float* stats, hipStream_t st);
+void launch_gather3(const float* a, const float* b, const float* c, float* out , int n, hipStream_t st);
 void launch_gn_apply(Src2 x, const float* stats, const float* gamma, const float* beta, int B, int H, int W, int C, int G,
                      int mode, int silu, float* out, float* pooled_raw, hipStream_t st);
 void launch_gn_bwd_sums(Src2 x, const float* stats, const float* gamma, const float* beta, const float* da, int B, int H, int W, int C, int G,
diff --git a/buddy_amd/csrc/net.hip b/buddy_amd/csrc/net.hip
--- a/buddy_amd/csrc/net.hip
+++ b/buddy_amd/csrc/net.hip
@@ -168,6 +168,7 @@
   std::vector<std::function<void()>> tape;
   std::vector<std::pair<int, Tens*>> taps;
   double* partial = nullptr; float* red = nullptr;
+  Tens* pend = nullptr; int pend_chunks = 0;
   bool have_tape = false;
   hipStream_t st = nullptr;
   bool pgrad = false, pg_run = false; float* pg = nullptr; float* dtemb = nullptr; int tape_gen = 0;
@@ -655,6 +656,12 @@
   const int sc = wino6_stat_chunks(p, 1);
   return sc > 0 && (long long)sc * Cout <= 256LL * 1024 && (long long)wino6_stat_chunks(p, 0) * Cin <= 256LL * 1024;
 }
+static void settle_csum(Net* N) {
+  if (N->pend == nullptr) return;
+  Tens* t = N->pend;
+  launch_csum_collapse(N->partial, N->pend_chunks, t->B, t->C, t->csum, N->st);
+  t->has_csum = true; N->pend = nullptr;
+}
 static int conv3(Net* N, const Conv3& c) {
   const float* a = c.a; const int B = c.B, H = c.H, W = c.W, Cin = c.Cin, Cout = c.Cout;
   if (N->prep_failed) return -1;
@@ -675,6 +682,7 @@
     }
     return 0;
   }
+  settle_csum(N);
   if (c.up) {
     IgemmParams p = ig_base();
     p.A0 = a; p.ldA0 = Cin; p.Cin = Cin; p.H = H; p.W = W; p.M = B * H * W; p.N = Cout; p.C = c.out; p.ldC = Cout;
@@ -695,7 +703,7 @@
                  wv->x[x3], c.up, x3, vm);
     igemm_prof_record(pr, 9, 1, N->st, false, xr);
     if (stat && (want_bwd || direct)) return sc;
-    if (stat && stat_out) { launch_csum_collapse(N->partial, sc, B, Cout, stat_out->csum, N->st); stat_out->has_csum = true; }
+    if (stat && stat_out) { N->pend = stat_out; N->pend_chunks = sc; }
     return 0;
   }
   IgemmParams p = ig_base();
@@ -731,7 +739,7 @@
     launch_wino6(p, U6, N->w4_scratch, N->w4_scratch + vf, N->st, gn, stat ? N->partial : nullptr, (stat && want_bwd) ? bwd_gn : nullptr, U6x, 0, xf, vm);
     igemm_prof_record(p, 9, 1, N->st, false, xr);
     if (stat && (want_bwd || direct)) return sc;
-    if (stat && stat_out) { launch_csum_collapse(N->partial, sc, B, Cout, stat_out->csum, N->st); stat_out->has_csum = true; }
+    if (stat && stat_out) { N->pend = stat_out; N->pend_chunks = sc; }
   } else if (w4) {
     const int x4 = xf ? 1 : 0;
     const WVar* wv = conv_weights(N, *c.w, c.dgrad, 4, x4);
@@ -743,7 +751,7 @@
     igemm_prof_record(p, 9, 1, N->st, true, 0.25);
     launch_wino4(p, U4, N->w4_scratch, N->w4_scratch + vf, N->st, gn, stat ? N->partial : nullptr, U4x);
     igemm_prof_record(p, 9, 1, N->st, false, 0.25);
-    if (stat) { launch_csum_collapse(N->partial, sc, B, Cout, stat_out->csum, N->st); stat_out->has_csum = true; }
+    if (stat) { N->pend = stat_out; N->pend_chunks = sc; }
   } else if (use_wino && wino_ok && wino_supported(p)) {
     const WVar* wv = conv_weights(N, *c.w, c.dgrad, 2, 0);
     if (!wv) return -1;
@@ -788,6 +796,17 @@
 static void view_stats(Net* N, const View& x, int HW, int G, float* stats) {
   hipStream_t st = N->st;
   const int B = x.a->B;
+  if (N->pend != nullptr && N->pend == x.a && (x.b == nullptr || x.b->has_csum)) {
+    launch_csum_collapse_stats(N->partial, N->pend_chunks, x.a->csum, x.b ? x.b->csum : nullptr, x.a->C, B, HW, x.C(), G, 1e-6f, stats, st);
+    x.a->has_csum = true; N->pend = nullptr;
+    return;
+  }
+  settle_csum(N);
+  if (!x.a->has_csum && (x.b == nullptr || x.b->has_csum)) {
+    N->pend = x.a; N->pend_chunks = launch_chan_sums(x.a->p, B, HW, x.a->C, N->partial, nullptr, st);
+    view_stats(N, x, HW, G, stats);
+    return;
+  }
   for (Tens* t : {x.a, x.b})
     if (t != nullptr && !t->has_csum) { launch_chan_sums(t->p, B, HW, t->C, N->partial, t->csum, st); t->has_csum = true; }
   launch_gn_stats_csum(x.a->csum, x.b ? x.b->csum : nullptr, x.a->C, B, HW, x.C(), G, 1e-6f, stats, st);
@@ -1194,16 +1213,12 @@
   const int T = 1 + L / hop, Tp = (T + 15) / 16 * 16;
   const int Lp = (L + nfft + 8 + 3) / 4 * 4;
   N->B = B; N->L = L; N->T = T; N->Tp = Tp; N->Lp = Lp;
-  N->pool.clear(); N->tape.clear(); N->taps.clear();
+  N->pool.clear(); N->tape.clear(); N->taps.clear(); N->pend = nullptr;
   N->arena.off = 0;
   N->k_cin = N->k_cskip = N->k_cout = nullptr;
   if (cin_b) {
     float* sc = N->tmp(3 * (long long)B);
-    if (!N->dry()) {
-      (void)hipMemcpyAsync(sc, cin_b, (size_t)B * 4, hipMemcpyDeviceToDevice, st);
-      (void)hipMemcpyAsync(sc + B, cskip_b, (size_t)B * 4, hipMemcpyDeviceToDevice, st);
-      (void)hipMemcpyAsync(sc + 2 * B, cout_b, (size_t)B * 4, hipMemcpyDeviceToDevice, st);
-    }
+    if (!N->dry()) launch_gather3(cin_b, cskip_b, cout_b, sc, B, st);
     N->k_cin = sc; N->k_cskip = sc + B; N->k_cout = sc + 2 * B;
     cin_b = N->k_cin; cskip_b = N->k_cskip; cout_b = N->k_cout;
   }
@@ -1306,19 +1321,16 @@
       const int C = h->C, G = gn_groups(C), Hh = h->H, Ww = h->W;
       Tens* np = N->mk(B, Hh, Ww, 2, rec);
       float* stats = N->tmp((long long)B * G * 2);
-      const size_t mark = N->arena.off;
-      float* a = N->tmp(h->numel());
       Tens* prevp = pyr; Tens* hh = h;
       if (!N->dry()) {
         { View vx; vx.a = h; view_stats(N, vx, Hh * Ww, G, stats); }
-        launch_gn_apply(single(h->p, C), stats, gw.gamma, gw.beta, B, Hh, Ww, C, G, 0, 1, a, nullptr, st);
+        const C2oGn gn{stats, gw.gamma, gw.beta, G, 1};
         if (N->fir) {
-          launch_conv_c2out(a, C, cw.wf, cw.bias, nullptr, np->p, B, Hh, Ww, C, 9, 0, st);
+          launch_conv_c2out(h->p, C, cw.wf, cw.bias, nullptr, np->p, B, Hh, Ww, C, 9, 0, st, &gn);
           if (prevp) launch_fir_up2(prevp->p, np->p, B, Hh / 2, Ww / 2, 2, 1.f, 1, st);
         } else
-        launch_conv_c2out(a, C, cw.wf, cw.bias, prevp ? prevp->p : nullptr, np->p, B, Hh, Ww, C, 9, 0, st);
+        launch_conv_c2out(h->p, C, cw.wf, cw.bias, prevp ? prevp->p : nullptr, np->p, B, Hh, Ww, C, 9, 0, st, &gn);
       }
-      N->arena.off = mark;
       if (rec) { const GNW* gp = &gw; const ConvW* cp = &cw; N->tape.push_back([=]() {
         const size_t mk = N->arena.off;
         float* da = N->tmp(hh->numel());
@@ -1351,6 +1363,7 @@
     gemm_b(N, o2, 2 * Fb, 0, false, N->W->basisI, 2 * Fb, 0, false, frames, Kp, 0, B * Tp, Kp, 2 * Fb, nullptr, nullptr, 1.f, 0, 1);
     launch_ola(frames, Kp, Tp, nfft, hop, N->inv_env, y, B, L, N->pad, cskip_b ? x : nullptr, cskip_b, cout_b, st);
   }
+  if (!N->dry()) settle_csum(N);
   N->have_tape = rec;
 }
 
diff --git a/buddy_amd/csrc/ops.hip b/buddy_amd/csrc/ops.hip
--- a/buddy_amd/csrc/ops.hip
+++ b/buddy_amd/csrc/ops.hip
@@ -18,6 +18,12 @@
 __device__ __forceinline__ void st4(float* p, float4 v) { *reinterpret_cast<float4*>(p) = v; }
 __device__ __forceinline__ float4 add4(float4 a, float4 b) { return make_float4(a.x + b.x, a.y + b.y, a.z + b.z, a.w + b.w); }
 __device__ __forceinline__ float4 mul4(float4 a, float s) { return make_float4(a.x * s, a.y * s, a.z * s, a.w * s); }
+__device__ __forceinline__ float4 gn_act4(float4 v, float mean, float rstd, float4 gm, float4 bt, int silu) {
+  float4 z = make_float4((v.x - mean) * rstd * gm.x + bt.x, (v.y - mean) * rstd * gm.y + bt.y,
+                         (v.z - mean) * rstd * gm.z + bt.z, (v.w - mean) * rstd * gm.w + bt.w);
+  if (silu) z = make_float4(silu_f(z.x), silu_f(z.y), silu_f(z.z), silu_f(z.w));
+  return z;
+}
 
 __device__ __forceinline__ float4 da_eff(const float* da, int mode, int b, int h, int w, int H, int W, int C, int c) {
   if (mode == 0) return ld4(da + (((long long)b * H + h) * W + w) * C + c);
@@ -188,6 +194,57 @@
   }
 }
 
+__global__ __launch_bounds__(256) void csum_collapse_finalize_kernel(const double* __restrict__ partial, int chunks, int C0, double* __restrict__ csum0,
+                                                                     const double* __restrict__ c1, int C, int G, int HW, float eps,
+                                                                     float* __restrict__ out) {
+  __shared__ double red[256 * 2];
+  __shared__ double cs[64 * 2];
+  const int tid = threadIdx.x, cl = tid & 15, sl = tid >> 4, g = blockIdx.x, b = blockIdx.y;
+  const int cpg = C / G;
+  for (int base = 0; base < cpg; base += 16) {
+    const int i = base + cl, c = g * cpg + i;
+    const bool mine = i < cpg && c < C0;
+    double s = 0, t = 0;
+    if (mine)
+      for (int ch = sl; ch < chunks; ch += 16) {
+        const double2 v = *reinterpret_cast<const double2*>(partial + (((long long)b * chunks + ch) * C0 + c) * 2);
+        s += v.x; t += v.y;
+      }
+    red[tid * 2] = s; red[tid * 2 + 1] = t;
+    __syncthreads();
+    if (sl == 0 && i < cpg) {
+      if (mine) {
+        for (int l = 1; l < 16; ++l) { s += red[(l * 16 + cl) * 2]; t += red[(l * 16 + cl) * 2 + 1]; }
+        csum0[((long long)b * C0 + c) * 2] = s; csum0[((long long)b * C0 + c) * 2 + 1] = t;
+      } else {
+        const double* p = c1 + ((long long)b * (C - C0) + (c - C0)) * 2;
+        s = p[0]; t = p[1];
+      }
+      cs[i * 2] = s; cs[i * 2 + 1] = t;
+    }
+    __syncthreads();
+  }
+  if (tid < 64) {
+    double s = 0, t = 0;
+    for (int i = tid; i < cpg; i += 64) { s += cs[i * 2]; t += cs[i * 2 + 1]; }
+#pragma unroll
+    for (int off = 32; off > 0; off >>= 1) { s += __shfl_down(s, off, 64); t += __shfl_down(t, off, 64); }
+    if (tid == 0) {
+      const double n = (double)cpg * (double)HW;
+      float* o = out + ((long long)b * G + g) * 2;
+      const double mean = s / n;
+      double var = t / n - mean * mean;
+      if (var < 0) var = 0;
+      o[0] = (float)mean; o[1] = (float)(1.0 / sqrt(var + (double)eps));
+    }
+  }
+}
+
+__global__ __launch_bounds__(64) void gather3_kernel(const float* a, const float* b, const float* c, float* out, int n) {
+  const int i = blockIdx.x * 64 + threadIdx.x;
+  if (i < n) { out[i] = a[i]; out[n + i] = b[i]; out[2 * n + i] = c[i]; }
+}
+
 __global__ __launch_bounds__(256) void gn_apply_kernel(Src2 x, const float* stats, const float* gamma, const float* beta, int B, int H,
                                                        int W, int C, int G, int mode, int silu, float* out, float* pooled_raw) {
   const int q = C >> 2, cpg = C / G;
@@ -199,12 +256,7 @@
     const int c = quad * 4, g = c / cpg;
     const float mean = stats[((long long)b * G + g) * 2], rstd = stats[((long long)b * G + g) * 2 + 1];
     const float4 gm = ld4(gamma + c), bt = ld4(beta + c);
-    auto act = [&](float4 v) {
-      float4 z = make_float4((v.x - mean) * rstd * gm.x + bt.x, (v.y - mean) * rstd * gm.y + bt.y,
-                             (v.z - mean) * rstd * gm.z + bt.z, (v.w - mean) * rstd * gm.w + bt.w);
-      if (silu) z = make_float4(silu_f(z.x), silu_f(z.y), silu_f(z.z), silu_f(z.w));
-      return z;
-    };
+    auto act = [&](float4 v) { return gn_act4(v, mean, rstd, gm, bt, silu); };
     if (mode == 0) {
       const long long p = ((long long)b * H + h) * W + w;
       st4(out + p * C + c, act(ld4(src_ptr(x, p, c))));
@@ -278,12 +330,7 @@
   src += (long long)b * a.HW * ld;
   float* dst = out + (long long)b * a.HW * a.C + c;
   const int p0 = blockIdx.x * a.ppc, p1 = min(a.HW, p0 + a.ppc);
-  auto act = [&](float4 v) {
-    float4 z = make_float4((v.x - mean) * rstd * gm.x + bt.x, (v.y - mean) * rstd * gm.y + bt.y,
-                           (v.z - mean) * rstd * gm.z + bt.z, (v.w - mean) * rstd * gm.w + bt.w);
-    if (silu) z = make_float4(silu_f(z.x), silu_f(z.y), silu_f(z.z), silu_f(z.w));
-    return z;
-  };
+  auto act = [&](float4 v) { return gn_act4(v, mean, rstd, gm, bt, silu); };
   int p = p0 + lp;
   for (; p + 3 * a.pl < p1; p += 4 * a.pl) {
     float4 v[4];
@@ -595,9 +642,9 @@
   }
 }
 
-template <int TAPS>
+template <int TAPS, bool GN>
 __global__ __launch_bounds__(256) void conv_c2out_kernel(const float* x, int ldX, const float* w, const float* bias, const float* up_add,
-                                                         float* y, int B, int H, int W, int Cin, int accumulate) {
+                                                         float* y, int B, int H, int W, int Cin, int accumulate, C2oGn gn) {
   const int lpp = Cin >> 2, ppb = 256 / lpp;
   const int tid = threadIdx.x, sub = tid % lpp, slot = tid / lpp;
   const int c = sub * 4;
@@ -608,6 +655,8 @@
     for (int j = 0; j < 8; ++j) wr[t][j] = w[((long long)t * Cin + c) * 2 + j];
   const long long npix = (long long)B * H * W;
   const long long ngroups = (npix + ppb - 1) / ppb;
+  float4 gm = make_float4(0.f, 0.f, 0.f, 0.f), bt = gm;
+  if constexpr (GN) { gm = ld4(gn.gamma + c); bt = ld4(gn.beta + c); }
   for (long long gidx = blockIdx.x; gidx < ngroups; gidx += gridDim.x) {
     const long long p = gidx * ppb + slot;
     float s0 = 0.f, s1 = 0.f;
@@ -615,11 +664,14 @@
     if (p < npix) {
       long long pix = p;
       wq = (int)(pix % W); pix /= W; h = (int)(pix % H); b = (int)(pix / H);
+      float mean = 0.f, rstd = 0.f;
+      if constexpr (GN) { const float* sp = gn.stats + ((long long)b * gn.G + c / (Cin / gn.G)) * 2; mean = sp[0]; rstd = sp[1]; }
 #pragma unroll
       for (int t = 0; t < TAPS; ++t) {
         const int dy = (TAPS == 9) ? t / 3 - 1 : 0, dx = (TAPS == 9) ? t % 3 - 1 : 0;
         if ((unsigned)(h + dy) >= (unsigned)H || (unsigned)(wq + dx) >= (unsigned)W) continue;
-        const float4 v = ld4(x + (p + dy * W + dx) * ldX + c);
+        float4 v = ld4(x + (p + dy * W + dx) * ldX + c);
+        if constexpr (GN) v = gn_act4(v, mean, rstd, gm, bt, gn.silu);
         s0 += v.x * wr[t][0] + v.y * wr[t][2] + v.z * wr[t][4] + v.w * wr[t][6];
         s1 += v.x * wr[t][1] + v.y * wr[t][3] + v.z * wr[t][5] + v.w * wr[t][7];
       }
@@ -639,8 +691,9 @@
 }
 
 constexpr int C2O_TH = 8, C2O_TW = 32, C2O_CK = 32, C2O_PITCH = C2O_CK + 4;
+template <bool GN>
 __global__ __launch_bounds__(256) void conv_c2out_tiled_kernel(const float* __restrict__ x, int ldX, const float* __restrict__ w, const float* bias,
-                                                               const float* up_add, float* y, int B, int H, int W, int Cin, int accumulate) {
+                                                               const float* up_add, float* y, int B, int H, int W, int Cin, int accumulate, C2oGn gn) {
   __shared__ __attribute__((aligned(16))) float tile[(C2O_TH + 2) * (C2O_TW + 2) * C2O_PITCH];
   __shared__ __attribute__((aligned(16))) float wsh[9 * C2O_CK * 2];
   const int tid = threadIdx.x;
@@ -656,6 +709,7 @@
   constexpr int NLD = (NPX * (C2O_CK / 4) + 255) / 256;
   for (int c0 = 0; c0 < Cin; c0 += C2O_CK) {
     float4 v[NLD];
+    unsigned inb = 0;
 #pragma unroll
     for (int i = 0; i < NLD; ++i) {
       const int e = tid + 256 * i;
@@ -663,7 +717,18 @@
       const int hr = px / (C2O_TW + 2), wc = px - hr * (C2O_TW + 2);
       const int gh = h0 - 1 + hr, gw = w0 - 1 + wc;
       v[i] = make_float4(0.f, 0.f, 0.f, 0.f);
-      if (e < NPX * (C2O_CK / 4) && (unsigned)gh < (unsigned)H && (unsigned)gw < (unsigned)W) v[i] = ld4(x + (((long long)b * H + gh) * W + gw) * ldX + c0 + c4);
+      if (e < NPX * (C2O_CK / 4) && (unsigned)gh < (unsigned)H && (unsigned)gw < (unsigned)W) {
+        v[i] = ld4(x + (((long long)b * H + gh) * W + gw) * ldX + c0 + c4);
+        if constexpr (GN) inb |= 1u << i;
+      }
+    }
+    if constexpr (GN) {
+      const int c = c0 + (tid & 7) * 4;
+      const float* sp = gn.stats + ((long long)b * gn.G + c / (Cin / gn.G)) * 2;
+      const float mean = sp[0], rstd = sp[1];
+      const float4 gm = ld4(gn.gamma + c), bt = ld4(gn.beta + c);
+#pragma unroll
+      for (int i = 0; i < NLD; ++i) if (inb >> i & 1) v[i] = gn_act4(v[i], mean, rstd, gm, bt, gn.silu);
     }
     float wv[3];
 #pragma unroll
@@ -703,8 +768,9 @@
   }
 }
 
+template <bool GN>
 __global__ __launch_bounds__(256, 3) void conv_c2out_strip_kernel(const float* __restrict__ x, int ldX, const float* __restrict__ w, const float* bias,
-                                                               const float* up_add, float* y, int B, int H, int W, int Cin, int accumulate) {
+                                                               const float* up_add, float* y, int B, int H, int W, int Cin, int accumulate, C2oGn gn) {
   __shared__ __attribute__((aligned(16))) float tile[(C2O_TH + 2) * (C2O_TW + 2) * C2O_PITCH];
   __shared__ __attribute__((aligned(16))) float wsh[9 * C2O_CK * 2];
   const int tid = threadIdx.x;
@@ -721,6 +787,7 @@
   constexpr int NLD = (NPX * (C2O_CK / 4) + 255) / 256;
   for (int c0 = 0; c0 < Cin; c0 += C2O_CK) {
     float4 v[NLD];
+    unsigned inb = 0;
 #pragma unroll
     for (int i = 0; i < NLD; ++i) {
       const int e = tid + 256 * i;
@@ -728,7 +795,18 @@
       const int hr = px / (C2O_TW + 2), wc = px - hr * (C2O_TW + 2);
       const int gh = h0 - 1 + hr, gw = w0 - 1 + wc;
       v[i] = make_float4(0.f, 0.f, 0.f, 0.f);
-      if (e < NPX * (C2O_CK / 4) && (unsigned)gh < (unsigned)H && (unsigned)gw < (unsigned)W) v[i] = ld4(x + (((long long)b * H + gh) * W + gw) * ldX + c0 + c4);
+      if (e < NPX * (C2O_CK / 4) && (unsigned)gh < (unsigned)H && (unsigned)gw < (unsigned)W) {
+        v[i] = ld4(x + (((long long)b * H + gh) * W + gw) * ldX + c0 + c4);
+        if constexpr (GN) inb |= 1u << i;
+      }
+    }
+    if constexpr (GN) {
+      const int c = c0 + (tid & 7) * 4;
+      const float* sp = gn.stats + ((long long)b * gn.G + c / (Cin / gn.G)) * 2;
+      const float mean = sp[0], rstd = sp[1];
+      const float4 gm = ld4(gn.gamma + c), bt = ld4(gn.beta + c);
+#pragma unroll
+      for (int i = 0; i < NLD; ++i) if (inb >> i & 1) v[i] = gn_act4(v[i], mean, rstd, gm, bt, gn.silu);
     }
     float wv[3];
 #pragma unroll
@@ -961,19 +1039,32 @@
 void launch_csum_collapse(const double* partial, int chunks, int B, int C, double* csum, hipStream_t st) {
   hipLaunchKernelGGL(csum_collapse_kernel, dim3((C + 15) / 16, B), dim3(256), 0, st, partial, chunks, C, csum);
 }
-void launch_chan_sums(const float* x, int B, int HW, int C, double* partial, double* csum, hipStream_t st) {
+int launch_chan_sums(const float* x, int B, int HW, int C, double* partial, double* csum, hipStream_t st) {
   Src2 s; s.p0 = x; s.p1 = nullptr; s.C0 = C; s.ld0 = C; s.ld1 = 0;
   RedArgs a = make_red(s, B, 1, HW, C, 1, partial);
   prof_hbm_begin(4.0 * B * HW * C, st);
   hipLaunchKernelGGL(chan_reduce_kernel<0>, dim3(a.chunks, B), dim3(256), 0, st, a);
-  launch_csum_collapse(partial, a.chunks, B, C, csum, st);
+  if (csum) launch_csum_collapse(partial, a.chunks, B, C, csum, st);
   prof_hbm_end(st);
+  return a.chunks;
 }
 void launch_gn_stats_partial(const double* partial, int chunks, int B, int HW, int C, int G, float eps, float* stats, hipStream_t st) {
   hipLaunchKernelGGL(group_finalize_kernel<0>, dim3(G, B), dim3(256), 0, st, partial, stats, C, G, chunks, HW, eps);
 }
 void launch_gn_stats_csum(const double* csum0, const double* csum1, int C0, int B, int HW, int C, int G, float eps, float* stats, hipStream_t st) {
   hipLaunchKernelGGL(group_finalize_csum_kernel, dim3(G, B), dim3(64), 0, st, csum0, csum1, csum1 ? C0 : C, C, G, HW, eps, stats);
+}
+void launch_csum_collapse_stats(const double* partial, int chunks, double* csum0, const double* csum1, int C0, int B, int HW, int C, int G, float eps,
+                                float* stats, hipStream_t st) {
+  if (C / G > 64) {
+    launch_csum_collapse(partial, chunks, B, C0, csum0, st);
+    launch_gn_stats_csum(csum0, csum1, C0, B, HW, C, G, eps, stats, st);
+    return;
+  }
+  hipLaunchKernelGGL(csum_collapse_finalize_kernel, dim3(G, B), dim3(256), 0, st, partial, chunks, C0, csum0, csum1, C, G, HW, eps, stats);
+}
+void launch_gather3(const float* a, const float* b, const float* c, float* out, int n, hipStream_t st) {
+  hipLaunchKernelGGL(gather3_kernel, dim3(cdiv(n, 64)), dim3(64), 0, st, a, b, c, out, n);
 }
 
 void launch_gn_apply(Src2 x, const float* stats, const float* gamma, const float* beta, int B, int H, int W, int C, int G, int mode, int silu,
@@ -1098,21 +1189,28 @@
 }
 
 void launch_conv_c2out(const float* x, int ldX, const float* w, const float* bias, const float* up_add, float* y, int B, int H, int W, int Cin,
-                       int taps, int accumulate, hipStream_t st) {
+                       int taps, int accumulate, hipStream_t st, const C2oGn* gn) {
   const int ppb = 256 / (Cin / 4);
   long long groups = ((long long)B * H * W + ppb - 1) / ppb;
   int grid = (int)(groups < 256 * 8 ? groups : 256 * 8);
   const bool tiled = cur_opt().c2out_tiled != 0;
+  const C2oGn g = gn ? *gn : C2oGn{nullptr, nullptr, nullptr, 1, 0};
+#define C2O(K, GRID) do { if (gn) hipLaunchKernelGGL((K<true>), dim3(GRID), dim3(256), 0, st, x, ldX, w, bias, up_add, y, B, H, W, Cin, accumulate, g); \
+                          else hipLaunchKernelGGL((K<false>), dim3(GRID), dim3(256), 0, st, x, ldX, w, bias, up_add, y, B, H, W, Cin, accumulate, g); } while (0)
   if (taps == 9 && cur_opt().c2out_tiled == 2 && Cin % C2O_CK == 0 && ldX % 4 == 0) {
     const int blocks = B * ((H + C2O_TH - 1) / C2O_TH) * ((W + C2O_TW - 1) / C2O_TW);
-    hipLaunchKernelGGL(conv_c2out_strip_kernel, dim3(blocks), dim3(256), 0, st, x, ldX, w, bias, up_add, y, B, H, W, Cin, accumulate);
+    C2O(conv_c2out_strip_kernel, blocks);
   } else if (taps == 9 && tiled && Cin % C2O_CK == 0 && ldX % 4 == 0) {
     const int blocks = B * ((H + C2O_TH - 1) / C2O_TH) * ((W + C2O_TW - 1) / C2O_TW);
-    hipLaunchKernelGGL(conv_c2out_tiled_kernel, dim3(blocks), dim3(256), 0, st, x, ldX, w, bias, up_add, y, B, H, W, Cin, accumulate);
-  } else if (taps == 9)
-    hipLaunchKernelGGL(conv_c2out_kernel<9>, dim3(grid), dim3(256), 0, st, x, ldX, w, bias, up_add, y, B, H, W, Cin, accumulate);
-  else
-    hipLaunchKernelGGL(conv_c2out_kernel<1>, dim3(grid), dim3(256), 0, st, x, ldX, w, bias, up_add, y, B, H, W, Cin, accumulate);
+    C2O(conv_c2out_tiled_kernel, blocks);
+  } else if (taps == 9) {
+    if (gn) hipLaunchKernelGGL((conv_c2out_kernel<9, true>), dim3(grid), dim3(256), 0, st, x, ldX, w, bias, up_add, y, B, H, W, Cin, accumulate, g);
+    else hipLaunchKernelGGL((conv_c2out_kernel<9, false>), dim3(grid), dim3(256), 0, st, x, ldX, w, bias, up_add, y, B, H, W, Cin, accumulate, g);
+  } else {
+    if (gn) hipLaunchKernelGGL((conv_c2out_kernel<1, true>), dim3(grid), dim3(256), 0, st, x, ldX, w, bias, up_add, y, B, H, W, Cin, accumulate, g);
+    else hipLaunchKernelGGL((conv_c2out_kernel<1, false>), dim3(grid), dim3(256), 0, st, x, ldX, w, bias, up_add, y, B, H, W, Cin, accumulate, g);
+  }
+#undef C2O
 }
 
 void launch_reflect_pad(const float* x, float* xp, int B, int L, int pad, int Lp, float scale, const float* scale_b, hipStream_t st) {
diff --git a/include/buddy_hip.h b/include/buddy_hip.h
--- a/include/buddy_hip.h
+++ b/include/buddy_hip.h
@@ -124,6 +124,11 @@
 int buddy_groupnorm_act_bwd(const float* x, const float* gamma, const float* beta, const float* stats, const float* dy, float* dx,
                             void* scratch, float* red, int B, int H, int W, int C, int G, int mode, int silu, void* stream);
 
+int buddy_gn_conv_c2out(const float* x, const float* gamma, const float* beta, const float* stats, int G, int silu, const float* w, const float* bias,
+                        const float* up_add, float* y, float* act_tmp, int B, int H, int W, int C, void* stream);
+int buddy_gn_stats_from_partials(const double* partial, int chunks, double* csum0, const double* csum1, int C0, int B, int HW, int C, int G, int merged,
+                                 float* stats, void* stream);
+
 int buddy_fir_resample2(const float* x, float* y, int B, int H, int W, int C, int up, float scale, int accumulate, void* stream);
 int buddy_ncsnpp_set_fir(void* handle, int fir);
 int buddy_options_check(void);
```

After: 142.0. 0.989x the previous value.
